# Bismarrck/tensoralloy

Hardware: AMD Instinct MI355X
Metric: atom-steps/sec (energy+forces), 4000-atom Ni rcut=6.5 A (higher is better)
Workload: dtype f64

## Files before the change

### tensoralloy_amd/csrc/ta_api.hip

```cpp
#include <hip/hip_runtime.h>

#include <algorithm>
#include <chrono>
#include <climits>
#include <cmath>
#include <cstdio>
#include <cstdlib>
#include <cstring>
#include <stdexcept>
#include <string>
#include <vector>

#include "ta_device.h"
#include "ta_internal.h"
#include "ta_md.h"
#include "ta_neb.h"
#include "ta_relax.h"

namespace ta {
size_t mlp_scratch_doubles(const MlpDev &mlp);
void launch_mlp_impl(const MlpDev &mlp, int activation, int ndim, const int32_t *atoms, int n_atoms,
                     const DeviceBatch &b, const Options &opt, double *scratch, hipStream_t s,
                     MlpLaunchInfo *info = nullptr);
size_t mlp_all_scratch_doubles(const MlpDev *mlps_host, int nel, const int32_t *elem_start);
size_t td_scratch_doubles(const MlpDev *nets, int nel, int K, const int32_t *elem_start, bool da_global);
void launch_td_all(const MlpDev *nets_dev, const MlpDev *nets_host, int nel, int K, int act_h, int act,
                   int sommerfeld, int ndim, const DeviceBatch &b, bool da_global, const double *T, double *u_atom,
                   double *s_atom, double *scratch, hipStream_t s, MlpLaunchInfo *info = nullptr);
void launch_mlp_all(const MlpDev *mlps_dev, const MlpDev *mlps_host, int nel, int activation, int ndim,
                    const DeviceBatch &b, const Options &opt, double *scratch, hipStream_t s,
                    MlpLaunchInfo *info = nullptr);
int mlp_param_count(const MlpDev &mlp);
size_t mlp_grad_scratch_doubles(const MlpDev &mlp, int n_atoms);
size_t mlp_grad_partial_doubles(const MlpDev &mlp, int n_atoms);
void launch_mlp_grad(const MlpDev &mlp, int activation, int ndim, const int32_t *atoms, int n_atoms,
                     const DeviceBatch &b, const double *frame_coeff, double *scratch, double *partial,
                     double *grad, hipStream_t s);
size_t mlp_grad2_scratch_doubles(const MlpDev &mlp, int n_atoms);
void launch_mlp_grad2(const MlpDev &mlp, int activation, int ndim, const int32_t *atoms, int n_atoms,
                      const DeviceBatch &b, const double *dG, const double *frame_coeff, double *scratch,
                      double *partial, double *grad, hipStream_t s, double *kappa_out = nullptr);
int td_param_count(const MlpDev *nets, int nel);
void td_grad2_sizes(const MlpDev *nets, int nel, int K, const int32_t *elem_start, size_t *scratch,
                    size_t *partial);
void launch_td_grad2(const MlpDev *nets_dev, const MlpDev *nets_host, int nel, int K, int act_h, int act,
                     int sommerfeld, int ndim, const DeviceBatch &b, const double *T, const double *dG,
                     const double *coeff, double *scratch, double *partial, double *grad, hipStream_t s);
void launch_pair_vec(const DeviceBatch &b, double *Dv, hipStream_t s);
void launch_backward_hvp(const SFParams &sf, const AngChunk &ch, int nb, int ng, int nz, bool first, bool angular,
                         const DeviceBatch &b, const double *Dv, const double *Dd, const double *wdot, double *gv,
                         double *gd, hipStream_t s);
void launch_hvp_gather(const DeviceBatch &b, const double *Dv, const double *Dd, const double *gv, const double *gd,
                       double *fdot, double *wdot_at, hipStream_t s);
void launch_pair_tangent(const DeviceBatch &b, const double *dR, const double *dh, double *dD, hipStream_t s);
void launch_descriptor_jvp(const DeviceBatch &b, int ndim, const double *J, const double *dD, double *dG,
                           hipStream_t s);
void launch_one_hot(double *dEdG, int64_t n_atoms, int ndim, int c, hipStream_t s);
struct GrapModel;
bool grap_hvp_supported(const GrapModel *);
void launch_grap_hvp(GrapModel *, const DeviceBatch &b, double eps, const double *Dv, const double *Dd,
                     const double *wdot, double *gv, double *gd, hipStream_t s);
GrapModel *grap_create(const ta_model_desc *m, std::string &err);
int grap_ndim(const GrapModel *g);
bool grap_uses_filter_net(const GrapModel *g);
void grap_destroy(GrapModel *);
void grap_ensure(GrapModel *, const DeviceBatch &b);
void launch_grap_forward(GrapModel *, const DeviceBatch &b, double eps, hipStream_t s);
void launch_grap_backward(GrapModel *, const DeviceBatch &b, hipStream_t s);
int64_t grap_filter_param_count(const GrapModel *g);
void grap_update_filter_weights(GrapModel *g, const double *flat, int64_t n, hipStream_t s);
int grap_filter_table_knots(const GrapModel *g);
void grap_set_filter_tables(GrapModel *g, bool on, int n_knots, hipStream_t s);
int grap_filter_table_target(const GrapModel *g, bool on, int n_knots);
void grap_mark_trained(GrapModel *g);
void grap_suspend_filter_tables(GrapModel *g, bool suspend);
std::string grap_filter_train_refusal(const GrapModel *g);
size_t grap_filter_grad_doubles(const GrapModel *g, const DeviceBatch &b);
void launch_grap_filter_tangent(GrapModel *g, const DeviceBatch &b, double eps, const double *Dv, const double *Dd,
                                double *Gdot, hipStream_t s);
void grap_filter_gradient(GrapModel *g, const DeviceBatch &b, double eps, const double *Dv, const double *Dd,
                          const double *kappa, double *scratch, double *grad, hipStream_t s);
struct EamModel;
EamModel *eam_create(const ta_model_desc *m, const Options &opt, std::string &err);
void eam_destroy(EamModel *);
void eam_ensure(EamModel *, const DeviceBatch &b);
void eam_tabulate(EamModel *m, int n_r, const double *r, int n_rho, const double *rho, double *rho_of_r,
                  double *phi_of_r, double *embed_of_rho, double *u_of_r, double *w_of_r,
                  hipStream_t s);
void eam_compute(EamModel *, const DeviceBatch &b, uint32_t want, hipStream_t s,
                 hipEvent_t *ev );
void eam_set_list_cutoff(EamModel *, double rc );
bool eam_is_plain(const EamModel *);
void eam_set_nn_tables(EamModel *, bool on);
bool eam_hvp_supported(const EamModel *);
size_t eam_hvp_extra_doubles(const EamModel *, const DeviceBatch &b, int n_dir);
void eam_hvp(EamModel *, const DeviceBatch &b, int n_dir, bool unit, int first, const double *dR, const double *dh,
             double *dFdot, double *fdot, double *wdot, double *extra, hipStream_t s);
bool eam_nn_tables_on(const EamModel *);
void eam_mark_trained(EamModel *);
int64_t eam_param_count(const EamModel *);
void eam_update_weights(EamModel *, const double *flat, int64_t n);
int64_t eam_constant_count(const EamModel *);
void eam_get_constants(const EamModel *, double *flat);
void eam_update_constants(EamModel *, const double *flat, int64_t n);
void eam_constant_gradient(EamModel *, const DeviceBatch &b, const double *frame_coeff, const double *dR,
                           const double *dh, double *grad, hipStream_t s);
void eam_energy_gradient(EamModel *, const DeviceBatch &b, const double *frame_coeff, double *grad,
                         hipStream_t s);
bool eam_loss_gradient_supported(const EamModel *);
void eam_loss_gradient(EamModel *, const DeviceBatch &b, const double *frame_coeff, const double *dR,
                       const double *dh, double *grad, hipStream_t s);
}

namespace {

thread_local std::string g_create_error;

struct HipError : std::runtime_error {
  using std::runtime_error::runtime_error;
};

#define HIP_CHECK(expr)                                                                      \
  do {                                                                                       \
    hipError_t _e = (expr);                                                                  \
    if (_e != hipSuccess)                                                                    \
      throw HipError(std::string(#expr) + ": " + hipGetErrorString(_e) + " (" __FILE__ ":" + \
                     std::to_string(__LINE__) + ")");                                        \
  } while (0)

template <typename T>
struct DevBuf {
  T *ptr = nullptr;
  size_t cap = 0;
  void ensure(size_t n) {
    if (n <= cap) return;
    size_t want = n + n / 8 + 64;
    T *fresh = nullptr;
    hipError_t e = hipMalloc((void **)&fresh, want * sizeof(T));
    if (e != hipSuccess && ptr) {
      (void)hipGetLastError();
      HIP_CHECK(hipFree(ptr));
      ptr = nullptr;
      cap = 0;
      e = hipMalloc((void **)&fresh, want * sizeof(T));
    }
    if (e != hipSuccess) {
      (void)hipGetLastError();
      throw HipError(std::string("hipMalloc of ") + std::to_string(want * sizeof(T)) + " bytes: " +
                     hipGetErrorString(e));
    }
    if (ptr) HIP_CHECK(hipFree(ptr));
    ptr = fresh;
    cap = want;
  }
  void release() {
    if (ptr) (void)hipFree(ptr);
    ptr = nullptr;
    cap = 0;
  }
};

__global__ __launch_bounds__(256) void staged_copy_kernel(double *__restrict__ dst,
                                                          const double *__restrict__ src, size_t n) {
  for (size_t k = (size_t)blockIdx.x * 256 + threadIdx.x; k < n; k += (size_t)gridDim.x * 256) dst[k] = src[k];
}
constexpr size_t kStagedCopyMaxBytes = 4u << 20;

void staged_copy(double *dst, const double *src, size_t n, bool to_host, const ta::Options &opt, hipStream_t s) {
  if (n == 0) return;
  if (n * sizeof(double) > kStagedCopyMaxBytes || opt.staged_copy_dma) {
    HIP_CHECK(hipMemcpyAsync(dst, src, n * sizeof(double), to_host ? hipMemcpyDeviceToHost : hipMemcpyHostToDevice, s));
    return;
  }
  const unsigned blocks = (unsigned)std::min<size_t>((n + 255) / 256, 256);
  hipLaunchKernelGGL(staged_copy_kernel, dim3(blocks), dim3(256), 0, s, dst, src, n);
  HIP_CHECK(hipGetLastError());
}

void wait_stream(hipStream_t s, const ta::Options &opt) {
  if (!opt.sync_blocking) {
    const auto t0 = std::chrono::steady_clock::now();
    for (;;) {
      const hipError_t e = hipStreamQuery(s);
      if (e == hipSuccess) return;
      if (e != hipErrorNotReady) {
        (void)hipGetLastError();
        break;
      }
      if (std::chrono::steady_clock::now() - t0 > std::chrono::microseconds(400)) break;
    }
  }
  HIP_CHECK(hipStreamSynchronize(s));
}

struct PinnedBuf {
  char *ptr = nullptr;
  size_t cap = 0;
  void ensure(size_t n) {
    if (n <= cap) return;
    if (ptr) HIP_CHECK(hipHostFree(ptr));
    ptr = nullptr;
    cap = 0;
    size_t want = n + n / 8 + 256;
    HIP_CHECK(hipHostMalloc((void **)&ptr, want, hipHostMallocDefault));
    cap = want;
  }
  void release() {
    if (ptr) (void)hipHostFree(ptr);
    ptr = nullptr;
    cap = 0;
  }
};

struct ChunkPlan {
  ta::AngChunk ch;
  int nb, ng, nz;
};

}

struct ta_context {
  ta::Options opt;
  int device = 0;
  hipStream_t stream = nullptr;
  hipStream_t own_stream = nullptr;
  int kind = 0;
  int n_elements = 0;
  int activation = 0;
  double rmax = 0.0;
  ta::SFParams sf;
  std::vector<ChunkPlan> chunks;
  std::vector<ChunkPlan> chunks_v2;
  bool use_v2 = false;
  ta::MlpDev *mlp_dev = nullptr;
  ta::MlpDev mlp[ta::kMaxElements];
  bool td = false, td_sommerfeld = false;
  int td_act = 0, td_K = 0;
  ta::MlpDev td_nets[3 * ta::kMaxElements];
  ta::MlpDev *td_dev = nullptr;
  std::vector<void *> model_allocs;
  ta::EamModel *eam = nullptr;
  ta::GrapModel *grap = nullptr;

  ta::HostPairs hp;
  ta::DeviceBatch db;
  bool have_batch = false;
  uint32_t last_want = 0;

  PinnedBuf stage_in, stage_out;
  DevBuf<char> inbuf;
  DevBuf<double> results;
  size_t o_blk = 0;
  int res_n_blk = 0;
  DevBuf<double> rec, part4, G, dEdG, g, wat, bpart, fown, benergy, mlp_scratch;
  DevBuf<double> td_T, td_u, td_s;
  DevBuf<unsigned long long> masks;
  DevBuf<uint32_t> job_word;
  DevBuf<int32_t> job_count;
  DevBuf<uint32_t> job_word_own;
  DevBuf<int32_t> job_count_own;
  bool triangles = true;
  bool tri_cells_ok = false;
  bool tri_cells_wide_ok = false;
  int last_bwd_variant = 0;
  ta::MlpLaunchInfo last_mlp_launch;
  DevBuf<int32_t> pair_start, seg_start, pair_i, pair_j, pair_shift, pair_rev;
  ta::NlGrid *d_grids = nullptr;
  DevBuf<int32_t> nl_wrap, nl_binid, nl_bin_count, nl_bin_start, nl_bin_cursor, nl_bin_atoms, nl_counts;
  DevBuf<unsigned long long> nl_stats, nl_zero;
  unsigned long long *nl_stats_ptr = nullptr;
  bool nl_sorted = false;
  bool nl_rev_done = false;
  bool nl_zero_clean = false;
  int64_t nl_zero_atoms = -1;
  int nl_zero_bins = -1;
  DevBuf<double> hvp_buf;
#ifdef TA_PHASE_STAMPS
  DevBuf<unsigned long long> stamp_buf;
#endif
  DevBuf<ta::NlRec> nl_recs;
  bool pairs_on_device = false;
  bool descriptors_valid = false;
  DevBuf<double> train_scratch, train_partial, train_grad, train_coeff;
  DevBuf<double> jvp_J, tan_dD, tan_dG, tan_dir;
  DevBuf<double> filt_scratch;
  bool jvp_valid = false;

  double skin = 0.0;
  double r_list = 0.0;
  std::vector<int32_t> keep_species;
  std::vector<int32_t> keep_natoms, keep_pbc;
  std::vector<double> ref_pos, ref_cells;
  size_t o_pos = 0, o_cells = 0, o_species = 0;
  DevBuf<int32_t> ex_pair_i, ex_pair_j, ex_pair_shift, ex_pair_rev, ex_pair_start, ex_pair_stop, ex_seg_start, ex_counts,
      ex_map, ex_blk, ex_slot_q;
  bool filtered = false;
  bool upload_pending = false;
  bool mirror_next = false;
  uint32_t mirror_want = 0;
  int64_t n_list_builds = 0, n_list_reuses = 0;

  bool md_valid = false;
  DevBuf<double> md_mass, md_vel, md_ref, md_epot, md_ke;
  DevBuf<int32_t> md_blk_start;
  DevBuf<unsigned> md_status;
  PinnedBuf md_status_host;
  std::vector<int32_t> md_blk_start_host;
  int md_chunk = 0, md_n_blk = 0;
  int64_t md_ref_builds = -1;
  double md_kT0 = 0.0, md_tau = 0.0;
  double md_lv_kT0 = 0.0, md_friction = 0.0;
  uint64_t md_seed = 0;
  int64_t md_step = 0;
  DevBuf<double> md_noise;
  bool md_baro_on = false;
  bool md_baro_running = false;
  ta_md_barostat_params md_baro_p = {0.0, 0.0, 0.0, {1, 1, 1}, 1};
  DevBuf<double> md_baro_scale, md_baro_rec;
  std::vector<double> md_baro_ones;
  bool md_rec_valid = false;
  std::vector<double> md_rec_volume, md_rec_press;

  bool relax_valid = false;
  ta_fire_params relax_p = {0.1, 1.0, 0.2, 1.1, 0.5, 0.1, 0.99, 5};
  DevBuf<double> relax_vel, relax_part;
  DevBuf<uint8_t> relax_fixed;
  DevBuf<ta::RelaxFrameState> relax_state;
  DevBuf<int> relax_count;
  std::vector<ta::RelaxFrameState> relax_state_host;
  bool relax_cell_on = false;
  bool cell_running = false;
  ta_relax_cell_params relax_cell_p = {0.0, 0.0, {1, 1, 1, 1, 1, 1}, 0, 0};
  DevBuf<double> relax_cell_h0, relax_cell_cf, relax_cell_G, relax_cell_vel, relax_cell_fmax2, md_ref_cells;
  std::vector<double> relax_cell_G_host, relax_cell_vel_host;
  bool relax_band_on = false;
  bool relax_band_ran = false;
  ta_band_params relax_band_p = {0.1, 0, 0};
  std::vector<uint8_t> relax_fixed_host;
  DevBuf<double> band_force, band_tau, band_part;
  DevBuf<uint8_t> band_fixed;
  DevBuf<ta::RelaxFrameState> band_state;
  DevBuf<int32_t> band_layout;
  ta::RelaxFrameState band_state_host = {};
  std::vector<double> band_energy_host;

  hipEvent_t ev[2 * TA_N_KERNEL_SLOTS + 2] = {nullptr};
  std::string err;
};

namespace {

int fail(ta_context *h, int code, const std::string &msg) {
  if (h)
    h->err = msg;
  else
    g_create_error = msg;
  return code;
}

std::string td_inference_only(const char *fn) {
  return std::string(fn) + ": not available for finite-temperature (temperature-dependent) models "
         "(no analytic Hessian-vector products)";
}

std::string fs_inference_only(const char *fn) {
  return std::string(fn) + ": not available for eam/fs models (inference only: no weight, constant or loss "
         "gradients and no analytic Hessian-vector products; differences of the forces give the latter)";
}

template <typename T>
T *upload(ta_context *h, const std::vector<T> &v) {
  T *d = nullptr;
  size_t n = v.size() ? v.size() : 1;
  HIP_CHECK(hipMalloc((void **)&d, n * sizeof(T)));
  h->model_allocs.push_back(d);
  if (!v.empty()) HIP_CHECK(hipMemcpy(d, v.data(), v.size() * sizeof(T), hipMemcpyHostToDevice));
  return d;
}

int round_up(int x, int m) { return (x + m - 1) / m * m; }

void hd_series(int cutoff, double beta, ta::AngChunk &ch) {
  ch.n_hd = 0;
  for (double &c : ch.hd) c = 0.0;
  if (cutoff != TA_CUTOFF_COSINE || !(beta >= 0.0)) return;
  constexpr int NT = 64;
  const long double pi2 = 9.869604401089358618834490999876151135L;
  long double fc[NT], ex[NT], prod[NT];
  long double t = 1.0L;
  for (int k = 0; k < NT; ++k) {
    fc[k] = 0.5L * t + (k == 0 ? 0.5L : 0.0L);
    t *= -pi2 / (long double)((2 * k + 1) * (2 * k + 2));
  }
  t = 1.0L;
  for (int k = 0; k < NT; ++k) {
    ex[k] = t;
    t *= -(long double)beta / (long double)(k + 1);
  }
  for (int k = 0; k < NT; ++k) {
    long double acc = 0.0L;
    for (int j = 0; j <= k; ++j) acc += fc[j] * ex[k - j];
    prod[k] = acc;
  }
  constexpr int N0 = 40;
  static long double tstar[N0][N0];
  static bool have_t = false;
  if (!have_t) {
    for (auto &row : tstar)
      for (auto &c : row) c = 0.0L;
    tstar[0][0] = 1.0L;
    tstar[1][0] = -1.0L;
    tstar[1][1] = 2.0L;
    for (int n = 1; n + 1 < N0; ++n)
      for (int k = 0; k <= n + 1; ++k)
        tstar[n + 1][k] = (k > 0 ? 4.0L * tstar[n][k - 1] : 0.0L) - 2.0L * tstar[n][k] - tstar[n - 1][k];
    have_t = true;
  }
  long double tail0 = 0.0L, dtail0 = 0.0L;
  for (int k = N0; k < NT; ++k) {
    tail0 += fabsl(prod[k]);
    dtail0 += (long double)k * fabsl(prod[k]);
  }
  for (int n : {12, 16, 24}) {
    long double a[N0];
    for (int k = 0; k < N0; ++k) a[k] = prod[k];
    long double err = tail0, derr = dtail0;
    for (int d = N0 - 1; d >= n; --d) {
      const long double q = a[d] / tstar[d][d];
      for (int k = 0; k <= d; ++k) a[k] -= q * tstar[d][k];
      err += fabsl(q);
      derr += 2.0L * (long double)d * (long double)d * fabsl(q);
    }
    if (err < 1e-17L && derr < 1e-15L) {
      ch.n_hd = n;
      for (int k = 0; k < n; ++k) ch.hd[k] = (double)a[k];
      return;
    }
  }
}

void build_mlp(ta_context *h, const ta_model_desc *m, int ndim);

void build_sf_model(ta_context *h, const ta_model_desc *m) {
  using namespace ta;
  SFParams &sf = h->sf;
  std::memset(&sf, 0, sizeof(sf));
  const int nel = m->n_elements;
  if (m->n_eta < 1 || m->n_omega < 1 || !m->eta || !m->omega)
    throw std::invalid_argument("eta / omega must be non-empty");
  if (m->n_eta * m->n_omega > kMaxRadial)
    throw std::domain_error("more than 64 radial (eta x omega) combinations");
  if (!(m->rcut > 0.0)) throw std::invalid_argument("rcut must be positive");
  sf.rcut = m->rcut;
  sf.acut = m->angular ? m->acut : m->rcut;
  if (m->angular && !(m->acut > 0.0)) throw std::invalid_argument("acut must be positive");
  sf.inv_rc2 = 1.0 / (sf.rcut * sf.rcut);
  sf.inv_ac2 = 1.0 / (sf.acut * sf.acut);
  sf.two_inv_ac2 = 2.0 * sf.inv_ac2;
  sf.eps = m->eps > 0.0 ? m->eps : 1e-14;
  sf.n_elements = nel;
  sf.n_rad = m->n_eta * m->n_omega;
  sf.angular = m->angular ? 1 : 0;
  sf.cutoff = m->cutoff_function;
  if (sf.cutoff != TA_CUTOFF_COSINE && sf.cutoff != TA_CUTOFF_POLYNOMIAL)
    throw std::invalid_argument("unknown cutoff function");
  for (int e = 0; e < m->n_eta; ++e)
    for (int o = 0; o < m->n_omega; ++o) {
      sf.eta[e * m->n_omega + o] = m->eta[e];
      sf.omega[e * m->n_omega + o] = m->omega[o];
    }
  for (int c = 1; c < sf.n_rad; ++c) {
    if ((c & 3) == 0 || sf.omega[c] != sf.omega[c - 1] || !(sf.eta[c - 1] > 0.0)) continue;
    const double k = sf.eta[c] / sf.eta[c - 1];
    if (k >= 2.0 && k <= 16.0 && k == std::nearbyint(k) && k * sf.eta[c - 1] == sf.eta[c] &&
        !h->opt.no_eta_chain)
      sf.eta_pow[c] = (signed char)k;
  }
  sf.n_radial_dim = nel * sf.n_rad;
  sf.n_ang = 0;
  sf.n_beta = 0;
  if (m->angular) {
    if (m->n_beta < 1 || m->n_gamma < 1 || m->n_zeta < 1 || !m->beta || !m->gamma || !m->zeta)
      throw std::invalid_argument("beta / gamma / zeta must be non-empty for an angular model");
    if (m->n_beta > kMaxBetaSlots)
      throw std::domain_error("more than 3 beta values are not supported by the pair record");
    sf.n_beta = m->n_beta;
    for (int k = 0; k < m->n_beta; ++k) sf.beta[k] = m->beta[k];
    sf.n_ang = m->n_beta * m->n_gamma * m->n_zeta;
    for (int pass = 0; pass < 2; ++pass)
    for (int b0 = 0; b0 < m->n_beta; b0 += (pass == 0 ? 2 : 1))
      for (int g0 = 0; g0 < m->n_gamma; g0 += 2)
        for (int z0 = 0; z0 < m->n_zeta; z0 += 2) {
          ChunkPlan cp;
          std::memset(&cp, 0, sizeof(cp));
          cp.nb = std::min(pass == 0 ? 2 : 1, m->n_beta - b0);
          cp.ng = std::min(2, m->n_gamma - g0);
          cp.nz = std::min(2, m->n_zeta - z0);
          for (int ib = 0; ib < cp.nb; ++ib) {
            cp.ch.beta[ib] = m->beta[b0 + ib];
            cp.ch.hslot[ib] = b0 + ib;
          }
          cp.ch.safe_pow = m->safe_pow ? 1 : 0;
          for (int ig = 0; ig < cp.ng; ++ig) cp.ch.gamma[ig] = m->gamma[g0 + ig];
          for (int iz = 0; iz < cp.nz; ++iz) {
            const double z = m->zeta[z0 + iz];
            cp.ch.zeta[iz] = z;
            cp.ch.kz[iz] = std::pow(2.0, 1.0 - z);
            const double zr = std::nearbyint(z);
            cp.ch.zeta_int[iz] = (zr == z && z >= 1.0 && z <= 1024.0) ? (int)zr : -1;
          }
          for (int ib = 0; ib < cp.nb; ++ib)
            for (int ig = 0; ig < cp.ng; ++ig)
              for (int iz = 0; iz < cp.nz; ++iz)
                cp.ch.chan[(ib * cp.ng + ig) * cp.nz + iz] =
                    ((b0 + ib) * m->n_gamma + (g0 + ig)) * m->n_zeta + (z0 + iz);
          if (pass == 1) hd_series(sf.cutoff, cp.ch.beta[0], cp.ch);
          (pass == 0 ? h->chunks : h->chunks_v2).push_back(cp);
        }
  }
  const int n_aterms = m->angular ? nel * (nel + 1) / 2 : 0;
  (void)0;
  sf.ndim = sf.n_radial_dim + n_aterms * sf.n_ang;
  h->rmax = std::max(sf.rcut, sf.acut);
  build_mlp(h, m, sf.ndim);
}

void build_net(ta_context *h, ta::MlpDev &md, int L, const int32_t *sizes, const double *&wsrc, int resnet) {
  using namespace ta;
  if (L < 1 || L > kMaxLayers) throw std::domain_error("MLP depth out of range (1..8 layers)");
  md.n_layers = L;
  md.max_np = md.max_kp = 0;
  for (int l = 0; l < L; ++l) {
    MlpLayerDev &ly = md.layer[l];
    ly.k = sizes[l];
    ly.n = sizes[l + 1];
    if (ly.k < 1 || ly.n < 1 || ly.k > 512 || ly.n > 512)
      throw std::domain_error("MLP layer width out of range (1..512)");
    ly.kp = round_up(ly.k, 16);
    ly.np = round_up(ly.n, 16);
    ly.act = (l < L - 1) ? 1 : 0;
    ly.res = (resnet && l > 0 && l < L - 1 && ly.k == ly.n) ? 1 : 0;
    std::vector<double> w((size_t)ly.kp * ly.np, 0.0), wt((size_t)ly.np * ly.kp, 0.0), bb(ly.np, 0.0);
    for (int k = 0; k < ly.k; ++k)
      for (int n = 0; n < ly.n; ++n) {
        const double v = wsrc[(size_t)k * ly.n + n];
        w[(size_t)k * ly.np + n] = v;
        wt[(size_t)n * ly.kp + k] = v;
      }
    wsrc += (size_t)ly.k * ly.n;
    for (int n = 0; n < ly.n; ++n) bb[n] = wsrc[n];
    wsrc += ly.n;
    ly.w = upload(h, w);
    ly.wt = upload(h, wt);
    ly.b = upload(h, bb);
    md.max_np = std::max(md.max_np, ly.np);
    md.max_kp = std::max(md.max_kp, ly.kp);
  }
}

void build_mlp(ta_context *h, const ta_model_desc *m, int ndim) {
  using namespace ta;
  const int nel = m->n_elements;
  if (!m->n_layers || !m->layer_sizes || !m->weights)
    throw std::invalid_argument("MLP description missing");
  h->activation = m->activation;
  if (m->activation < 0 || m->activation > TA_ACT_ELU)
    throw std::invalid_argument("unknown activation");
  const int td = m->finite_temperature;
  const int32_t *sizes = m->layer_sizes;
  const double *wsrc = m->weights;
  if (td) {
    if ((td & ~(TA_TD_ON | TA_TD_SOMMERFELD | (0xff << TA_TD_ACT_SHIFT))) || !(td & TA_TD_ON))
      throw std::invalid_argument("unknown finite_temperature bits");
    h->td = true;
    h->td_sommerfeld = (td & TA_TD_SOMMERFELD) != 0;
    h->td_act = (td >> TA_TD_ACT_SHIFT) & 0xff;
    if (h->td_act > TA_ACT_ELU) throw std::invalid_argument("unknown activation of the H nets");
    h->td_K = 0;
    for (int q = 0; q < 3; ++q)
      for (int el = 0; el < nel; ++el) {
        MlpDev &md = h->td_nets[q * nel + el];
        const int L = m->n_layers[q * nel + el];
        if (L < 1 || L > kMaxLayers) throw std::domain_error("MLP depth out of range (1..8 layers)");
        if (q == 0) {
          if (sizes[0] != ndim) throw std::invalid_argument("H input size does not match the descriptor length");
          if (el == 0) h->td_K = sizes[L];
          if (sizes[L] != h->td_K) throw std::invalid_argument("H output width differs between elements");
        } else {
          if (sizes[0] != h->td_K + 1) throw std::invalid_argument("U / S input size must be the H width + 1");
          if (sizes[L] != 1) throw std::invalid_argument("U / S output size must be 1");
        }
        build_net(h, md, L, sizes, wsrc, m->use_resnet_dt);
        if (q == 0 && m->minmax_scale) {
          if (!m->xlo || !m->xhi) throw std::invalid_argument("minmax_scale set but xlo/xhi missing");
          std::vector<double> lo(m->xlo + (size_t)el * ndim, m->xlo + (size_t)(el + 1) * ndim);
          std::vector<double> hi(m->xhi + (size_t)el * ndim, m->xhi + (size_t)(el + 1) * ndim);
          md.xlo = upload(h, lo);
          md.xhi = upload(h, hi);
// ... 204 lines not shown
            h->db.frame_of_atom, h->d_grids, w, h->pair_i.ptr, h->pair_j.ptr, h->pair_shift.ptr,
            h->pair_rev.ptr, h->stream);
  }
  HIP_CHECK(hipGetLastError());
}

#ifdef TA_PHASE_STAMPS
static void dump_stamps(ta_context *h) {
  const std::string &path = h->opt.phase_stamps_out;
  if (path.empty() || !h->db.stamps || h->db.n_blk <= 0) return;
  const size_t n = (size_t)2 * h->db.n_blk * 8;
  std::vector<unsigned long long> v(n);
  (void)hipStreamSynchronize(h->stream);
  (void)hipMemcpy(v.data(), h->db.stamps, n * sizeof(unsigned long long), hipMemcpyDeviceToHost);
  FILE *fp = std::fopen(path.c_str(), "w");
  if (!fp) return;
  for (int k = 0; k < 2; ++k)
    for (int b = 0; b < h->db.n_blk; ++b) {
      std::fprintf(fp, "%d %d", k, b);
      for (int q = 0; q < 8; ++q) std::fprintf(fp, " %llu", v[((size_t)k * h->db.n_blk + b) * 8 + q]);
      std::fprintf(fp, "\n");
    }
  std::fclose(fp);
}
#endif

void launch_head(ta_context *h, const ta::DeviceBatch &db, hipStream_t s) {
  if (h->td)
    ta::launch_td_all(h->td_dev, h->td_nets, h->n_elements, h->td_K, h->td_act, h->activation,
                      h->td_sommerfeld ? 1 : 0, h->sf.ndim, db, h->opt.mlp_da_global, h->td_T.ptr, h->td_u.ptr, h->td_s.ptr,
                      h->mlp_scratch.ptr, s, &h->last_mlp_launch);
  else
    ta::launch_mlp_all(h->mlp_dev, h->mlp, h->n_elements, h->activation, h->sf.ndim, db, h->opt, h->mlp_scratch.ptr,
                       s, &h->last_mlp_launch);
}

void compute_impl(ta_context *h, uint32_t want, bool timed, double *slot_ms) {
  using namespace ta;
#ifdef TA_PHASE_STAMPS
  if (h->db.n_blk > 0) {
    h->stamp_buf.ensure((size_t)2 * h->db.n_blk * 8 + 8);
    h->db.stamps = h->stamp_buf.ptr;
    (void)hipMemsetAsync(h->db.stamps, 0, (size_t)2 * h->db.n_blk * 8 * sizeof(unsigned long long), h->stream);
  }
#endif
  h->db.rec4 = nullptr;
  h->db.own_sums = 0;
  const DeviceBatch &db = h->db;
  hipStream_t s = h->stream;
  const bool need_forces = (want & (TA_WANT_FORCES | TA_WANT_VIRIAL)) != 0;
  auto begin = [&](int slot) {
    if (timed) HIP_CHECK(hipEventRecord(h->ev[2 * slot], s));
  };
  auto end = [&](int slot) {
    if (timed) HIP_CHECK(hipEventRecord(h->ev[2 * slot + 1], s));
  };
  bool used[TA_N_KERNEL_SLOTS] = {false};

  const bool has_mlp = h->kind == TA_MODEL_SF_MLP || h->kind == TA_MODEL_GRAP_MLP;
  if ((want & TA_WANT_REUSE_DESCRIPTORS) && has_mlp && h->descriptors_valid && !need_forces) {
    begin(TA_K_MLP);
    launch_head(h, db, s);
    end(TA_K_MLP);
    used[TA_K_MLP] = true;
  } else if (h->kind == TA_MODEL_SF_MLP) {
    h->db.rec4 = (h->sf.angular && h->use_v2 && !h->opt.full_records) ? h->db.rec : nullptr;
    if (!h->use_v2) {
      begin(TA_K_PAIR_GEOMETRY);
      launch_pair_geometry(h->sf, db, s);
      end(TA_K_PAIR_GEOMETRY);
      used[TA_K_PAIR_GEOMETRY] = true;
    }
    h->sf.ang_scale = h->use_v2 ? 1.0 : 0.5;
    const bool tri_cells = (h->relax_cell_on || h->md_baro_on) ? h->tri_cells_wide_ok : h->tri_cells_ok;
    const bool tri = h->use_v2 && h->triangles && tri_cells && h->n_elements == 1 && need_forces;
    h->db.job_word_own = (tri && h->db.job_count) ? h->job_word_own.ptr : nullptr;
    h->db.job_count_own = (tri && h->db.job_count) ? h->job_count_own.ptr : nullptr;
    h->last_bwd_variant = 0;
    const bool reduce_in_forward = h->sf.angular && h->use_v2;
    if (h->sf.angular) {
      begin(TA_K_G4_FORWARD);
      if (h->use_v2) {
        bool geometry = true;
        size_t left = h->chunks_v2.size();
        for (const ChunkPlan &cp : h->chunks_v2) {
          --left;
          launch_g4_forward_v2(h->sf, cp.ch, cp.ng, cp.nz, geometry, left == 0, db, h->opt, s);
          geometry = false;
        }
      } else
        for (const ChunkPlan &cp : h->chunks) launch_g4_forward(h->sf, cp.ch, cp.nb, cp.ng, cp.nz, db, s);
      end(TA_K_G4_FORWARD);
      used[TA_K_G4_FORWARD] = true;
    }
    if (!reduce_in_forward) {
      begin(TA_K_DESCRIPTOR_REDUCE);
      launch_descriptor_reduce(h->sf, db, s);
      end(TA_K_DESCRIPTOR_REDUCE);
      used[TA_K_DESCRIPTOR_REDUCE] = true;
    }
    begin(TA_K_MLP);
    launch_head(h, db, s);
    end(TA_K_MLP);
    used[TA_K_MLP] = true;
    if (need_forces) {
      begin(TA_K_BACKWARD);
      if (h->sf.angular) {
        bool first = true;
        if (h->use_v2)
          for (const ChunkPlan &cp : h->chunks_v2) {
            h->last_bwd_variant |= launch_backward_v2(h->sf, cp.ch, cp.ng, cp.nz, first, tri, db, h->opt, s);
            first = false;
          }
        else
          for (const ChunkPlan &cp : h->chunks) {
            launch_backward(h->sf, cp.ch, cp.nb, cp.ng, cp.nz, first, false, db, s);
            first = false;
          }
      } else {
        AngChunk dummy;
        std::memset(&dummy, 0, sizeof(dummy));
        launch_backward(h->sf, dummy, 1, 1, 1, true, true, db, s);
      }
      end(TA_K_BACKWARD);
      used[TA_K_BACKWARD] = true;
      begin(TA_K_FORCE_GATHER);
      launch_force_gather(h->sf, db, h->opt.gather_w, s);
      end(TA_K_FORCE_GATHER);
      used[TA_K_FORCE_GATHER] = true;
    }
  } else if (h->kind == TA_MODEL_GRAP_MLP) {
    const bool net_exact = ta::grap_uses_filter_net(h->grap) && !ta::grap_filter_table_knots(h->grap);
    h->db.rec4 = (!net_exact && !h->opt.full_records) ? h->db.rec : nullptr;
    begin(TA_K_GRAP);
    launch_grap_forward(h->grap, db, h->sf.eps, s);
    end(TA_K_GRAP);
    used[TA_K_GRAP] = true;
    begin(TA_K_MLP);
    launch_head(h, db, s);
    end(TA_K_MLP);
    used[TA_K_MLP] = true;
    if (need_forces) {
      begin(TA_K_BACKWARD);
      h->db.own_sums = h->opt.no_own_sums ? 0 : 1;
      launch_grap_backward(h->grap, db, s);
      end(TA_K_BACKWARD);
      used[TA_K_BACKWARD] = true;
      begin(TA_K_FORCE_GATHER);
      launch_force_gather(h->sf, db, h->opt.gather_w, s);
      end(TA_K_FORCE_GATHER);
      used[TA_K_FORCE_GATHER] = true;
    }
  } else {
    h->db.rec4 = h->opt.full_records ? nullptr : h->db.rec;
    begin(TA_K_EAM);
    eam_compute(h->eam, db, want, s, nullptr);
    end(TA_K_EAM);
    used[TA_K_EAM] = true;
  }
  begin(TA_K_FRAME_REDUCE);
  {
    double *mirror = nullptr;
    int64_t n_tail = 0;
    h->mirror_want = 0;
    if (h->mirror_next && !timed) {
      const size_t N = (size_t)db.n_atoms, F = (size_t)db.n_frames;
      h->stage_out.ensure((10 * F + 4 * N + 2) * sizeof(double));
      mirror = reinterpret_cast<double *>(h->stage_out.ptr);
      n_tail = (int64_t)(need_forces ? 4 * N : N);
      h->mirror_want = want | TA_WANT_ENERGY | TA_WANT_ATOMIC;
    }
    launch_frame_reduce(db, need_forces, mirror, n_tail, s);
  }
  end(TA_K_FRAME_REDUCE);
  used[TA_K_FRAME_REDUCE] = true;
  HIP_CHECK(hipGetLastError());
  h->last_want = want;
  h->descriptors_valid = true;

  if (timed) {
    HIP_CHECK(hipStreamSynchronize(s));
    for (int k = 0; k < TA_N_KERNEL_SLOTS; ++k) {
      if (!used[k]) continue;
      float ms = 0.f;
      HIP_CHECK(hipEventElapsedTime(&ms, h->ev[2 * k], h->ev[2 * k + 1]));
      slot_ms[k] += ms;
    }
  }
}

template <typename F>
int guarded(ta_context *h, F &&fn) {
  try {
    if (h) HIP_CHECK(hipSetDevice(h->device));
    fn();
    return TA_OK;
  } catch (const HipError &e) {
    return fail(h, TA_ERR_HIP, e.what());
  } catch (const std::domain_error &e) {
    return fail(h, TA_ERR_UNSUPPORTED, e.what());
  } catch (const std::invalid_argument &e) {
    return fail(h, TA_ERR_INVALID, e.what());
  } catch (const std::bad_alloc &) {
    return fail(h, TA_ERR_NOMEM, "host allocation failed");
  } catch (const std::exception &e) {
    return fail(h, TA_ERR_INVALID, e.what());
  }
}

}

extern "C" {

int ta_abi_version(void) { return TA_ABI_VERSION; }
int ta_model_desc_size(void) { return (int)sizeof(ta_model_desc); }

int ta_device_count(void) {
  int n = 0;
  if (hipGetDeviceCount(&n) != hipSuccess) return 0;
  return n;
}

const char *ta_last_error(ta_handle h) { return h ? h->err.c_str() : g_create_error.c_str(); }

int ta_create(const ta_model_desc *model, int device, ta_handle *out) {
  if (!model || !out) return fail(nullptr, TA_ERR_INVALID, "null argument");
  *out = nullptr;
  int ndev = 0;
  if (hipGetDeviceCount(&ndev) != hipSuccess || ndev <= 0)
    return fail(nullptr, TA_ERR_HIP, "no HIP device available: this library has no CPU fallback");
  if (device < 0 || device >= ndev) return fail(nullptr, TA_ERR_INVALID, "device index out of range");
  if (model->n_elements < 1 || model->n_elements > ta::kMaxElements)
    return fail(nullptr, TA_ERR_UNSUPPORTED, "n_elements must be in 1..8");
  ta_context *h = new ta_context();
  h->opt = ta::options_from_env();
  h->device = device;
  h->kind = model->kind;
  h->n_elements = model->n_elements;
  int rc = guarded(h, [&]() {
    hipDeviceProp_t prop;
    HIP_CHECK(hipGetDeviceProperties(&prop, device));
    if (std::strncmp(prop.gcnArchName, "gfx950", 6) != 0)
      throw HipError(std::string("device is ") + prop.gcnArchName +
                     ", this library is built for gfx950 only");
    HIP_CHECK(hipStreamCreateWithFlags(&h->own_stream, hipStreamNonBlocking));
    h->stream = h->own_stream;
    for (auto &e : h->ev) HIP_CHECK(hipEventCreate(&e));
    if (model->kind == TA_MODEL_SF_MLP) {
      build_sf_model(h, model);
    } else if (model->kind == TA_MODEL_GRAP_MLP) {
      if (model->cutoff_function != TA_CUTOFF_COSINE && model->cutoff_function != TA_CUTOFF_POLYNOMIAL)
        throw std::invalid_argument("unknown cutoff function");
      std::string err;
      h->grap = ta::grap_create(model, err);
      if (!h->grap) throw std::invalid_argument(err);
      h->rmax = model->rcut;
      std::memset(&h->sf, 0, sizeof(h->sf));
      h->sf.n_elements = model->n_elements;
      h->sf.eps = model->eps > 0.0 ? model->eps : 1e-14;
      h->sf.ndim = ta::grap_ndim(h->grap);
      build_mlp(h, model, h->sf.ndim);
    } else if (model->kind == TA_MODEL_EAM_ALLOY || model->kind == TA_MODEL_EAM_ADP || model->kind == TA_MODEL_EAM_FS) {
      std::string err;
      h->eam = ta::eam_create(model, h->opt, err);
      if (!h->eam) throw std::invalid_argument(err);
      h->rmax = model->rcut;
      std::memset(&h->sf, 0, sizeof(h->sf));
      h->sf.n_elements = model->n_elements;
      h->sf.eps = model->eps > 0.0 ? model->eps : 1e-14;
    } else {
      throw std::invalid_argument("unknown model kind");
    }
  });
  if (rc != TA_OK) {
    g_create_error = h->err;
    ta_destroy(h);
    return rc;
  }
  *out = h;
  return TA_OK;
}

int ta_destroy(ta_handle h) {
  if (!h) return TA_OK;
  (void)hipSetDevice(h->device);
#ifdef TA_PHASE_STAMPS
  dump_stamps(h);
#endif
  if (h->stream) (void)hipStreamSynchronize(h->stream);
  for (void *p : h->model_allocs) (void)hipFree(p);
  if (h->eam) ta::eam_destroy(h->eam);
  if (h->grap) ta::grap_destroy(h->grap);
  h->stage_in.release(); h->stage_out.release(); h->inbuf.release(); h->results.release();
  h->rec.release(); h->part4.release(); h->G.release();
  h->dEdG.release(); h->g.release(); h->wat.release(); h->bpart.release(); h->fown.release();
  h->benergy.release(); h->mlp_scratch.release();
  h->train_scratch.release(); h->train_partial.release(); h->train_grad.release(); h->train_coeff.release();
  h->jvp_J.release(); h->tan_dD.release(); h->tan_dG.release(); h->tan_dir.release();
  h->pair_start.release(); h->seg_start.release(); h->pair_i.release(); h->pair_j.release();
  h->pair_shift.release(); h->pair_rev.release();
  for (auto *b : {&h->ex_pair_i, &h->ex_pair_j, &h->ex_pair_shift, &h->ex_pair_rev, &h->ex_pair_start, &h->ex_pair_stop,
                  &h->ex_seg_start, &h->ex_counts, &h->ex_map, &h->ex_blk, &h->ex_slot_q})
    b->release();
  h->masks.release(); h->job_word.release(); h->job_count.release();
  h->job_word_own.release(); h->job_count_own.release();
  for (auto *b : {&h->nl_wrap, &h->nl_binid, &h->nl_bin_count, &h->nl_bin_start, &h->nl_bin_cursor,
                  &h->nl_bin_atoms, &h->nl_counts})
    b->release();
  h->nl_stats.release();
  h->nl_zero.release();
  h->hvp_buf.release();
  h->filt_scratch.release();
  h->nl_recs.release();
  for (auto *b : {&h->md_mass, &h->md_vel, &h->md_ref, &h->md_epot, &h->md_ke, &h->md_noise}) b->release();
  h->md_blk_start.release();
  h->md_status.release();
  h->md_status_host.release();
  h->relax_vel.release();
  h->relax_part.release();
  h->relax_fixed.release();
  h->relax_state.release();
  h->relax_count.release();
  for (auto *b : {&h->band_force, &h->band_tau, &h->band_part}) b->release();
  h->band_fixed.release();
  h->band_state.release();
  h->band_layout.release();
  for (auto *b : {&h->relax_cell_h0, &h->relax_cell_cf, &h->relax_cell_G, &h->relax_cell_vel, &h->relax_cell_fmax2,
                  &h->md_ref_cells})
    b->release();
  for (auto &e : h->ev)
    if (e) (void)hipEventDestroy(e);
  if (h->own_stream) (void)hipStreamDestroy(h->own_stream);
  delete h;
  return TA_OK;
}

}

namespace {
void ensure_job_lists(ta_context *h, size_t n_blk) {
  if (h->opt.no_jobs || !h->use_v2 || n_blk == 0) {
    h->db.job_count = nullptr;
    return;
  }
  const int stride = ta::v2_job_stride(h->db.cap);
  h->job_word.ensure(n_blk * (size_t)stride + 8);
  h->job_count.ensure(n_blk + 8);
  if (h->n_elements == 1) {
    h->job_word_own.ensure(n_blk * (size_t)stride + 8);
    h->job_count_own.ensure(n_blk + 8);
  }
  h->db.job_word = h->job_word.ptr;
  h->db.job_count = h->job_count.ptr;
  h->db.job_stride = stride;
}

bool filter_applies(const ta_context *h) {
  if (!(h->skin > 0.0) || h->hp.n_atoms == 0 || h->opt.no_list_filter) return false;
  if (h->kind == TA_MODEL_SF_MLP) return h->use_v2;
  if (h->kind == TA_MODEL_EAM_ALLOY || h->kind == TA_MODEL_EAM_FS) return ta::eam_is_plain(h->eam);
  return false;
}

void apply_filter(ta_context *h) {
  using namespace ta;
  const size_t N = (size_t)h->hp.n_atoms, P = (size_t)h->hp.n_pairs;
  const int nel = h->n_elements;
  h->ex_pair_i.ensure(P + 1);
  h->ex_pair_j.ensure(P + 1);
  h->ex_pair_shift.ensure(3 * P + 3);
  h->ex_pair_rev.ensure(P + 1);
  h->ex_pair_start.ensure(N + 1);
  h->ex_pair_stop.ensure(N + 1);
  h->ex_seg_start.ensure(N * (nel + 1) + 1);
  h->ex_map.ensure(P + 1);
  const int n_run_slots = nl_filter_blocks((int)N);
  h->ex_blk.ensure((size_t)n_run_slots + 4);
  const bool blocks = h->kind == TA_MODEL_SF_MLP;
  const bool indirect = blocks && !h->opt.filter_rev_kernel;
  if (indirect) h->ex_slot_q.ensure(P + 1);
  nl_filter((int)N, (int64_t)P, nel, h->rmax, h->db.pos, h->db.cells, h->db.frame_of_atom,
            h->pair_start.ptr, h->seg_start.ptr, h->pair_j.ptr, h->pair_shift.ptr, h->pair_rev.ptr, h->ex_map.ptr,
            h->ex_seg_start.ptr, h->ex_pair_start.ptr, h->ex_pair_stop.ptr, h->ex_pair_i.ptr, h->ex_pair_j.ptr,
            h->ex_pair_shift.ptr, h->ex_pair_rev.ptr, indirect ? h->ex_slot_q.ptr : nullptr, h->db.cap,
            blocks ? h->ex_blk.ptr : nullptr, h->stream);
  h->db.slot_q = indirect ? h->ex_slot_q.ptr : nullptr;
  h->db.rev_super = indirect ? h->pair_rev.ptr : nullptr;
  h->db.rev_map = indirect ? h->ex_map.ptr : nullptr;
  HIP_CHECK(hipGetLastError());
  h->db.pair_start = h->ex_pair_start.ptr;
  h->db.pair_stop = h->ex_pair_stop.ptr;
  h->db.seg_start = h->ex_seg_start.ptr;
  h->db.pair_i = h->ex_pair_i.ptr;
  h->db.pair_j = h->ex_pair_j.ptr;
  h->db.pair_shift = h->ex_pair_shift.ptr;
  h->db.pair_rev = h->ex_pair_rev.ptr;
  if (blocks) {
    h->db.blk_center = h->ex_blk.ptr;
    h->db.n_blk = n_run_slots;
    h->db.blk_groups = n_run_slots / 16;
    h->db.n_blk_dev = nullptr;
    ensure_job_lists(h, (size_t)n_run_slots);
  }
  h->filtered = true;
}

bool cells_admit_triangles(double rmax, int32_t n_frames, const ta_frame *frames) {
  for (int f = 0; f < n_frames; ++f) {
    const double *c = frames[f].cell;
    const double vol = std::fabs(c[0] * (c[4] * c[8] - c[5] * c[7]) - c[1] * (c[3] * c[8] - c[5] * c[6]) +
                                 c[2] * (c[3] * c[7] - c[4] * c[6]));
    for (int k = 0; k < 3; ++k) {
      if (!frames[f].pbc[k]) continue;
      const double *u = c + 3 * ((k + 1) % 3), *v = c + 3 * ((k + 2) % 3);
      const double nx = u[1] * v[2] - u[2] * v[1], ny = u[2] * v[0] - u[0] * v[2], nz = u[0] * v[1] - u[1] * v[0];
      const double area = std::sqrt(nx * nx + ny * ny + nz * nz);
      if (!(vol > rmax * area)) return false;
    }
  }
  return true;
}

void set_frames_impl(ta_context *h, int32_t n_frames, const ta_frame *frames, ta_batch_info *info) {
  for (int f = 0; f < n_frames; ++f) {
    const ta_frame &fr = frames[f];
    if (fr.n_atoms < 0 || (fr.n_atoms > 0 && (!fr.species || !fr.positions)) || !fr.cell || !fr.pbc)
      throw std::invalid_argument("frame " + std::to_string(f) + ": null array");
  }
  const auto t_begin = std::chrono::steady_clock::now();
  if (h->upload_pending) {
    HIP_CHECK(hipStreamSynchronize(h->stream));
    h->upload_pending = false;
  }
  h->have_batch = false;
  h->descriptors_valid = false;
  h->jvp_valid = false;
  h->mirror_want = 0;
  h->filtered = false;
  h->db.slot_q = h->db.rev_super = h->db.rev_map = nullptr;
  h->db.pair_stop = nullptr;
  h->db.blk_groups = 0;
  h->db.n_blk_dev = nullptr;
  h->r_list = h->rmax + h->skin;
  h->tri_cells_ok = cells_admit_triangles(h->rmax, n_frames, frames);
  h->tri_cells_wide_ok = cells_admit_triangles(h->r_list, n_frames, frames);
  size_t N = 0;
  for (int f = 0; f < n_frames; ++f) N += (size_t)frames[f].n_atoms;
  if (N >= (1u << 30)) throw std::runtime_error("batch too large for 32-bit atom indices");
  const size_t F = (size_t)n_frames;
  const int nel = h->n_elements;
  auto align16 = [](size_t x) { return (x + 15) & ~(size_t)15; };
  const size_t o_pos = 0;
  const size_t o_cells = align16(o_pos + 3 * N * sizeof(double));
  const size_t o_grids = align16(o_cells + 9 * F * sizeof(double));
  const size_t o_species = align16(o_grids + F * sizeof(ta::NlGrid));
  const size_t o_foa = align16(o_species + N * sizeof(int32_t));
  const size_t o_astart = align16(o_foa + N * sizeof(int32_t));
  const size_t o_elem = align16(o_astart + (F + 1) * sizeof(int32_t));
  const size_t o_blk = align16(o_elem + N * sizeof(int32_t));
  const size_t total = align16(o_blk + (N + 2) * sizeof(int32_t));
  h->stage_in.ensure(total);
  h->inbuf.ensure(total);
  char *hb = h->stage_in.ptr;
  double *pos = reinterpret_cast<double *>(hb + o_pos);
  double *cells = reinterpret_cast<double *>(hb + o_cells);
  ta::NlGrid *grids = reinterpret_cast<ta::NlGrid *>(hb + o_grids);
  int32_t *species = reinterpret_cast<int32_t *>(hb + o_species);
  int32_t *foa = reinterpret_cast<int32_t *>(hb + o_foa);
  int32_t *astart = reinterpret_cast<int32_t *>(hb + o_astart);
  int32_t *elem_atoms = reinterpret_cast<int32_t *>(hb + o_elem);
  size_t a = 0;
  astart[0] = 0;
  for (int f = 0; f < n_frames; ++f) {
    const ta_frame &fr = frames[f];
    const size_t n = (size_t)fr.n_atoms;
    if (n) {
      std::memcpy(&pos[3 * a], fr.positions, 3 * n * sizeof(double));
      std::memcpy(&species[a], fr.species, n * sizeof(int32_t));
    }
    std::memcpy(&cells[9 * (size_t)f], fr.cell, 9 * sizeof(double));
    for (size_t i = a; i < a + n; ++i) {
      foa[i] = f;
      if (species[i] < 0 || species[i] >= nel)
        throw std::runtime_error("frame " + std::to_string(f) + ": species index out of range");
      if (!std::isfinite(pos[3 * i]) || !std::isfinite(pos[3 * i + 1]) || !std::isfinite(pos[3 * i + 2]))
        throw std::runtime_error("frame " + std::to_string(f) + ": non-finite position");
    }
    a += n;
    astart[f + 1] = (int32_t)a;
  }
  {
    std::vector<int32_t> count(nel + 1, 0);
    for (size_t i = 0; i < N; ++i) count[species[i] + 1]++;
    for (int e = 0; e < nel; ++e) count[e + 1] += count[e];
    for (int e = 0; e <= nel; ++e) h->db.elem_start[e] = count[e];
    std::vector<int32_t> fill(count.begin(), count.end() - 1);
    for (size_t i = 0; i < N; ++i) elem_atoms[fill[species[i]]++] = (int32_t)i;
  }
  const auto t_nl = std::chrono::steady_clock::now();
  int n_bins = 0;
  bool device_nl = N > 0 && !h->opt.host_nl;
  for (int f = 0; f < n_frames && device_nl; ++f) {
    device_nl = ta::nl_make_grid(frames[f], h->r_list, n_bins, grids[f]);
    if (device_nl) n_bins += ta::nl_bins(grids[f]);
    if (n_bins > (1 << 24)) device_nl = false;
  }
  if (!device_nl) std::memset(static_cast<void *>(grids), 0, F * sizeof(ta::NlGrid));
  if (o_blk)
    staged_copy(reinterpret_cast<double *>(h->inbuf.ptr), reinterpret_cast<const double *>(hb), o_blk / sizeof(double),
                false, h->opt, h->stream);
  char *db_ = h->inbuf.ptr;
  h->db.n_frames = n_frames;
  h->db.pos = reinterpret_cast<double *>(db_ + o_pos);
  h->db.cells = reinterpret_cast<double *>(db_ + o_cells);
  h->d_grids = reinterpret_cast<ta::NlGrid *>(db_ + o_grids);
  h->db.species = reinterpret_cast<int32_t *>(db_ + o_species);
  h->db.frame_of_atom = reinterpret_cast<int32_t *>(db_ + o_foa);
  h->db.atom_start = reinterpret_cast<int32_t *>(db_ + o_astart);
  h->db.elem_atoms = reinterpret_cast<int32_t *>(db_ + o_elem);
  h->db.blk_center = reinterpret_cast<int32_t *>(db_ + o_blk);
  if (device_nl) {
    h->hp.atom_start.assign(astart, astart + F + 1);
    h->hp.frame_of_atom.assign(foa, foa + N);
    build_pairs_on_device(h, N, n_bins);
  } else {
    h->pairs_on_device = false;
    ta::build_pairs(n_frames, frames, nel, h->r_list, h->hp);
  }
  double nl_ms = std::chrono::duration<double, std::milli>(std::chrono::steady_clock::now() - t_nl).count();
  upload_batch(h);
  const auto t_fill = std::chrono::steady_clock::now();
  const bool list_done = h->pairs_on_device && h->nl_sorted && h->nl_rev_done;
  if (h->pairs_on_device && !list_done) {
    fill_pairs_on_device(h);
    staged_copy(reinterpret_cast<double *>(h->stage_out.ptr), reinterpret_cast<const double *>(h->nl_stats_ptr),
                8, true, h->opt, h->stream);
  }
  bool shapes_ok = h->n_elements <= 3;
  if (h->n_elements == 4 || h->n_elements == 5) {
    shapes_ok = !h->chunks_v2.empty();
    for (const ChunkPlan &cp : h->chunks_v2) shapes_ok = shapes_ok && cp.ng == 2 && cp.nz == 2;
  }
  h->use_v2 = h->kind == TA_MODEL_SF_MLP && h->sf.angular && shapes_ok &&
              h->hp.nnl_max <= ta::kCapMax && !h->opt.force_v1;
  const int cap = std::max(ta::kCapMin, (h->hp.nnl_max + 63) / 64 * 64);
  h->db.cap = cap;
  {
    int32_t *blk = reinterpret_cast<int32_t *>(hb + o_blk);
    int nb = 0;
    if (h->use_v2 && N) {
      blk[nb++] = 0;
      int32_t load = 0, ncent = 0;
      for (size_t i = 0; i < N; ++i) {
        const int32_t cnt = h->hp.pair_start[i + 1] - h->hp.pair_start[i];
        if (load + cnt > cap || ncent >= ta::kMaxCentersPerBlock) {
          blk[nb++] = (int32_t)i;
          load = 0;
          ncent = 0;
        }
        load += cnt;
        ++ncent;
      }
      blk[nb++] = (int32_t)N;
    }
    h->db.n_blk = nb ? nb - 1 : 0;
    h->res_n_blk = h->db.n_blk;
    h->o_blk = o_blk;
    ensure_job_lists(h, (size_t)h->db.n_blk);
    if (nb) {
      if (list_done)
        staged_copy(reinterpret_cast<double *>(db_ + o_blk), reinterpret_cast<const double *>(blk), ((size_t)nb + 1) / 2,
                    false, h->opt, h->stream);
      else
        HIP_CHECK(hipMemcpyAsync(db_ + o_blk, blk, (size_t)nb * sizeof(int32_t), hipMemcpyHostToDevice, h->stream));
    }
  }
  if (h->kind == TA_MODEL_SF_MLP) {
    if (!h->use_v2 && ta::g4_lds_bytes(h->hp.nnl_max) > 160 * 1024 && h->sf.angular)
      throw std::domain_error("more than 1150 neighbours per atom exceed the LDS staging buffer");
    size_t need = ta::mlp_all_scratch_doubles(h->mlp, h->n_elements, h->db.elem_start);
    h->mlp_scratch.ensure(need);
  } else if (h->kind == TA_MODEL_GRAP_MLP) {
    h->mlp_scratch.ensure(ta::mlp_all_scratch_doubles(h->mlp, h->n_elements, h->db.elem_start));
    ta::grap_ensure(h->grap, h->db);
  } else {
    ta::eam_ensure(h->eam, h->db);
  }
  if (h->td) {
    const size_t N = (size_t)h->db.n_atoms;
    h->mlp_scratch.ensure(ta::td_scratch_doubles(h->td_nets, h->n_elements, h->td_K, h->db.elem_start, h->opt.mlp_da_global));
    h->td_u.ensure(N + 1);
    h->td_s.ensure(N + 1);
    h->td_T.ensure((size_t)h->db.n_frames + 1);
  }
  h->o_pos = o_pos;
  h->o_cells = o_cells;
  h->o_species = o_species;
  h->ref_pos.assign(pos, pos + 3 * N);
  h->ref_cells.assign(cells, cells + 9 * F);
  h->keep_species.assign(species, species + N);
  h->keep_natoms.resize(F);
  h->keep_pbc.resize(3 * F);
  for (size_t f = 0; f < F; ++f) {
    h->keep_natoms[f] = frames[f].n_atoms;
    for (int a3 = 0; a3 < 3; ++a3) h->keep_pbc[3 * f + a3] = frames[f].pbc[a3] ? 1 : 0;
  }
  if (list_done) {
    h->upload_pending = true;
  } else {
    wait_stream(h->stream, h->opt);
    h->upload_pending = false;
  }
  if (h->pairs_on_device && !list_done) {
    nl_ms += std::chrono::duration<double, std::milli>(std::chrono::steady_clock::now() - t_fill).count();
    if (reinterpret_cast<const int32_t *>(h->stage_out.ptr)[6] != 0)
      throw std::runtime_error("neighbour list is not symmetric (reverse pair missing)");
  }
  if (filter_applies(h)) apply_filter(h);
  if (h->eam) ta::eam_set_list_cutoff(h->eam, (h->skin > 0.0 && !h->filtered) ? h->rmax : 0.0);
  ++h->n_list_builds;
  h->have_batch = true;
  if (info) {
    info->n_frames = n_frames;
    info->n_atoms = h->hp.n_atoms;
    info->n_pairs = h->hp.n_pairs;
    info->n_triples = h->hp.n_triples;
    info->nnl_max = h->hp.nnl_max;
    info->descriptor_dim = (h->kind == TA_MODEL_SF_MLP || h->kind == TA_MODEL_GRAP_MLP) ? h->sf.ndim : 0;
    info->nl_on_device = h->pairs_on_device ? 1 : 0;
    info->reserved_ = 0;
    info->nl_ms = nl_ms;
    info->set_frames_ms =
        std::chrono::duration<double, std::milli>(std::chrono::steady_clock::now() - t_begin).count();
  }
}
void rebuild_list(ta_context *h, const double *positions, const double *cells) {
  const size_t F = h->keep_natoms.size();
  std::vector<ta_frame> frames(F);
  const std::vector<int32_t> species(h->keep_species), pbc(h->keep_pbc), natoms(h->keep_natoms);
  const std::vector<double> old_cells(h->ref_cells);
  size_t a = 0;
  for (size_t f = 0; f < F; ++f) {
    frames[f].n_atoms = natoms[f];
    frames[f].species = species.data() + a;
    frames[f].positions = positions + 3 * a;
    frames[f].cell = (cells ? cells : old_cells.data()) + 9 * f;
    frames[f].pbc = pbc.data() + 3 * f;
    a += (size_t)natoms[f];
  }
  set_frames_impl(h, (int32_t)F, frames.data(), nullptr);
}
}

extern "C" {

int ta_set_frames(ta_handle h, int32_t n_frames, const ta_frame *frames, ta_batch_info *info) {
  if (!h) return TA_ERR_INVALID;
  if (n_frames < 0 || (n_frames > 0 && !frames)) return fail(h, TA_ERR_INVALID, "bad frames argument");
  h->md_valid = false;
  h->relax_valid = false;
  h->relax_cell_on = false;
  h->relax_band_on = h->relax_band_ran = false;
  return guarded(h, [&]() {
    set_frames_impl(h, n_frames, frames, info);
    if (h->td)
      HIP_CHECK(hipMemsetAsync(h->td_T.ptr, 0, (size_t)n_frames * sizeof(double), h->stream));
  });
}

int ta_set_electron_temperatures(ta_handle h, int32_t n_frames, const double *T) {
  if (!h) return TA_ERR_INVALID;
  if (!h->td) return fail(h, TA_ERR_INVALID, "ta_set_electron_temperatures: not a temperature-dependent model");
  if (!h->have_batch && h->keep_natoms.empty()) return fail(h, TA_ERR_INVALID, "no resident batch");
  if (n_frames != (int32_t)h->keep_natoms.size() || (n_frames > 0 && !T))
    return fail(h, TA_ERR_INVALID, "ta_set_electron_temperatures: one temperature per frame of the batch");
  for (int32_t f = 0; f < n_frames; ++f)
    if (!std::isfinite(T[f])) return fail(h, TA_ERR_INVALID, "electron temperatures must be finite");
  return guarded(h, [&]() {
    HIP_CHECK(hipStreamSynchronize(h->stream));
    if (n_frames > 0) {
      HIP_CHECK(hipMemcpyAsync(h->td_T.ptr, T, (size_t)n_frames * sizeof(double), hipMemcpyHostToDevice, h->stream));
      HIP_CHECK(hipStreamSynchronize(h->stream));
    }
  });
}

int ta_get_td_results(ta_handle h, double *energy, double *eentropy, double *energy_atomic, double *eentropy_atomic) {
  if (!h) return TA_ERR_INVALID;
  if (!h->td) return fail(h, TA_ERR_INVALID, "ta_get_td_results: not a temperature-dependent model");
  if (!h->have_batch) return fail(h, TA_ERR_INVALID, "no resident batch");
  return guarded(h, [&]() {
    const size_t N = (size_t)h->db.n_atoms, F = h->keep_natoms.size();
    std::vector<double> u(N), s(N);
    HIP_CHECK(hipStreamSynchronize(h->stream));
    if (N) {
      HIP_CHECK(hipMemcpy(u.data(), h->td_u.ptr, N * sizeof(double), hipMemcpyDeviceToHost));
      HIP_CHECK(hipMemcpy(s.data(), h->td_s.ptr, N * sizeof(double), hipMemcpyDeviceToHost));
    }
    if (energy_atomic && N) std::memcpy(energy_atomic, u.data(), N * sizeof(double));
    if (eentropy_atomic && N) std::memcpy(eentropy_atomic, s.data(), N * sizeof(double));
    size_t a = 0;
    for (size_t f = 0; f < F; ++f) {
      double su = 0.0, ss = 0.0;
      for (int32_t k = 0; k < h->keep_natoms[f]; ++k, ++a) {
        su += u[a];
        ss += s[a];
      }
      if (energy) energy[f] = su;
      if (eentropy) eentropy[f] = ss;
    }
  });
}

int ta_set_skin(ta_handle h, double skin) {
  if (!h) return TA_ERR_INVALID;
  if (!(skin >= 0.0) || !std::isfinite(skin)) return fail(h, TA_ERR_INVALID, "skin must be a finite length >= 0");
  if (skin != h->skin) {
    h->skin = skin;
    h->have_batch = false;
    h->descriptors_valid = false;
  }
  return TA_OK;
}

int ta_update_positions(ta_handle h, const double *positions, const double *cells, int32_t *rebuilt) {
  if (!h || !positions) return fail(h, TA_ERR_INVALID, "null argument");
  if (h->ref_pos.empty() && h->keep_natoms.empty())
    return fail(h, TA_ERR_INVALID, "ta_update_positions called before ta_set_frames");
  return guarded(h, [&]() {
    const size_t N = h->keep_species.size(), F = h->keep_natoms.size();
    bool keep = h->have_batch && h->skin > 0.0;
    if (keep && cells) keep = std::memcmp(cells, h->ref_cells.data(), 9 * F * sizeof(double)) == 0;
    if (keep) {
      if (h->upload_pending) {
        HIP_CHECK(hipStreamSynchronize(h->stream));
        h->upload_pending = false;
      }
      double *stage = reinterpret_cast<double *>(h->stage_in.ptr + h->o_pos);
      std::memcpy(stage, positions, 3 * N * sizeof(double));
      staged_copy(h->db.pos, stage, 3 * N, false, h->opt, h->stream);
      h->upload_pending = true;
      if (h->filtered) apply_filter(h);
      h->descriptors_valid = false;
      h->jvp_valid = false;
      const double lim2 = 0.25 * h->skin * h->skin;
      const double *ref = h->ref_pos.data();
      for (size_t i = 0; i < N; ++i) {
        const double dx = positions[3 * i] - ref[3 * i], dy = positions[3 * i + 1] - ref[3 * i + 1],
                     dz = positions[3 * i + 2] - ref[3 * i + 2];
        const double d2 = dx * dx + dy * dy + dz * dz;
        if (!(d2 <= lim2)) {
          keep = false;
          break;
        }
      }
    }
    if (rebuilt) *rebuilt = keep ? 0 : 1;
    if (keep) {
      ++h->n_list_reuses;
      return;
    }
    rebuild_list(h, positions, cells);
    if (cells && h->relax_cell_on && h->relax_valid && F) {
      HIP_CHECK(hipMemcpy(h->relax_cell_h0.ptr, h->ref_cells.data(), 9 * F * sizeof(double), hipMemcpyHostToDevice));
      h->relax_cell_G_host.assign(9 * F, 0.0);
      for (size_t f = 0; f < F; ++f) h->relax_cell_G_host[9 * f] = h->relax_cell_G_host[9 * f + 4] = h->relax_cell_G_host[9 * f + 8] = 1.0;
      h->relax_cell_vel_host.assign(9 * F, 0.0);
    }
  });
}

int ta_list_stats(ta_handle h, int64_t *n_builds, int64_t *n_reuses) {
  if (!h) return TA_ERR_INVALID;
  if (n_builds) *n_builds = h->n_list_builds;
  if (n_reuses) *n_reuses = h->n_list_reuses;
  return TA_OK;
}

int ta_list_sizes(ta_handle h, int64_t *n_pairs, int64_t *n_triples, int32_t *nnl_max) {
  if (!h) return TA_ERR_INVALID;
  if (!h->have_batch) return fail(h, TA_ERR_INVALID, "no resident batch");
  if (n_pairs) *n_pairs = h->hp.n_pairs;
  if (n_triples) *n_triples = h->hp.n_triples;
  if (nnl_max) *nnl_max = h->hp.nnl_max;
  return TA_OK;
}

int ta_compute(ta_handle h, uint32_t want) {
  if (!h) return TA_ERR_INVALID;
  if (!h->have_batch) return fail(h, TA_ERR_INVALID, "ta_compute called before ta_set_frames");
  return guarded(h, [&]() { compute_impl(h, want, false, nullptr); });
}

int ta_synchronize(ta_handle h) {
  if (!h) return TA_ERR_INVALID;
  return guarded(h, [&]() { HIP_CHECK(hipStreamSynchronize(h->stream)); });
}

namespace {
const double *results_to_stage(ta_context *h, bool energy, bool forces, bool virial, bool atomic, double *descriptors) {
  const size_t N = (size_t)h->db.n_atoms, F = (size_t)h->db.n_frames;
  hipStream_t s = h->stream;
  const bool have_forces = (h->last_want & (TA_WANT_FORCES | TA_WANT_VIRIAL)) != 0;
  if ((forces || virial) && !have_forces)
    throw std::invalid_argument("forces / virial requested but the last ta_compute did not produce them");
  if (descriptors && h->kind != TA_MODEL_SF_MLP && h->kind != TA_MODEL_GRAP_MLP)
    throw std::invalid_argument("descriptors are only defined for symmetry-function and GRAP models");
  size_t lo = (size_t)-1, hi = 0;
  auto need = [&](bool on, size_t off, size_t n) {
    if (!on || n == 0) return;
    lo = std::min(lo, off);
    hi = std::max(hi, off + n);
  };
  need(energy, 0, F);
  need(virial, F, 9 * F);
  need(atomic, 10 * F, N);
  need(forces, 10 * F + N, 3 * N);
  const double *stage = nullptr;
  const bool fv = (h->mirror_want & (TA_WANT_FORCES | TA_WANT_VIRIAL)) != 0;
  if (hi > lo && h->mirror_want && (!(forces || virial) || fv)) {
    stage = reinterpret_cast<const double *>(h->stage_out.ptr);
  } else if (hi > lo) {
    h->mirror_want = 0;
    h->stage_out.ensure((hi - lo) * sizeof(double));
    stage = reinterpret_cast<const double *>(h->stage_out.ptr) - lo;
    staged_copy(reinterpret_cast<double *>(h->stage_out.ptr), h->results.ptr + lo, hi - lo, true, h->opt, s);
  }
  if (descriptors && N)
    HIP_CHECK(hipMemcpyAsync(descriptors, h->db.G, N * h->sf.ndim * sizeof(double), hipMemcpyDeviceToHost, s));
  wait_stream(s, h->opt);
  h->upload_pending = false;
  return stage;
}
}

int ta_get_results(ta_handle h, double *energy, double *forces, double *virial, double *atomic,
                   double *descriptors) {
  if (!h) return TA_ERR_INVALID;
  if (!h->have_batch) return fail(h, TA_ERR_INVALID, "no resident batch");
  return guarded(h, [&]() {
    const size_t N = (size_t)h->db.n_atoms, F = (size_t)h->db.n_frames;
    const double *stage = results_to_stage(h, energy != nullptr, forces != nullptr, virial != nullptr,
                                           atomic != nullptr, descriptors);
    if (energy && F) std::memcpy(energy, stage, F * sizeof(double));
    if (virial && F) std::memcpy(virial, stage + F, 9 * F * sizeof(double));
    if (atomic && N) std::memcpy(atomic, stage + 10 * F, N * sizeof(double));
    if (forces && N) std::memcpy(forces, stage + 10 * F + N, 3 * N * sizeof(double));
  });
}

int ta_view_results(ta_handle h, uint32_t want, const double **energy, const double **forces,
                    const double **virial, const double **atomic) {
  if (!h) return TA_ERR_INVALID;
  if (!h->have_batch) return fail(h, TA_ERR_INVALID, "no resident batch");
  return guarded(h, [&]() {
    const size_t N = (size_t)h->db.n_atoms, F = (size_t)h->db.n_frames;
    const bool fv = (want & (TA_WANT_FORCES | TA_WANT_VIRIAL)) != 0;
    const double *stage = results_to_stage(h, energy != nullptr, forces && fv, virial && fv,
                                           atomic && (want & TA_WANT_ATOMIC), nullptr);
    if (energy) *energy = (stage && F) ? stage : nullptr;
    if (virial) *virial = (stage && fv && F) ? stage + F : nullptr;
    if (atomic) *atomic = (stage && (want & TA_WANT_ATOMIC) && N) ? stage + 10 * F : nullptr;
    if (forces) *forces = (stage && fv && N) ? stage + 10 * F + N : nullptr;
  });
}

int ta_step(ta_handle h, const double *positions, const double *cells, uint32_t want, double *energy,
            double *forces, double *virial, double *atomic, int32_t *rebuilt) {
  int rc = ta_update_positions(h, positions, cells, rebuilt);
  if (rc != TA_OK) return rc;
  h->mirror_next = true;
  rc = ta_compute(h, want);
  h->mirror_next = false;
  if (rc != TA_OK) return rc;
  return ta_get_results(h, energy, forces, virial, atomic, nullptr);
}

// ... 1986 lines not shown
```

### tensoralloy_amd/csrc/ta_device.h

```cpp
#pragma once
#include <hip/hip_runtime.h>

#include <cstdint>

#include "ta_options.h"
#include "tensoralloy_amd.h"

namespace ta {

constexpr int kMaxRadial = 64;
constexpr int kMaxElements = 8;
constexpr int kMaxBetaSlots = 3;
constexpr int kRecDoubles = 8;
constexpr int kMaxLayers = 8;
constexpr int kCapMin = 192;
constexpr int kCapMax = 1024;
constexpr int kMaxCentersPerBlock = 16;
constexpr int kMaxHd = 24;

struct SFParams {
  double rcut, acut;
  double inv_rc2, inv_ac2;
  double two_inv_ac2;
  double eps;
  double ang_scale;
  int n_elements;
  int n_rad;
  int n_ang;
  int n_radial_dim;
  int ndim;
  int angular;
  int cutoff;
  int n_beta;
  double eta[kMaxRadial], omega[kMaxRadial];
  double beta[kMaxBetaSlots];
  signed char eta_pow[kMaxRadial];
};

struct AngChunk {
  double beta[2];
  int hslot[2];
  double gamma[2];
  double zeta[2];
  double kz[2];
  int zeta_int[2];
  int chan[8];
  int safe_pow;
  int n_hd;
  double hd[kMaxHd];
};

struct DeviceBatch {
  int64_t n_atoms = 0, n_pairs = 0;
  int n_frames = 0, nnl_max = 0;
  double *pos = nullptr;
  double *cells = nullptr;
  int32_t *species = nullptr;
  int32_t *frame_of_atom = nullptr;
  int32_t *atom_start = nullptr;
  int32_t *pair_start = nullptr;
  int32_t *pair_stop = nullptr;
  int32_t *seg_start = nullptr;
  int32_t *pair_i = nullptr, *pair_j = nullptr, *pair_shift = nullptr, *pair_rev = nullptr;
  const int32_t *slot_q = nullptr, *rev_super = nullptr, *rev_map = nullptr;
  int32_t *blk_center = nullptr;
  int n_blk = 0;
  int blk_groups = 0;
  const int32_t *n_blk_dev = nullptr;
  int cap = kCapMin;
  int32_t *elem_atoms = nullptr;
  int32_t elem_start[kMaxElements + 1] = {0};

  double *rec = nullptr;
  double *rec4 = nullptr;
  double *part4 = nullptr;
  unsigned long long *masks = nullptr;
  uint32_t *job_word = nullptr;
  int32_t *job_count = nullptr;
  int job_stride = 0;
  uint32_t *job_word_own = nullptr;
  int32_t *job_count_own = nullptr;
  double *G = nullptr;
  double *dEdG = nullptr;
  double *eatom = nullptr;
  double *g = nullptr;
  double *forces = nullptr;
  double *wat = nullptr;
  double *fown = nullptr;
  int own_sums = 0;
#ifdef TA_PHASE_STAMPS
  unsigned long long *stamps = nullptr;
#endif
  double *bpart = nullptr;
  double *energy = nullptr;
  double *virial = nullptr;
  double *batch_energy = nullptr;
};

__host__ __device__ inline int triangle_owner_rank(uint32_t index_sum) {
#ifdef __HIP_DEVICE_COMPILE__
  const uint32_t h = __umul24(index_sum, 0x9E3779u);
#else
  const uint32_t h = index_sum * 0x9E3779u;
#endif
  return (int)(((h & 0xFFFFFFu) * 3u) >> 24);
}
__host__ __device__ inline bool owns_triangle(int32_t i, int32_t j, int32_t k) {
  return triangle_owner_rank((uint32_t)i + (uint32_t)j + (uint32_t)k) == (j < i ? 1 : 0) + (k < i ? 1 : 0);
}

#ifdef __HIPCC__
__device__ __forceinline__ int pair_stop_of(const DeviceBatch &b, int64_t i) {
  return b.pair_stop ? b.pair_stop[i] : b.pair_start[i + 1];
}
#endif

#ifdef __HIPCC__
__device__ __forceinline__ int pair_rev_of(const DeviceBatch &b, int q) {
  return b.slot_q ? b.rev_map[b.rev_super[b.slot_q[q]]] : b.pair_rev[q];
}
__device__ __forceinline__ const double2 *pair_geom(const DeviceBatch &b, size_t q) {
  return reinterpret_cast<const double2 *>(b.rec4 ? b.rec4 + 4 * q : b.rec + kRecDoubles * q);
}
#endif

struct MlpLayerDev {
  int k, n;
  int kp, np;
  double *w;
  double *wt;
  double *b;
  int act;
  int res;
};
struct MlpDev {
  int n_layers = 0;
  MlpLayerDev layer[kMaxLayers];
  double *xlo = nullptr, *xhi = nullptr;
  int max_np = 0, max_kp = 0;
};

struct MlpLaunchInfo {
  int family = 0;
  int threads = 0;
  int lh = 0;
  int nt = 0;
  int grid_x = 0, grid_y = 0;
  long long lds_bytes = 0;
  int da = 0;
};

void launch_pair_geometry(const SFParams &sf, const DeviceBatch &b, hipStream_t s);
void launch_g4_forward(const SFParams &sf, const AngChunk &ch, int nb, int ng, int nz,
                       const DeviceBatch &b, hipStream_t s);
void launch_descriptor_reduce(const SFParams &sf, const DeviceBatch &b, hipStream_t s);
void launch_mlp(const SFParams &sf, const MlpDev &mlp, int activation, int element,
                const DeviceBatch &b, hipStream_t s);
void launch_backward(const SFParams &sf, const AngChunk &ch, int nb, int ng, int nz,
                     bool first, bool radial_only, const DeviceBatch &b, hipStream_t s);
void launch_force_gather(const SFParams &sf, const DeviceBatch &b, int gather_w, hipStream_t s);
void launch_frame_reduce(const DeviceBatch &b, bool want_virial, double *mirror, int64_t n_tail, hipStream_t s);

size_t g4_lds_bytes(int nnl_max);

size_t v2_lds_bytes(bool backward, int cap, int n_local = 0, int nspec = 0, bool triangles = false);
int v2_job_stride(int cap);
void launch_g4_forward_v2(const SFParams &sf, const AngChunk &ch, int ng, int nz, bool geometry,
                          bool reduce, const DeviceBatch &b, const Options &opt, hipStream_t s);
int launch_backward_v2(const SFParams &sf, const AngChunk &ch, int ng, int nz, bool first, bool triangles,
                       const DeviceBatch &b, const Options &opt, hipStream_t s);

struct NlGrid {
  double h[9];
  double hinv[9];
  double lo[3];
  double inv_w[3];
  int32_t nb[3];
  int32_t pbc[3];
  int32_t bin_offset;
  int32_t pad_;
  int32_t m[3];
  int32_t ortho;
  double bw[3];
};
struct NlRec {
  double x, y, z;
  int32_t wx, wy, wz;
  int32_t j;
  int32_t sp;
  int32_t pad_;
};
struct NlWork {
  int32_t *wrap;
  int32_t *binid;
  int32_t *bin_count;
  int32_t *bin_start;
  int32_t *bin_cursor;
  int32_t *bin_atoms;
  NlRec *recs;
  int32_t *counts;
  int32_t *seg_start;
  unsigned long long *stats;
};
bool nl_make_grid(const ta_frame &fr, double rmax, int bin_offset, NlGrid &g);
int nl_bins(const NlGrid &g);
void nl_count(int n_atoms, int n_bins, int nel, double rmax, const double *pos, const int32_t *species,
              const int32_t *frame_of_atom, const NlGrid *grids, NlWork &w, int32_t *pair_start,
              hipStream_t s);
size_t nl_build_zero_words(int n_atoms, int n_bins);
void nl_build(int n_atoms, int n_bins, int nel, double rmax, const double *pos, const int32_t *species,
              const int32_t *frame_of_atom, const NlGrid *grids, NlWork &w, unsigned long long *zero,
              bool zero_is_clean, long long capacity, int32_t *pair_start, int32_t *host_pair_start,
              int32_t *pair_i, int32_t *pair_j, int32_t *pair_shift, int32_t *pair_rev, long long rev_cover,
              hipStream_t s);
void nl_reverse_sorted(int64_t n_pairs, int nel, const int32_t *species, const int32_t *seg_start,
                       const int32_t *pair_i, const int32_t *pair_j, const int32_t *pair_shift,
                       int32_t *pair_rev, unsigned long long *stats, hipStream_t s);
int nl_filter_blocks(int n_atoms);
void nl_filter(int n_atoms, int64_t n_super, int nel, double rmax, const double *pos, const double *cells,
               const int32_t *frame_of_atom, const int32_t *start_super, const int32_t *seg_super,
               const int32_t *pj_super, const int32_t *ps_super, const int32_t *rev_super, int32_t *map,
               int32_t *seg_exact, int32_t *pair_start, int32_t *pair_stop, int32_t *pi_out, int32_t *pj_out,
               int32_t *ps_out, int32_t *rev_out, int32_t *slot_q, int cap, int32_t *blk_center, hipStream_t s);
void nl_fill(int n_atoms, int64_t n_pairs, int nel, double rmax, const double *pos,
             const int32_t *species, const int32_t *frame_of_atom, const NlGrid *grids, NlWork &w,
             int32_t *pair_i, int32_t *pair_j, int32_t *pair_shift, int32_t *pair_rev, hipStream_t s);

}
```

### tensoralloy_amd/csrc/ta_kernels_v2.hip

```cpp
#include <hip/hip_runtime.h>

#include <cstdio>
#include <cstdlib>
#include <stdexcept>
#include <type_traits>

#include "ta_device.h"
#include "ta_math.h"
#include "ta_reduce.h"

namespace ta {
namespace {

constexpr int kBlock = 256;
constexpr int kNF = 8;
constexpr int kNFf = 7;
constexpr int kSegW = 6;
constexpr int kOwnCtl = 60 + 2 * kMaxCentersPerBlock * kSegW;
constexpr int kJobCtlBytes = (kOwnCtl + 40) * 4;
__host__ __device__ inline int v2_pcols(int cap, int nspec) {
  return nspec >= 1 ? cap / 4 + kMaxCentersPerBlock * nspec : cap;
}
constexpr int kRingPad = 64;
constexpr int kRTab = 8;

#ifdef TA_LDS_PROBE
__device__ __forceinline__ bool kProbe(int flags, int bit) { return (flags >> bit) & 1; }
#else
__device__ __forceinline__ constexpr bool kProbe(int, int) { return false; }
#endif

#ifdef TA_PHASE_STAMPS
#define TA_STAMP(b, kernel, k)                                                                          \
  do {                                                                                                  \
    if ((b).stamps && threadIdx.x == 0)                                                                 \
      (b).stamps[((size_t)(kernel) * gridDim.x + blockIdx.x) * 8 + (k)] = __builtin_amdgcn_s_memrealtime(); \
  } while (0)
#else
#define TA_STAMP(b, kernel, k) do {} while (0)
#endif

__device__ __forceinline__ int angular_term2(int s1, int s2, int nel) {
  int a = s1 < s2 ? s1 : s2, b = s1 < s2 ? s2 : s1;
  return a * nel - (a * (a - 1)) / 2 + (b - a);
}
__device__ __forceinline__ int radial_term2(int center, int other) {
  return other == center ? 0 : (other < center ? other + 1 : other);
}

struct Fields {
  double2 *zr, *xy, *ih, *gs;
  double *sp1;
  float *xf, *yf, *zf;
};

__device__ __forceinline__ Fields carve(double *lds, int cap, bool forward = false) {
  Fields f;
  f.zr = reinterpret_cast<double2 *>(lds);
  f.xy = f.zr + cap;
  f.ih = f.xy + cap;
  f.gs = forward ? nullptr : f.ih + cap;
  f.sp1 = forward ? reinterpret_cast<double *>(f.ih + cap) : nullptr;
  f.xf = forward ? reinterpret_cast<float *>(f.sp1 + cap) : nullptr;
  f.yf = forward ? f.xf + (2 * cap + kRingPad) : nullptr;
  f.zf = forward ? f.yf + (2 * cap + kRingPad) : nullptr;
  return f;
}

template <int HD>
__device__ __forceinline__ void hd_eval(const SFParams &sf, const AngChunk &ch, double beta,
                                        double u, double &h, double &dh) {
  if constexpr (HD > 0) {
    double p = ch.hd[HD - 1], d = 0.0;
#pragma unroll
    for (int k = HD - 2; k >= 0; --k) {
      d = fma(d, u, p);
      p = fma(p, u, ch.hd[k]);
    }
    h = p;
    dh = d;
  } else {
    double fd, dfd;
    cutoff_u(sf.cutoff, u, fd, dfd);
    const double ed = ta_exp(-beta * u);
    h = ed * fd;
    dh = ed * (dfd - beta * fd);
  }
}
template <int HD>
__device__ __forceinline__ double hd_value(const SFParams &sf, const AngChunk &ch, double beta,
                                           double u) {
  if constexpr (HD > 0) {
    double p = ch.hd[HD - 1];
#pragma unroll
    for (int k = HD - 2; k >= 0; --k) p = fma(p, u, ch.hd[k]);
    return p;
  } else {
    return ta_exp(-beta * u) * cutoff_u_value(sf.cutoff, u);
  }
}

template <int HD>
__device__ __forceinline__ void stage(const SFParams &sf, const AngChunk &ch, double beta, const DeviceBatch &b,
                                      const Fields &f, int s0, int M, int geom = 0, bool forward = false,
                                      int *jidx = nullptr) {
  for (int item = threadIdx.x; item < M; item += blockDim.x) {
    double2 v0, v1, v2;
    if (geom) {
      const int64_t p = (int64_t)s0 + item;
      const int i = b.pair_i[p], j = b.pair_j[p];
      const double *h = b.cells + 9 * (size_t)b.frame_of_atom[i];
      const double sx = (double)b.pair_shift[3 * p], sy = (double)b.pair_shift[3 * p + 1],
                   sz = (double)b.pair_shift[3 * p + 2];
      const double *ri = b.pos + 3 * (size_t)i, *rj = b.pos + 3 * (size_t)j;
      const double dx = (rj[0] - ri[0]) + (sx * h[0] + sy * h[3] + sz * h[6]);
      const double dy = (rj[1] - ri[1]) + (sx * h[1] + sy * h[4] + sz * h[7]);
      const double dz = (rj[2] - ri[2]) + (sx * h[2] + sy * h[5] + sz * h[8]);
      const double r2 = dx * dx + dy * dy + dz * dz + sf.eps;
      v0 = make_double2(dx, dy);
      v1 = make_double2(dz, r2);
      v2 = make_double2(1.0 / sqrt(r2), 0.0);
      if (b.rec4) {
        double2 *dst = reinterpret_cast<double2 *>(b.rec4 + 4 * (size_t)p);
        dst[0] = v0;
        dst[1] = v1;
      } else {
        double2 *dst = reinterpret_cast<double2 *>(b.rec + kRecDoubles * (size_t)p);
        dst[0] = v0;
        dst[1] = v1;
        dst[2] = v2;
        dst[3] = make_double2(0.0, 0.0);
      }
    } else if (b.rec4) {
      const double2 *src = reinterpret_cast<const double2 *>(b.rec4 + 4 * (size_t)(s0 + item));
      v0 = src[0];
      v1 = src[1];
      v2 = make_double2(1.0 / sqrt(v1.y), 0.0);
    } else {
      const double2 *src = reinterpret_cast<const double2 *>(b.rec + kRecDoubles * (size_t)(s0 + item));
      v0 = src[0];
      v1 = src[1];
      v2 = src[2];
    }
    f.xy[item] = v0;
    f.zr[item] = v1;
    if (forward) {
      const int ci = b.pair_i[s0 + item];
      const int cbase = b.pair_start[ci] - s0, cn = pair_stop_of(b, ci) - b.pair_start[ci];
      const int k0 = 2 * cbase + (item - cbase);
      f.xf[k0] = f.xf[k0 + cn] = (float)v0.x;
      f.yf[k0] = f.yf[k0 + cn] = (float)v0.y;
      f.zf[k0] = f.zf[k0 + cn] = (float)v1.x;
    }
    const double u = v1.y * sf.inv_ac2;
    double H = 0.0, L = 0.0;
    if (u < 1.0) {
      if (forward) {
        H = hd_value<HD>(sf, ch, beta, u);
      } else {
        double dH;
        hd_eval<HD>(sf, ch, beta, u, H, dH);
        L = (H != 0.0) ? sf.two_inv_ac2 * dH / H : 0.0;
      }
    }
    f.ih[item] = make_double2(v2.x, H);
    if (jidx) jidx[item] = b.pair_j[s0 + item];
    else if (forward) f.sp1[item] = (double)b.species[b.pair_j[s0 + item]];
    else f.gs[item] = make_double2(L, (double)b.species[b.pair_j[s0 + item]]);
  }
  __syncthreads();
}

__device__ __forceinline__ unsigned long long partner_mask(const SFParams &sf, const Fields &f,
                                                           int base, int n, int a, int sc, int smax) {
  const int ring = 2 * base + a;
  const float ax = f.xf[ring], ay = f.yf[ring], az = f.zf[ring];
  const float lim = (float)(sf.acut * sf.acut) * 1.0001f;
  unsigned long long mask = 0ull;
  const int count = smax - sc + 1;
  typedef float f32x2 __attribute__((ext_vector_type(2)));
  const f32x2 ax2 = {ax, ax}, ay2 = {ay, ay}, az2 = {az, az};
  for (int g = 0; g < 4 && 16 * g < count; ++g) {
    const float *px = f.xf + ring + sc + 16 * g, *py = f.yf + ring + sc + 16 * g,
                *pz = f.zf + ring + sc + 16 * g;
    unsigned m = 0u;
#pragma unroll
    for (int k = 14; k >= 0; k -= 2) {
      const f32x2 vx = {px[k], px[k + 1]}, vy = {py[k], py[k + 1]}, vz = {pz[k], pz[k + 1]};
      const f32x2 ex = vx - ax2, ey = vy - ay2, ez = vz - az2;
      const f32x2 d2 = __builtin_elementwise_fma(ex, ex, __builtin_elementwise_fma(ey, ey, ez * ez));
      const float dhi = d2.y, dlo = d2.x;
      asm("v_cmp_lt_f32 vcc, %1, %2\n\tv_addc_co_u32 %0, vcc, %0, %0, vcc" : "+v"(m) : "v"(dhi), "v"(lim) : "vcc");
      asm("v_cmp_lt_f32 vcc, %1, %2\n\tv_addc_co_u32 %0, vcc, %0, %0, vcc" : "+v"(m) : "v"(dlo), "v"(lim) : "vcc");
    }
    mask |= (unsigned long long)m << (16 * g);
  }
  if (count < 64) mask &= (1ull << count) - 1ull;
  const int half = n >> 1;
  if (!(n & 1) && a >= half && half >= sc && half < sc + 64) mask &= ~(1ull << (half - sc));
  return mask;
}

__device__ __forceinline__ void deal_by_popcount(const Fields &f, int cap, int M, int &item,
                                                 unsigned long long &mask) {
  int *hist = reinterpret_cast<int *>(f.xf);
  int *start = hist + 66;
  unsigned long long *pmask = reinterpret_cast<unsigned long long *>(hist + 132);
  int *pitem = reinterpret_cast<int *>(pmask + cap);
  const int tid = threadIdx.x;
  const bool active = tid < M;
  __syncthreads();
  if (tid < 66) hist[tid] = 0;
  __syncthreads();
  const int bucket = 64 - (active ? __popcll(mask) : 0);
  int rank = 0;
  if (active) rank = atomicAdd(&hist[bucket], 1);
  __syncthreads();
  if (tid < 65) {
    int s = 0;
    for (int k = 0; k < tid; ++k) s += hist[k];
    start[tid] = s;
  }
  __syncthreads();
  if (active) {
    const int slot = start[bucket] + rank;
    pitem[slot] = item;
    pmask[slot] = mask;
  }
  __syncthreads();
  if (active) {
    item = pitem[tid];
    mask = pmask[tid];
  }
}

struct JobLists {
  uint32_t *word;
  int *hist, *start;
};

__device__ __forceinline__ JobLists job_lists(const Fields &f) {
  JobLists j;
  j.word = reinterpret_cast<uint32_t *>(f.xf);
  return j;
}
__device__ __forceinline__ int job_item(uint32_t w) { return (int)(w & 255u); }
__device__ __forceinline__ int job_centre(uint32_t w) { return (int)((w >> 10) & 15u); }
static_assert(kMaxCentersPerBlock <= 16, "four bits of a job word name the centre");

__host__ __device__ inline size_t v2_counter_offset(int cap) {
  const size_t end = (size_t)cap * kNFf * sizeof(double) + 3 * (size_t)(2 * cap + kRingPad) * sizeof(float);
  return (end + 15) & ~(size_t)15;
}
__host__ __device__ inline int v2_max_jobs(int cap) { return 4 * cap; }

__device__ __forceinline__ int make_jobs(JobLists &j, bool active, int item, int centre, unsigned long long m0) {
  const int tid = threadIdx.x;
  int cnt[4] = {0, 0, 0, 0}, rank[4] = {0, 0, 0, 0};
  if (active) {
#pragma unroll
    for (int w = 0; w < 4; ++w) {
      const int c = __popc((unsigned)((m0 >> (16 * w)) & 0xffffull));
      cnt[w] = c;
      if (c) rank[w] = atomicAdd(&j.hist[16 - c], 1);
    }
  }
  __syncthreads();
  if (tid < 64) {
    const int v = tid < 16 ? j.hist[tid] : 0;
    int incl = v;
#pragma unroll
    for (int off = 1; off < 16; off <<= 1) {
      const int u = __shfl_up(incl, off);
      if (tid >= off) incl += u;
    }
    if (tid < 16) j.start[tid] = incl - v;
    if (tid == 15) j.start[16] = incl;
  }
  __syncthreads();
  if (active) {
#pragma unroll
    for (int w = 0; w < 4; ++w)
      if (cnt[w]) {
        const int slot = j.start[16 - cnt[w]] + rank[w];
        j.word[slot] = (uint32_t)item | ((uint32_t)w << 8) | ((uint32_t)centre << 10) |
                       ((uint32_t)((m0 >> (16 * w)) & 0xffffull) << 16);
      }
  }
  const int n = j.start[16];
  __syncthreads();
  return n;
}

__device__ __forceinline__ int job_slot(int r, int tid, int T) { return r * T + ((r & 1) ? T - 1 - tid : tid); }

__device__ __forceinline__ void make_owned_jobs(int *hist, int *start, const uint32_t word[4], const unsigned own[4],
                                                uint32_t *out, int32_t *count) {
  const int tid = threadIdx.x;
  int cnt[4], rank[4] = {0, 0, 0, 0};
#pragma unroll
  for (int r = 0; r < 4; ++r) {
    cnt[r] = __popc(own[r]);
    if (cnt[r]) rank[r] = atomicAdd(&hist[16 - cnt[r]], 1);
  }
  __syncthreads();
  if (tid < 64) {
    const int v = tid < 16 ? hist[tid] : 0;
    int incl = v;
#pragma unroll
    for (int off = 1; off < 16; off <<= 1) {
      const int u = __shfl_up(incl, off);
      if (tid >= off) incl += u;
    }
    if (tid < 16) start[tid] = incl - v;
    if (tid == 15) *count = incl;
  }
  __syncthreads();
#pragma unroll
  for (int r = 0; r < 4; ++r)
    if (cnt[r]) out[start[16 - cnt[r]] + rank[r]] = (word[r] & 0xffffu) | (own[r] << 16);
}

template <int NG, int NZ>
__device__ __forceinline__ void defz_coeffs(const AngChunk &ch, const double *wsrc, double pc[5]) {
  double p0 = 0.0, p1 = 0.0, p2 = 0.0, p3 = 0.0, p4 = 0.0;
#pragma unroll
  for (int ig = 0; ig < NG; ++ig) {
    const double g1 = ch.gamma[ig], g2 = g1 * g1;
    const double w1 = wsrc[ch.chan[ig * NZ]] * ch.kz[0], w4 = wsrc[ch.chan[ig * NZ + 1]] * ch.kz[1];
    p0 += w1 + w4;
    p1 += g1 * (w1 + 4.0 * w4);
    p2 += 6.0 * g2 * w4;
    p3 += 4.0 * g2 * g1 * w4;
    p4 += g2 * g2 * w4;
  }
  pc[0] = p0;
  pc[1] = 0.5 * p1;
  pc[2] = 0.25 * p2;
  pc[3] = 0.125 * p3;
  pc[4] = 0.0625 * p4;
}

__device__ __forceinline__ double rsqrt_f64(double x) {
  double y = __builtin_amdgcn_rsq(x);
  const double hx = 0.5 * x;
  y = fma(y, fma(-hx * y, y, 0.5), y);
  y = fma(y, fma(-hx * y, y, 0.5), y);
  return y;
}

__device__ __forceinline__ void reduce_radial_from_lds(const SFParams &sf, const DeviceBatch &b,
                                                       const Fields &f, int c0, int c1, int s0) {
  const int nel = sf.n_elements;
  const int w = threadIdx.x >> 6, l = threadIdx.x & 63, nwaves = blockDim.x >> 6;
  bool no_shift = true;
  for (int c = 0; c < sf.n_rad; ++c) no_shift = no_shift && sf.omega[c] == 0.0;
  for (int64_t i = c0 + w; i < c1; i += nwaves) {
    const int sA = b.species[i];
    const int32_t *seg = b.seg_start + (size_t)i * (nel + 1);
    double *Gi = b.G + (size_t)i * sf.ndim;
    for (int sb = 0; sb < nel; ++sb) {
      const int tr = radial_term2(sA, sb);
      const int q0 = seg[sb] - s0, q1 = seg[sb + 1] - s0;
      for (int cc = 0; cc < sf.n_rad; cc += 4) {
        double acc[4] = {0.0, 0.0, 0.0, 0.0};
        for (int q = q0 + l; q < q1; q += 64) {
          const double r2 = f.zr[q].y;
          const double u = r2 * sf.inv_rc2;
          const double fc = (u < 1.0) ? cutoff_u_value(sf.cutoff, u) : 0.0;
          if (no_shift) {
#pragma unroll
            for (int k = 0; k < 4; ++k) {
              const int c = (cc + k < sf.n_rad) ? cc + k : cc;
              acc[k] += ta_exp(-sf.eta[c] * u) * fc;
            }
          } else {
            const double r = sqrt(r2);
#pragma unroll
            for (int k = 0; k < 4; ++k) {
              const int c = (cc + k < sf.n_rad) ? cc + k : cc;
              const double dr = r - sf.omega[c];
              acc[k] += ta_exp(-sf.eta[c] * dr * dr * sf.inv_rc2) * fc;
            }
          }
        }
#pragma unroll
        for (int k = 0; k < 4; ++k) {
          const double v = wave_sum(acc[k]);
          if (l == 0 && cc + k < sf.n_rad) Gi[tr * sf.n_rad + cc + k] = v;
        }
      }
    }
  }
}

template <int NSPEC, int NG, int NZ>
__device__ __forceinline__ void reduce_angular_from_lds(const SFParams &sf, const AngChunk &ch,
                                                        const DeviceBatch &b, const double *red, int cap,
                                                        int c0, int c1, int s0, int sp_lo, int sp_hi) {
  const int nel = sf.n_elements;
  const int w = threadIdx.x >> 6, l = threadIdx.x & 63, nwaves = blockDim.x >> 6;
  for (int64_t i = c0 + w; i < c1; i += nwaves) {
    const int32_t *seg = b.seg_start + (size_t)i * (nel + 1);
    double *Gi = b.G + (size_t)i * sf.ndim + sf.n_radial_dim;
    for (int sp = sp_lo; sp < sp_hi; ++sp)
      for (int sg = 0; sg < NSPEC; ++sg) {
        const int t = angular_term2(sg, sp, nel);
        const int q0 = seg[sg] - s0, q1 = seg[sg + 1] - s0;
#pragma unroll
        for (int gz = 0; gz < NG * NZ; ++gz) {
          double v = 0.0;
          const double *col = red + (size_t)((sp - sp_lo) * NG * NZ + gz) * cap;
          for (int q = q0 + l; q < q1; q += 64) v += col[q];
          v = wave_sum(v) * sf.ang_scale;
          if (l == 0) {
            double *dst = Gi + t * sf.n_ang + ch.chan[gz];
            *dst = (sg >= sp) ? v : *dst + v;
          }
        }
      }
  }
}

template <int NSPEC, int NG, int NZ>
__device__ __forceinline__ void assemble_flat(const SFParams &sf, const AngChunk &ch, const DeviceBatch &b,
                                              const Fields &f, const double *P, const int *sslot, int c0, int c1,
                                              int s0, int item, bool active, bool skip_radial, int cap) {
  constexpr int kGZ = NG * NZ;
  constexpr int kTerms = NSPEC * (NSPEC + 1) / 2;
  double *R = reinterpret_cast<double *>(f.xy);
  const int row = threadIdx.x >> 4, l = threadIdx.x & 15, nrows = blockDim.x >> 4;
  const int ncent = c1 - c0;
  bool no_shift = true;
  for (int c = 0; c < sf.n_rad; ++c) no_shift = no_shift && sf.omega[c] == 0.0;
  const double r2 = active ? f.zr[item].y : 0.0;
  const int n_rad = skip_radial ? 0 : sf.n_rad;
  for (int cc = 0; cc == 0 || cc < n_rad; cc += 4) {
    if (cc) __syncthreads();
    if (active && cc < n_rad) {
      const double u = r2 * sf.inv_rc2;
      const double fc = (u < 1.0) ? cutoff_u_value(sf.cutoff, u) : 0.0;
      const double r = no_shift ? 0.0 : sqrt(r2);
      double ev[4];
#pragma unroll
      for (int k = 0; k < 4; ++k) {
        const int c = (cc + k < n_rad) ? cc + k : cc;
        const int pw = (cc + k < n_rad && k > 0) ? sf.eta_pow[c] : 0;
        if (pw > 0) {
          ev[k] = pow_int_m1(ev[k > 0 ? k - 1 : 0], pw) * ev[k > 0 ? k - 1 : 0];
        } else {
          double arg = sf.eta[c] * u;
          if (!no_shift) {
            const double dr = r - sf.omega[c];
            arg = sf.eta[c] * dr * dr * sf.inv_rc2;
          }
          ev[k] = ta_exp(-arg);
        }
        R[k * cap + item] = ev[k] * fc;
      }
    }
    __syncthreads();
    const int nrad_here = cc < n_rad ? (n_rad - cc < 4 ? n_rad - cc : 4) : 0;
    const int n_radial_tasks = NSPEC * nrad_here;
    const int per_centre = n_radial_tasks + (cc == 0 ? kTerms * kGZ : 0);
    for (int t = row; t < ncent * per_centre; t += nrows) {
      const int ci = t / per_centre, k = t - ci * per_centre;
      const int64_t i = c0 + ci;
      const int32_t *seg = b.seg_start + (size_t)i * (NSPEC + 1);
      double *Gi = b.G + (size_t)i * sf.ndim;
      double v = 0.0;
      if (k < n_radial_tasks) {
        const int sb = NSPEC == 1 ? 0 : k / nrad_here, kk = k - sb * nrad_here;
        const double *col = R + (size_t)kk * cap;
        for (int q = seg[sb] - s0 + l; q < seg[sb + 1] - s0; q += 16) v += col[q];
        v = row16_sum(v);
        if (l == 0) Gi[radial_term2(b.species[i], sb) * sf.n_rad + cc + kk] = v;
      } else {
        const int k2 = k - n_radial_tasks;
        const int term = k2 / kGZ, gz = k2 - term * kGZ;
        int sa = 0, sb = 0;
        for (int rem = term, len = NSPEC; rem >= len; rem -= len, --len) ++sa;
        sb = term - (sa * NSPEC - (sa * (sa - 1)) / 2) + sa;
        const int *ss = sslot + ci * kSegW;
        const double *colA = P + (size_t)(sa * kGZ + gz) * v2_pcols(cap, NSPEC);
        for (int q = ss[sb] + l; q < ss[sb + 1]; q += 16) v += colA[q];
        if (sa != sb) {
          const double *colB = P + (size_t)(sb * kGZ + gz) * v2_pcols(cap, NSPEC);
          for (int q = ss[sa] + l; q < ss[sa + 1]; q += 16) v += colB[q];
        }
        v = row16_sum(v);
        if (l == 0) Gi[sf.n_radial_dim + term * sf.n_ang + ch.chan[gz]] = v * sf.ang_scale;
      }
    }
  }
}

__device__ __forceinline__ void stagger(int flags) {
  const int n = (flags >> 8) & 0xff;
  if (n && ((blockIdx.x >> ((flags >> 16) & 31)) & 1))
    for (int k = 0; k < n; ++k) __builtin_amdgcn_s_sleep(127);
}

template <int NSPEC, int NG, int NZ, int HD, bool DEFZ, int CAP, int WPE = (DEFZ && NSPEC <= 2 ? 5 : 0)>
__global__ __launch_bounds__(kBlock)
    __attribute__((amdgpu_waves_per_eu(WPE > 0 ? WPE : 1, 8))) void g4_forward_v2_kernel(SFParams sf, AngChunk ch,
                                                               DeviceBatch b, int flags) {
  static_assert(!DEFZ || NZ == 2, "DEFZ needs the two-zeta grid");
  const int kCap = CAP > 0 ? CAP : b.cap;
  const int geom = flags & 1;
  if (b.n_blk_dev && (int)blockIdx.x >= *b.n_blk_dev) return;
  stagger(flags);
  extern __shared__ double lds[];
  const Fields f = carve(lds, kCap, true);
  const int slot = b.blk_groups > 0 ? 16 * ((int)blockIdx.x % b.blk_groups) + (int)blockIdx.x / b.blk_groups
                                    : (int)blockIdx.x;
  const int c0 = b.blk_center[slot], c1 = b.blk_center[slot + 1];
  if (c0 >= c1) return;
  const int s0 = b.pair_start[c0];
  const int M = pair_stop_of(b, c1 - 1) - s0;
  const double beta = ch.beta[0];
  if (b.job_count) {
    char *raw = reinterpret_cast<char *>(lds);
    int *cnt = reinterpret_cast<int *>(raw + v2_counter_offset(kCap));
    if (threadIdx.x < 40) cnt[threadIdx.x] = 0;
    else if (threadIdx.x < 40 + 17 && (int)threadIdx.x - 40 <= c1 - c0)
      cnt[threadIdx.x] = ((int)threadIdx.x - 40 < c1 - c0 ? b.pair_start[c0 + threadIdx.x - 40] : s0 + M) - s0;
    else if (threadIdx.x >= 64 && (int)threadIdx.x - 64 < (c1 - c0) * (NSPEC + 1)) {
      const int k = ((int)threadIdx.x - 64) / (NSPEC + 1), sg = ((int)threadIdx.x - 64) % (NSPEC + 1);
      cnt[60 + k * kSegW + sg] = b.seg_start[(size_t)(c0 + k) * (NSPEC + 1) + sg] - s0;
    }
    if (NSPEC == 1 && b.job_word_own && threadIdx.x < 20) cnt[kOwnCtl + threadIdx.x] = 0;
    double *P0 = reinterpret_cast<double *>(raw + v2_counter_offset(kCap) + kJobCtlBytes);
    for (int k = threadIdx.x; k < NSPEC * NG * NZ * v2_pcols(kCap, NSPEC); k += blockDim.x) P0[k] = 0.0;
  }
  int *jidx = (NSPEC == 1 && b.job_word_own && b.job_count) ? reinterpret_cast<int *>(f.sp1) : nullptr;
  TA_STAMP(b, 0, 0);
  stage<HD>(sf, ch, beta, b, f, s0, M, geom, true, jidx);
  TA_STAMP(b, 0, 1);
  if (b.job_count && threadIdx.x == 0) {
    int *ctl = reinterpret_cast<int *>(reinterpret_cast<char *>(lds) + v2_counter_offset(kCap));
    const int *segl = ctl + 60;
    int *sslot = ctl + 60 + kMaxCentersPerBlock * kSegW;
    int acc = 0;
    for (int k = 0; k < c1 - c0; ++k)
      for (int sg = 0; sg <= NSPEC; ++sg) {
        sslot[k * kSegW + sg] = acc;
        if (sg < NSPEC) acc += (segl[k * kSegW + sg + 1] - segl[k * kSegW + sg] + 3) >> 2;
      }
  }

  auto run_item = [&](int item, bool have_mask, unsigned long long mask0, double *out, double *pacc, auto is_job) {
    constexpr bool kJob = decltype(is_job)::value;
    const int64_t p = (int64_t)s0 + item;
    int base, n;
    int pslot = item;
    unsigned own = 0u;
    int kbit = 0;
    uint32_t sij = 0u;
    int ic = 0, rij = 0;
    if constexpr (kJob) {
      const int *cstart = reinterpret_cast<const int *>(reinterpret_cast<const char *>(lds) + v2_counter_offset(kCap)) + 40;
      const int ci = job_centre((uint32_t)mask0);
      if (NSPEC == 1 && jidx) {
        ic = c0 + ci;
        const int j = jidx[item];
        sij = (uint32_t)ic + (uint32_t)j;
        rij = j < ic ? 1 : 0;
      }
      base = cstart[ci];
      n = cstart[ci + 1] - base;
      {
        const int *segl = cstart + 20, *sslot = segl + kMaxCentersPerBlock * kSegW;
        const int sg = NSPEC == 1 ? 0 : (int)f.sp1[item];
        pslot = sslot[ci * kSegW + sg] + ((item - segl[ci * kSegW + sg]) >> 2);
      }
    } else {
      const int i = b.pair_i[p];
      base = b.pair_start[i] - s0;
      n = pair_stop_of(b, i) - b.pair_start[i];
    }
    const int a = item - base;
    const double2 axy = f.xy[item], azr = f.zr[item], aih = f.ih[item];
    const double ax = axy.x, ay = axy.y, az = azr.x;
    const double ra2 = azr.y, inv_ra = aih.x, Ha = aih.y;

    double acc[NSPEC][NG][NZ];
#pragma unroll
    for (int sp = 0; sp < NSPEC; ++sp)
#pragma unroll
      for (int ig = 0; ig < NG; ++ig)
#pragma unroll
        for (int iz = 0; iz < NZ; ++iz) acc[sp][ig][iz] = 0.0;
    double mom[NSPEC][5];
#pragma unroll
    for (int sp = 0; sp < NSPEC; ++sp)
#pragma unroll
      for (int k = 0; k < 5; ++k) mom[sp][k] = 0.0;

    auto triple = [&](int bl) {
        bl = (int)min((unsigned)bl, (unsigned)bl - (unsigned)n);
        const int q = kProbe(flags, 30) ? (int)threadIdx.x : base + bl;
        const double2 bxy = f.xy[q], bzr = f.zr[q];
        const double ex = bxy.x - ax, ey = bxy.y - ay, ez = bzr.x - az;
        const double d2 = fma(ex, ex, fma(ey, ey, fma(ez, ez, sf.eps)));
        const double u = kProbe(flags, 30) ? 0.5 : d2 * sf.inv_ac2;
        if (!(u < 1.0)) return;
        if constexpr (kJob && NSPEC == 1) {
          if (jidx) {
            const int kk = jidx[q];
            own |= (triangle_owner_rank(sij + (uint32_t)kk) == rij + (kk < ic ? 1 : 0) ? 1u : 0u) << kbit;
          }
        }
        const double2 bih = f.ih[kProbe(flags, 29) ? (int)threadIdx.x : q];
        const double cth = (ra2 + bzr.y - d2) * 0.5 * inv_ra * bih.x;
        const double common = Ha * bih.y * hd_value<HD>(sf, ch, beta, u);
        const int sb = NSPEC == 1 ? 0 : (int)f.sp1[q];
        if constexpr (DEFZ) {
          const double c2 = cth * cth;
          const double t1 = common * cth, t2 = common * c2, t3 = t1 * c2, t4 = t2 * c2;
#pragma unroll
          for (int sp = 0; sp < NSPEC; ++sp) {
            const bool on = NSPEC == 1 || sb == sp;
            mom[sp][0] += on ? common : 0.0;
            mom[sp][1] += on ? t1 : 0.0;
            mom[sp][2] += on ? t2 : 0.0;
            mom[sp][3] += on ? t3 : 0.0;
            mom[sp][4] += on ? t4 : 0.0;
          }
        } else {
#pragma unroll
          for (int ig = 0; ig < NG; ++ig) {
            const double basev = fma(ch.gamma[ig], cth, 1.0);
#pragma unroll
            for (int iz = 0; iz < NZ; ++iz) {
              double pw;
              if (ch.zeta_int[iz] > 0)
                pw = pow_int_m1(basev, ch.zeta_int[iz]) * basev;
              else
                pw = safe_pow_value(ch.safe_pow, basev, ch.zeta[iz]);
              const double v = pw * common;
#pragma unroll
              for (int sp = 0; sp < NSPEC; ++sp)
                acc[sp][ig][iz] += (NSPEC == 1 || sb == sp) ? v : 0.0;
            }
          }
        }
    };
    if constexpr (kJob) {
      const uint32_t jw = (uint32_t)mask0;
      unsigned m = (flags & (1 << 24)) ? 0u : jw >> 16;
      const int k0 = a + 1 + 16 * (int)((jw >> 8) & 3u);
      while (m) {
        const int k = __ffs((int)m) - 1;
        m &= m - 1;
        kbit = k;
        triple(k0 + k);
      }
    } else {
    const int smax = (Ha != 0.0) ? n / 2 : 0;
    for (int sc = 1; sc <= smax; sc += 64) {
      unsigned long long mask;
      if (have_mask) {
        mask = (flags & (1 << 24)) ? 0ull : mask0;
      } else {
        mask = partner_mask(sf, f, base, n, a, sc, smax);
        if (b.masks) b.masks[(size_t)(sc >> 6) * b.n_pairs + p] = mask;
      }
      while (mask) {
        const int k = __ffsll((long long)mask) - 1;
        mask &= mask - 1;
        triple(a + sc + k);
      }
    }
    }
    if constexpr (DEFZ) {
#pragma unroll
      for (int sp = 0; sp < NSPEC; ++sp)
#pragma unroll
        for (int ig = 0; ig < NG; ++ig) {
          const double g1 = ch.gamma[ig], g2 = g1 * g1;
          acc[sp][ig][0] = fma(g1, mom[sp][1], mom[sp][0]);
          acc[sp][ig][1] = fma(g2 * g2, mom[sp][4], fma(4.0 * g2 * g1, mom[sp][3],
                               fma(6.0 * g2, mom[sp][2], fma(4.0 * g1, mom[sp][1], mom[sp][0]))));
        }
    }
#pragma unroll
    for (int sp = 0; sp < NSPEC; ++sp)
#pragma unroll
      for (int ig = 0; ig < NG; ++ig)
#pragma unroll
        for (int iz = 0; iz < NZ; ++iz) {
          const int c = ch.chan[ig * NZ + iz];
          const double v = acc[sp][ig][iz] * ch.kz[iz];
          if (pacc) {
            if (v != 0.0) atomicAdd(&pacc[(size_t)((sp * NG + ig) * NZ + iz) * v2_pcols(kCap, NSPEC) + pslot], v);
          } else if (out)
            out[(sp * NG + ig) * NZ + iz] = v;
          else
            b.part4[(size_t)(sp * sf.n_ang + c) * b.n_pairs + p] = v;
        }
    return own;
  };

  int item = threadIdx.x;
  const bool active = item < M;
  int n_own = 0;
  if (active) {
    const int i = b.pair_i[s0 + item];
    n_own = pair_stop_of(b, i) - b.pair_start[i];
  }
  const bool one_pass = M <= (int)blockDim.x && !__syncthreads_or(active && (n_own >> 1) > 64);
  if (one_pass) {
    unsigned long long mask = 0ull;
    if (active) {
      const int64_t p = (int64_t)s0 + item;
      const int i = b.pair_i[p];
      const int base = b.pair_start[i] - s0;
      const int smax = (f.ih[item].y != 0.0) ? n_own / 2 : 0;
      if (smax > 0 && !(flags & (1 << 25))) mask = partner_mask(sf, f, base, n_own, item - base, 1, smax);
      if (b.masks && !b.job_count) b.masks[p] = mask;
    }
    TA_STAMP(b, 0, 2);
    if (b.job_count) {
      char *raw = reinterpret_cast<char *>(lds);
      JobLists jl = job_lists(f);
      jl.hist = reinterpret_cast<int *>(raw + v2_counter_offset(kCap));
      jl.start = jl.hist + 20;
      double *P = reinterpret_cast<double *>(raw + v2_counter_offset(kCap) + kJobCtlBytes);
      const int n_jobs = make_jobs(jl, active, item, active ? b.pair_i[s0 + item] - c0 : 0, mask);
      TA_STAMP(b, 0, 3);
      const size_t jbase = (size_t)blockIdx.x * b.job_stride;
      if (threadIdx.x == 0) b.job_count[blockIdx.x] = n_jobs;
      for (int slot = threadIdx.x; slot < n_jobs; slot += blockDim.x) b.job_word[jbase + slot] = jl.word[slot];
      TA_STAMP(b, 0, 4);
      uint32_t swept[4] = {0u, 0u, 0u, 0u};
      unsigned owned[4] = {0u, 0u, 0u, 0u};
      if (!(flags & (1 << 27)))
        for (int r = 0; r * (int)blockDim.x < n_jobs; ++r) {
          const int slot = job_slot(r, threadIdx.x, blockDim.x);
          if (slot < n_jobs) {
            const uint32_t jw = jl.word[slot];
            const unsigned o = run_item(job_item(jw), true, jw, nullptr, P, std::true_type{});
            if (r < 4) {
              swept[r] = jw;
              owned[r] = o;
            }
          }
        }
      if (jidx)
        make_owned_jobs(jl.hist + kOwnCtl, jl.hist + kOwnCtl + 20, swept, owned, b.job_word_own + jbase,
                        b.job_count_own + blockIdx.x);
      __syncthreads();
      TA_STAMP(b, 0, 5);
      if (flags & 4) {
        assemble_flat<NSPEC, NG, NZ>(sf, ch, b, f, P, jl.hist + 60 + kMaxCentersPerBlock * kSegW, c0, c1, s0, item, active,
                                     (flags & (1 << 26)) != 0, kCap);
        TA_STAMP(b, 0, 6);
        return;
      }
      if (active) {
        const int64_t p = (int64_t)s0 + threadIdx.x;
        const int ci = b.pair_i[p] - c0, sg = NSPEC == 1 ? 0 : (int)f.sp1[threadIdx.x];
        const int *segl = jl.hist + 60, *sslot = segl + kMaxCentersPerBlock * kSegW;
        const int rel = (int)threadIdx.x - segl[ci * kSegW + sg];
        const int pidx = sslot[ci * kSegW + sg] + (rel >> 2);
        const bool holds = (rel & 3) == 0;
#pragma unroll
        for (int sp = 0; sp < NSPEC; ++sp)
#pragma unroll
          for (int gz = 0; gz < NG * NZ; ++gz)
            b.part4[(size_t)(sp * sf.n_ang + ch.chan[gz]) * b.n_pairs + p] =
                holds ? P[(size_t)(sp * NG * NZ + gz) * v2_pcols(kCap, NSPEC) + pidx] : 0.0;
      }
    } else {
    deal_by_popcount(f, kCap, M, item, mask);
    constexpr int kLocal = NSPEC * NG * NZ;
    constexpr int kGZ = NG * NZ;
    constexpr int kSpPerPass = 8 / kGZ;
    if (flags & 4) {
      double mine[kLocal];
#pragma unroll
      for (int k = 0; k < kLocal; ++k) mine[k] = 0.0;
      if (active) run_item(item, true, mask, mine, nullptr, std::false_type{});
      __syncthreads();
      double *red = reinterpret_cast<double *>(f.xy);
#pragma unroll
      for (int sp_lo = 0; sp_lo < NSPEC; sp_lo += kSpPerPass) {
        const int sp_hi = sp_lo + kSpPerPass < NSPEC ? sp_lo + kSpPerPass : NSPEC;
        if (active) {
#pragma unroll
          for (int k = 0; k < kSpPerPass * kGZ; ++k)
            if (sp_lo * kGZ + k < kLocal) red[(size_t)k * kCap + item] = mine[sp_lo * kGZ + k];
        }
        __syncthreads();
        if (sp_lo == 0) reduce_radial_from_lds(sf, b, f, c0, c1, s0);
        reduce_angular_from_lds<NSPEC, NG, NZ>(sf, ch, b, red, kCap, c0, c1, s0, sp_lo, sp_hi);
        __syncthreads();
      }
      return;
    }
    if (active) run_item(item, true, mask, nullptr, nullptr, std::false_type{});
    }
  } else {
    if (b.job_count && threadIdx.x == 0) b.job_count[blockIdx.x] = -1;
    if (jidx && threadIdx.x == 0) b.job_count_own[blockIdx.x] = -1;
    for (int it = threadIdx.x; it < M; it += blockDim.x) run_item(it, false, 0ull, nullptr, nullptr, std::false_type{});
  }

  if (flags & 2) {
    __syncthreads();
    const int ncent = c1 - c0;
    const int nwaves = blockDim.x >> 6;
    if (ncent <= nwaves) {
      const int w = threadIdx.x >> 6, l = threadIdx.x & 63;
      const bool act = w < ncent;
      const int64_t i = c0 + (act ? w : 0);
      atom_descriptors<64>(sf, b, i, l, act, [&](int c, double v) { b.G[(size_t)i * sf.ndim + c] = v; });
    } else {
      const int row = threadIdx.x >> 4, l = threadIdx.x & 15, nrows = blockDim.x >> 4;
      for (int k0 = 0; k0 < ncent; k0 += nrows) {
        const bool act = k0 + row < ncent;
        const int64_t i = c0 + (act ? k0 + row : 0);
        atom_descriptors<16>(sf, b, i, l, act, [&](int c, double v) { b.G[(size_t)i * sf.ndim + c] = v; });
      }
    }
  }
}

template <int NSPEC, int NG, int NZ, int HD, bool DEFZ, int CAP, int WPE = (DEFZ ? (NSPEC <= 2 ? 5 : 4) : 0),
          bool TRI = false>
__global__ __launch_bounds__(kBlock)
    __attribute__((amdgpu_waves_per_eu(WPE > 0 ? WPE : 1, 8))) void backward_v2_kernel(SFParams sf, AngChunk ch,
                                                             DeviceBatch b, int flags) {
  static_assert(!DEFZ || NZ == 2, "DEFZ needs the two-zeta grid");
  static_assert(!TRI || (NSPEC == 1 && DEFZ && HD > 0), "the triangle build is one-element, default grid, Hd series");
  const int first = flags & 1;
  if (b.n_blk_dev && (int)blockIdx.x >= *b.n_blk_dev) return;
  stagger(flags);
  extern __shared__ double lds[];
  const int kCap = CAP > 0 ? CAP : b.cap;
  const Fields f = carve(lds, kCap);
  double *gacc = lds + kNF * kCap + kCap / 8;
  const int slot = b.blk_groups > 0 ? 16 * ((int)blockIdx.x % b.blk_groups) + (int)blockIdx.x / b.blk_groups
                                    : (int)blockIdx.x;
  const int c0 = b.blk_center[slot], c1 = b.blk_center[slot + 1];
  if (c0 >= c1) return;
  const int s0 = b.pair_start[c0];
  const int M = pair_stop_of(b, c1 - 1) - s0;
  const double beta = ch.beta[0];
  for (int k = threadIdx.x; k < 3 * kCap; k += blockDim.x) gacc[k] = 0.0;
  int *cstart = reinterpret_cast<int *>(gacc) - 20;
  if ((int)threadIdx.x <= c1 - c0 && threadIdx.x < 17)
    cstart[threadIdx.x] = ((int)threadIdx.x < c1 - c0 ? b.pair_start[c0 + threadIdx.x] : s0 + M) - s0;
  double *pctab = gacc + 3 * kCap;
  if constexpr (DEFZ && NSPEC == 1) {
    const int k = (int)blockDim.x - 1 - (int)threadIdx.x;
    if (k < c1 - c0) {
      const double *wsrc = b.dEdG + (size_t)(c0 + k) * sf.ndim + sf.n_radial_dim;
      double p0 = 0.0, p1 = 0.0, p2 = 0.0, p3 = 0.0, p4 = 0.0;
#pragma unroll
      for (int ig = 0; ig < NG; ++ig) {
        const double g1 = ch.gamma[ig], g2 = g1 * g1;
        const double w1 = wsrc[ch.chan[ig * NZ]] * ch.kz[0], w4 = wsrc[ch.chan[ig * NZ + 1]] * ch.kz[1];
        p0 += w1 + w4;
        p1 += g1 * (w1 + 4.0 * w4);
        p2 += 6.0 * g2 * w4;
        p3 += 4.0 * g2 * g1 * w4;
        p4 += g2 * g2 * w4;
      }
      pctab[5 * k] = p0;
      pctab[5 * k + 1] = 0.5 * p1;
      pctab[5 * k + 2] = 0.25 * p2;
      pctab[5 * k + 3] = 0.125 * p3;
      pctab[5 * k + 4] = 0.0625 * p4;
    }
  }
  double *rtab = pctab + 5 * kMaxCentersPerBlock;
  const bool use_rtab = first && NSPEC * sf.n_rad <= kRTab;
  if (use_rtab) {
    const int per = NSPEC * sf.n_rad;
    const int t = (int)blockDim.x - 1 - (int)threadIdx.x - kMaxCentersPerBlock;
    if (t >= 0 && t < (c1 - c0) * per) {
      const int ci = t / per, rem = t - ci * per;
      const int sb = rem / sf.n_rad, c = rem - sb * sf.n_rad;
      const int64_t i = c0 + ci;
      rtab[ci * kRTab + rem] = b.dEdG[(size_t)i * sf.ndim + radial_term2(b.species[i], sb) * sf.n_rad + c];
    }
  }
  double2 *pn01 = reinterpret_cast<double2 *>(rtab + kMaxCentersPerBlock * kRTab), *pn23 = pn01 + kCap;
  double *pn4 = reinterpret_cast<double *>(pn23 + kCap);
  if constexpr (TRI) {
    for (int item = threadIdx.x; item < M; item += blockDim.x) {
      double pc[5];
      defz_coeffs<NG, NZ>(ch, b.dEdG + (size_t)b.pair_j[s0 + item] * sf.ndim + sf.n_radial_dim, pc);
      pn01[item] = make_double2(pc[0], pc[1]);
      pn23[item] = make_double2(pc[2], pc[3]);
      pn4[item] = pc[4];
    }
  }
  TA_STAMP(b, 1, 0);
  stage<HD>(sf, ch, beta, b, f, s0, M);
  TA_STAMP(b, 1, 1);
  const int nel = sf.n_elements;

  auto run_tri = [&](int item, bool have_mask, unsigned long long mask0, auto is_job) {
    constexpr bool kJob = decltype(is_job)::value;
    const int64_t p = (int64_t)s0 + item;
    int i, base, n;
    if constexpr (kJob) {
      const int ci = job_centre((uint32_t)mask0);
      i = c0 + ci;
      base = cstart[ci];
      n = cstart[ci + 1] - base;
    } else {
      i = b.pair_i[p];
      base = b.pair_start[i] - s0;
      n = pair_stop_of(b, i) - b.pair_start[i];
    }
    const int a = item - base;
    const double2 axy = f.xy[item], azr = f.zr[item], aih = f.ih[item], ags = f.gs[item];
    const double ax = axy.x, ay = axy.y, az = azr.x;
    const double A = azr.y, inv_ra = aih.x, Ha = aih.y, La = ags.x;
    const double inv_A = inv_ra * inv_ra;
    double pi_[5], pj_[5];
#pragma unroll
    for (int k = 0; k < 5; ++k) pi_[k] = pctab[5 * (i - c0) + k];
    {
      const double2 p01 = pn01[item], p23 = pn23[item];
      pj_[0] = p01.x;
      pj_[1] = p01.y;
      pj_[2] = p23.x;
      pj_[3] = p23.y;
      pj_[4] = pn4[item];
    }
    const int ja = kJob ? 0 : b.pair_j[p];
    double csum = 0.0, gx = 0.0, gy = 0.0, gz = 0.0;
    auto tri = [&](int bl) {
      bl = (int)min((unsigned)bl, (unsigned)bl - (unsigned)n);
      const int q = base + bl;
      if constexpr (!kJob) {
        if (!owns_triangle(i, ja, b.pair_j[s0 + q])) return;
      }
      const double2 bxy = f.xy[q], bzr = f.zr[q];
      const double bx = bxy.x, by = bxy.y, bz = bzr.x;
      const double ex = bx - ax, ey = by - ay, ez = bz - az;
      const double D = fma(ex, ex, fma(ey, ey, fma(ez, ez, sf.eps)));
      const double u = D * sf.inv_ac2;
      if (!(u < 1.0)) return;
      const double2 bih = f.ih[q], bgs = f.gs[q], p01 = pn01[q], p23 = pn23[q];
      const double pk4 = pn4[q];
      const double B = bzr.y, inv_rb = bih.x, Hb = bih.y, Lb = bgs.x;
      double Hd, dHd;
      hd_eval<HD>(sf, ch, beta, u, Hd, dHd);
      const double inv_d = rsqrt_f64(D);
      const double inv_ab = inv_ra * inv_rb, inv_ad = inv_ra * inv_d, inv_bd = inv_rb * inv_d;
      const double wi = (A + B - D) * inv_ab, wj = (A + D - B) * inv_ad, wk = (B + D - A) * inv_bd;
      const double Si = fma(fma(fma(fma(pi_[4], wi, pi_[3]), wi, pi_[2]), wi, pi_[1]), wi, pi_[0]);
      const double Pi = fma(fma(fma(4.0 * pi_[4], wi, 3.0 * pi_[3]), wi, 2.0 * pi_[2]), wi, pi_[1]);
      const double Sj = fma(fma(fma(fma(pj_[4], wj, pj_[3]), wj, pj_[2]), wj, pj_[1]), wj, pj_[0]);
      const double Pj = fma(fma(fma(4.0 * pj_[4], wj, 3.0 * pj_[3]), wj, 2.0 * pj_[2]), wj, pj_[1]);
      const double Sk = fma(fma(fma(fma(pk4, wk, p23.y), wk, p23.x), wk, p01.y), wk, p01.x);
      const double Pk = fma(fma(fma(4.0 * pk4, wk, 3.0 * p23.y), wk, 2.0 * p23.x), wk, p01.y);
      const double HH = Ha * Hb, T = HH * Hd;
      const double sum = Si + Sj + Sk;
      const double TS = T * sum;
      const double X = (sum * HH) * (sf.two_inv_ac2 * dHd);
      const double Yi = Pi * T, Yj = Pj * T, Yk = Pk * T;
      const double Ywi = Yi * wi, Ywj = Yj * wj, Ywk = Yk * wk;
      const double inv_D = inv_d * inv_d;
      const double ZD = (Ywj + Ywk) * inv_D;
      const double Yjd = Yj * inv_ad, Ykd = Yk * inv_bd;
      const double ca = fma(TS, La, fma(-(Ywi + Ywj), inv_A, fma(4.0, Yjd, X - ZD)));
      const double cb = fma(TS, Lb, fma(-(Ywi + Ywk), inv_rb * inv_rb, fma(4.0, Ykd, X - ZD)));
      const double Q = fma(2.0, fma(Yi, inv_ab, -(Yjd + Ykd)), ZD - X);
      csum += ca;
      gx = fma(Q, bx, gx);
      gy = fma(Q, by, gy);
      gz = fma(Q, bz, gz);
      atomicAdd(&gacc[q], fma(cb, bx, Q * ax));
      atomicAdd(&gacc[kCap + q], fma(cb, by, Q * ay));
      atomicAdd(&gacc[2 * kCap + q], fma(cb, bz, Q * az));
    };
    if constexpr (kJob) {
      const uint32_t jw = (uint32_t)mask0;
      unsigned m = (flags & (1 << 24)) ? 0u : jw >> 16;
      const int k0 = a + 1 + 16 * (int)((jw >> 8) & 3u);
      while (m) {
        const int k = __ffs((int)m) - 1;
        m &= m - 1;
        tri(k0 + k);
      }
    } else {
      const int smax = (Ha != 0.0) ? n / 2 : 0;
      for (int sc = 1; sc <= smax; sc += 64) {
        unsigned long long mask = have_mask ? mask0 : b.masks[(size_t)(sc >> 6) * b.n_pairs + p];
        if (flags & (1 << 24)) mask = 0ull;
        while (mask) {
          const int k = __ffsll((long long)mask) - 1;
          mask &= mask - 1;
          tri(a + sc + k);
        }
      }
    }
    atomicAdd(&gacc[item], fma(csum, ax, gx));
    atomicAdd(&gacc[kCap + item], fma(csum, ay, gy));
    atomicAdd(&gacc[2 * kCap + item], fma(csum, az, gz));
  };

  auto run_item = [&](int item, bool have_mask, unsigned long long mask0, auto is_job) {
    constexpr bool kJob = decltype(is_job)::value;
    const int64_t p = (int64_t)s0 + item;
    int i, base, n;
    if constexpr (kJob) {
      const int ci = job_centre((uint32_t)mask0);
      i = c0 + ci;
      base = cstart[ci];
      n = cstart[ci + 1] - base;
    } else {
      i = b.pair_i[p];
      base = b.pair_start[i] - s0;
      n = pair_stop_of(b, i) - b.pair_start[i];
    }
    const int a = item - base;
    const double2 axy = f.xy[item], azr = f.zr[item], aih = f.ih[item], ags = f.gs[item];
    const double ax = axy.x, ay = axy.y, az = azr.x;
    const double ra2 = azr.y, inv_ra = aih.x, Ha = aih.y, La = ags.x;
    const double inv_ra2 = inv_ra * inv_ra;
    const int sa = (int)ags.y;

    constexpr bool kTable = kJob && DEFZ && NSPEC == 1;
    double w_[NSPEC][NG][NZ], wd[NSPEC][NG][NZ];
#pragma unroll
    for (int sp = 0; sp < (kTable ? 0 : NSPEC); ++sp) {
      const double *wsrc = b.dEdG + (size_t)i * sf.ndim + sf.n_radial_dim +
                           angular_term2(sa, sp, nel) * sf.n_ang;
#pragma unroll
      for (int ig = 0; ig < NG; ++ig)
#pragma unroll
        for (int iz = 0; iz < NZ; ++iz) {
          w_[sp][ig][iz] = wsrc[ch.chan[ig * NZ + iz]] * ch.kz[iz];
          wd[sp][ig][iz] = w_[sp][ig][iz] * ch.zeta[iz] * ch.gamma[ig];
        }
    }

    double pc[NSPEC][5];
    if constexpr (kTable) {
      const double *src = pctab + 5 * (i - c0);
#pragma unroll
      for (int k = 0; k < 5; ++k) pc[0][k] = src[k];
    } else if constexpr (DEFZ) {
#pragma unroll
      for (int sp = 0; sp < NSPEC; ++sp) {
#pragma unroll
        for (int k = 0; k < 5; ++k) pc[sp][k] = 0.0;
#pragma unroll
        for (int ig = 0; ig < NG; ++ig) {
          const double g1 = ch.gamma[ig], g2 = g1 * g1;
          const double w1 = w_[sp][ig][0], w4 = w_[sp][ig][1];
          pc[sp][0] += w1 + w4;
          pc[sp][1] += 0.5 * g1 * (w1 + 4.0 * w4);
          pc[sp][2] += 0.25 * 6.0 * g2 * w4;
          pc[sp][3] += 0.125 * 4.0 * g2 * g1 * w4;
          pc[sp][4] += 0.0625 * g2 * g2 * w4;
        }
      }
    }
    double csum = 0.0, gx = 0.0, gy = 0.0, gz = 0.0;
    auto triple = [&](int bl) {
        bl = (int)min((unsigned)bl, (unsigned)bl - (unsigned)n);
        const int q = kProbe(flags, 30) ? (int)threadIdx.x : base + bl;
        const double2 bxy = f.xy[q], bzr = f.zr[q];
        const double bx = bxy.x, by = bxy.y, bz = bzr.x;
        const double ex = bx - ax, ey = by - ay, ez = bz - az;
        const double d2 = fma(ex, ex, fma(ey, ey, fma(ez, ez, sf.eps)));
        const double u = kProbe(flags, 30) ? 0.5 : d2 * sf.inv_ac2;
        if (!(u < 1.0)) return;
        const int q2 = kProbe(flags, 29) ? (int)threadIdx.x : q;
        const double2 bih = f.ih[q2], bgs = f.gs[q2];
        const double inv_rb = bih.x, Hb = bih.y, Lb = bgs.x;
        const int sb = NSPEC == 1 ? 0 : (int)bgs.y;
        const double inv_ab = inv_ra * inv_rb;
        const double w = (ra2 + bzr.y - d2) * inv_ab;
        double Hd, dHd;
        hd_eval<HD>(sf, ch, beta, u, Hd, dHd);
        const double Hd2 = sf.two_inv_ac2 * dHd;
        double S0 = 0.0, Yc, Y;
        const double HH = Ha * Hb, T = HH * Hd;
        if constexpr (DEFZ) {
          double p0 = pc[0][0], p1 = pc[0][1], p2 = pc[0][2], p3 = pc[0][3], p4 = pc[0][4];
#pragma unroll
          for (int sp = 1; sp < NSPEC; ++sp) {
            p0 = (sb == sp) ? pc[sp][0] : p0;
            p1 = (sb == sp) ? pc[sp][1] : p1;
            p2 = (sb == sp) ? pc[sp][2] : p2;
            p3 = (sb == sp) ? pc[sp][3] : p3;
            p4 = (sb == sp) ? pc[sp][4] : p4;
          }
          S0 = fma(fma(fma(fma(p4, w, p3), w, p2), w, p1), w, p0);
          const double S1w = fma(fma(fma(4.0 * p4, w, 3.0 * p3), w, 2.0 * p2), w, p1);
          const double Z = S1w * T;
          Yc = Z * w;
          Y = Z + Z;
        } else {
          const double cth = 0.5 * w;
          double S1 = 0.0;
#pragma unroll
          for (int ig = 0; ig < NG; ++ig) {
            const double basev = fma(ch.gamma[ig], cth, 1.0);
#pragma unroll
            for (int iz = 0; iz < NZ; ++iz) {
              double ws = w_[0][ig][iz], wds = wd[0][ig][iz];
#pragma unroll
              for (int sp = 1; sp < NSPEC; ++sp) {
                ws = (sb == sp) ? w_[sp][ig][iz] : ws;
                wds = (sb == sp) ? wd[sp][ig][iz] : wds;
              }
              double pm1;
              if (ch.zeta_int[iz] > 0)
                pm1 = pow_int_m1(basev, ch.zeta_int[iz]);
              else
                pm1 = safe_pow_grad(ch.safe_pow, basev, ch.zeta[iz] - 1.0);
              S0 = fma(ws, pm1 * basev, S0);
              S1 = fma(wds, pm1, S1);
            }
          }
          Y = S1 * T;
          Yc = Y * cth;
        }
        const double S0T = S0 * T;
        const double X = (S0 * HH) * Hd2;
        const double ca = fma(S0T, La, fma(-Yc, inv_ra2, X));
        const double cb = fma(S0T, Lb, fma(-Yc, inv_rb * inv_rb, X));
        const double Q = fma(Y, inv_ab, -X);
        csum += ca;
        gx = fma(Q, bx, gx);
        gy = fma(Q, by, gy);
        gz = fma(Q, bz, gz);
        const int q3 = kProbe(flags, 28) ? (int)threadIdx.x : q;
        atomicAdd(&gacc[q3], fma(cb, bx, Q * ax));
        atomicAdd(&gacc[kCap + q3], fma(cb, by, Q * ay));
        atomicAdd(&gacc[2 * kCap + q3], fma(cb, bz, Q * az));
    };
    if constexpr (kJob) {
      const uint32_t jw = (uint32_t)mask0;
      unsigned m = (flags & (1 << 24)) ? 0u : jw >> 16;
      const int k0 = a + 1 + 16 * (int)((jw >> 8) & 3u);
      while (m) {
        const int k = __ffs((int)m) - 1;
        m &= m - 1;
        triple(k0 + k);
      }
    } else {
    const int smax = (Ha != 0.0) ? n / 2 : 0;
    for (int sc = 1; sc <= smax; sc += 64) {
      unsigned long long mask = have_mask ? mask0 : b.masks[(size_t)(sc >> 6) * b.n_pairs + p];
      if (flags & (1 << 24)) mask = 0ull;
      while (mask) {
        const int k = __ffsll((long long)mask) - 1;
        mask &= mask - 1;
        triple(a + sc + k);
      }
    }
    }
    atomicAdd(&gacc[item], fma(csum, ax, gx));
    atomicAdd(&gacc[kCap + item], fma(csum, ay, gy));
    atomicAdd(&gacc[2 * kCap + item], fma(csum, az, gz));
  };

  {
    int item = threadIdx.x;
    const bool active = item < M;
    int n_own = 0;
    if (active) {
      const int i = b.pair_i[s0 + item];
      n_own = pair_stop_of(b, i) - b.pair_start[i];
    }
    const bool one_pass = M <= (int)blockDim.x && !__syncthreads_or(active && (n_own >> 1) > 64);
    const int32_t *jcount = TRI ? b.job_count_own : b.job_count;
    const uint32_t *jword = TRI ? b.job_word_own : b.job_word;
    const int n_jobs = (one_pass && jcount) ? jcount[blockIdx.x] : -1;
    if (n_jobs >= 0) {
      const size_t jbase = (size_t)blockIdx.x * b.job_stride;
      uint32_t jws[4];
#pragma unroll
      for (int r = 0; r < 4; ++r) {
        const int slot = job_slot(r, threadIdx.x, blockDim.x);
        jws[r] = slot < n_jobs ? jword[jbase + slot] : 0u;
      }
      TA_STAMP(b, 1, 2);
#pragma unroll
      for (int r = 0; r < 4; ++r) {
        if (r * (int)blockDim.x >= n_jobs) break;
        const int slot = job_slot(r, threadIdx.x, blockDim.x);
        if (slot < n_jobs) {
          if constexpr (TRI) run_tri(job_item(jws[r]), true, jws[r], std::true_type{});
          else run_item(job_item(jws[r]), true, jws[r], std::true_type{});
        }
      }
      TA_STAMP(b, 1, 3);
    } else if (one_pass) {
      unsigned long long mask = 0ull;
      if (active) {
        const int64_t p = (int64_t)s0 + item;
        const int smax = (f.ih[item].y != 0.0) ? n_own / 2 : 0;
        if (smax > 0) mask = b.masks[p];
      }
      if (active) {
        if constexpr (TRI) run_tri(item, true, mask, std::false_type{});
        else run_item(item, true, mask, std::false_type{});
      }
    } else {
      for (int it = threadIdx.x; it < M; it += blockDim.x) {
        if constexpr (TRI) run_tri(it, false, 0ull, std::false_type{});
        else run_item(it, false, 0ull, std::false_type{});
      }
    }
  }
  __syncthreads();
  TA_STAMP(b, 1, 4);
  for (int item = threadIdx.x; item < M; item += blockDim.x) {
    const int64_t p = (int64_t)s0 + item;
    double gx = gacc[item], gy = gacc[kCap + item], gz = gacc[2 * kCap + item];
    if (first) {
      const double *wr;
      if (use_rtab) {
        int ci = 0;
        for (int k = 1; k < c1 - c0; ++k) ci += (item >= cstart[k]) ? 1 : 0;
        wr = rtab + ci * kRTab + (NSPEC == 1 ? 0 : (int)f.gs[item].y * sf.n_rad);
      } else {
        const int i = b.pair_i[p];
        wr = b.dEdG + (size_t)i * sf.ndim + radial_term2(b.species[i], (int)f.gs[item].y) * sf.n_rad;
      }
      const double r2 = f.zr[item].y, inv_r = f.ih[item].x;
      const double ur = r2 * sf.inv_rc2;
      double s = 0.0;
      if (ur < 1.0) {
        double fc, dfdu;
        cutoff_u(sf.cutoff, ur, fc, dfdu);
        const double r = r2 * inv_r;
        const double dfdr = dfdu * 2.0 * r * sf.inv_rc2;
        double e = 0.0;
        for (int c = 0; c < sf.n_rad; ++c) {
          const double dr = r - sf.omega[c];
          const int pw = sf.eta_pow[c];
          e = pw > 0 ? pow_int_m1(e, pw) * e : ta_exp(-sf.eta[c] * dr * dr * sf.inv_rc2);
          s = fma(wr[c], e * (dfdr - 2.0 * sf.eta[c] * dr * fc * sf.inv_rc2), s);
        }
      }
      s *= inv_r;
      gx = fma(s, f.xy[item].x, gx);
      gy = fma(s, f.xy[item].y, gy);
      gz = fma(s, f.zr[item].x, gz);
    } else {
      gx += b.g[4 * (size_t)p];
      gy += b.g[4 * (size_t)p + 1];
      gz += b.g[4 * (size_t)p + 2];
    }
    b.g[4 * (size_t)p] = gx;
    b.g[4 * (size_t)p + 1] = gy;
    b.g[4 * (size_t)p + 2] = gz;
  }
  TA_STAMP(b, 1, 5);
}

template <int NSPEC, int NG, int NZ>
void fwd_t(const SFParams &sf, const AngChunk &ch, const DeviceBatch &b, int geom, int wpe, hipStream_t s) {
  const dim3 grid((unsigned)b.n_blk), block((unsigned)(b.cap < kBlock ? b.cap : kBlock));
  const size_t lds = v2_lds_bytes(false, b.cap, b.job_count ? NSPEC * NG * NZ : 0, NSPEC);
  if constexpr (NZ == 2) {
    if (ch.n_hd == 12 && ch.zeta_int[0] == 1 && ch.zeta_int[1] == 4) {
      if (b.cap == kCapMin) {
        if constexpr (NSPEC <= 2) {
          if (wpe != 5) {
            hipLaunchKernelGGL((g4_forward_v2_kernel<NSPEC, NG, NZ, 12, true, kCapMin, 6>), grid, block, lds, s, sf, ch,
                               b, geom);
            return;
          }
        }
        hipLaunchKernelGGL((g4_forward_v2_kernel<NSPEC, NG, NZ, 12, true, kCapMin>), grid, block, lds, s, sf, ch, b, geom);
      } else
        hipLaunchKernelGGL((g4_forward_v2_kernel<NSPEC, NG, NZ, 12, true, 0>), grid, block, lds, s, sf, ch, b, geom);
      return;
    }
    if (ch.n_hd == 16 && ch.zeta_int[0] == 1 && ch.zeta_int[1] == 4) {
      hipLaunchKernelGGL((g4_forward_v2_kernel<NSPEC, NG, NZ, 16, true, 0>), grid, block, lds, s, sf, ch, b, geom);
      return;
    }
  }
  if (ch.n_hd > 0 && ch.n_hd <= 16)
    hipLaunchKernelGGL((g4_forward_v2_kernel<NSPEC, NG, NZ, 16, false, 0>), grid, block, lds, s, sf, ch, b, geom);
  else if (ch.n_hd == 24)
    hipLaunchKernelGGL((g4_forward_v2_kernel<NSPEC, NG, NZ, 24, false, 0>), grid, block, lds, s, sf, ch, b, geom);
  else
    hipLaunchKernelGGL((g4_forward_v2_kernel<NSPEC, NG, NZ, 0, false, 0>), grid, block, lds, s, sf, ch, b, geom);
}
template <int NSPEC, int NG, int NZ>
void bwd_t(const SFParams &sf, const AngChunk &ch, const DeviceBatch &b, int first, bool tri, int wpe, int &variant,
           hipStream_t s) {
  const dim3 grid((unsigned)b.n_blk), block((unsigned)(b.cap < kBlock ? b.cap : kBlock));
  const size_t lds = v2_lds_bytes(true, b.cap);
  variant = 1;
  if constexpr (NZ == 2 && NSPEC == 1) {
    if (tri && (ch.n_hd == 12 || ch.n_hd == 16) && ch.zeta_int[0] == 1 && ch.zeta_int[1] == 4) {
      const size_t lds_t = v2_lds_bytes(true, b.cap, 0, 0, true);
      variant = 2;
      if (ch.n_hd == 12 && b.cap == kCapMin && wpe == 4)
        hipLaunchKernelGGL((backward_v2_kernel<1, NG, NZ, 12, true, kCapMin, 4, true>), grid, block, lds_t, s, sf, ch,
                           b, first);
      else if (ch.n_hd == 12 && b.cap == kCapMin)
        hipLaunchKernelGGL((backward_v2_kernel<1, NG, NZ, 12, true, kCapMin, 5, true>), grid, block, lds_t, s, sf, ch,
                           b, first);
      else if (ch.n_hd == 12)
        hipLaunchKernelGGL((backward_v2_kernel<1, NG, NZ, 12, true, 0, 5, true>), grid, block, lds_t, s, sf, ch, b,
                           first);
      else
        hipLaunchKernelGGL((backward_v2_kernel<1, NG, NZ, 16, true, 0, 5, true>), grid, block, lds_t, s, sf, ch, b,
                           first);
      return;
    }
  }
  if constexpr (NZ == 2) {
    if (ch.n_hd == 12 && ch.zeta_int[0] == 1 && ch.zeta_int[1] == 4) {
      if (b.cap == kCapMin) {
        if constexpr (NSPEC == 1) {
          if (wpe == 6) {
            hipLaunchKernelGGL((backward_v2_kernel<NSPEC, NG, NZ, 12, true, kCapMin, 6>), grid, block, lds, s, sf, ch,
                               b, first);
            return;
          }
        }
        hipLaunchKernelGGL((backward_v2_kernel<NSPEC, NG, NZ, 12, true, kCapMin>), grid, block, lds, s, sf, ch, b, first);
      } else
        hipLaunchKernelGGL((backward_v2_kernel<NSPEC, NG, NZ, 12, true, 0>), grid, block, lds, s, sf, ch, b, first);
      return;
    }
    if (ch.n_hd == 16 && ch.zeta_int[0] == 1 && ch.zeta_int[1] == 4) {
      hipLaunchKernelGGL((backward_v2_kernel<NSPEC, NG, NZ, 16, true, 0>), grid, block, lds, s, sf, ch, b, first);
      return;
    }
  }
  if (ch.n_hd > 0 && ch.n_hd <= 16)
    hipLaunchKernelGGL((backward_v2_kernel<NSPEC, NG, NZ, 16, false, 0>), grid, block, lds, s, sf, ch, b, first);
  else if (ch.n_hd == 24)
    hipLaunchKernelGGL((backward_v2_kernel<NSPEC, NG, NZ, 24, false, 0>), grid, block, lds, s, sf, ch, b, first);
  else
    hipLaunchKernelGGL((backward_v2_kernel<NSPEC, NG, NZ, 0, false, 0>), grid, block, lds, s, sf, ch, b, first);
}

}

size_t v2_lds_bytes(bool backward, int cap, int n_local, int nspec, bool triangles) {
  if (!backward && n_local > 0)
    return v2_counter_offset(cap) + kJobCtlBytes + (size_t)n_local * v2_pcols(cap, nspec) * sizeof(double);
  if (backward)
    return (size_t)cap * kNF * sizeof(double) + cap + 3 * (size_t)cap * sizeof(double) +
           kMaxCentersPerBlock * (5 + kRTab) * sizeof(double) + (triangles ? 5 * (size_t)cap * sizeof(double) : 0);
  return (size_t)cap * kNF * sizeof(double) + 3 * (size_t)(2 * cap + kRingPad) * sizeof(float) + cap;
}
int v2_job_stride(int cap) { return v2_max_jobs(cap); }

#ifdef TA_V2_FEW
#define TA_DISPATCH_V2(FN, ...)                                   \
  do {                                                            \
    const int key = nspec * 100 + ng * 10 + nz;                   \
    if (key == 122) FN<1, 2, 2>(__VA_ARGS__);                     \
    else if (key == 222) FN<2, 2, 2>(__VA_ARGS__);                \
    else throw std::domain_error("TA_V2_FEW build");              \
  } while (0)
#else
#define TA_DISPATCH_V2(FN, ...)                                   \
  do {                                                            \
    const int key = nspec * 100 + ng * 10 + nz;                   \
    switch (key) {                                                \
      case 111: FN<1, 1, 1>(__VA_ARGS__); break;                  \
      case 112: FN<1, 1, 2>(__VA_ARGS__); break;                  \
      case 121: FN<1, 2, 1>(__VA_ARGS__); break;                  \
      case 122: FN<1, 2, 2>(__VA_ARGS__); break;                  \
      case 211: FN<2, 1, 1>(__VA_ARGS__); break;                  \
      case 212: FN<2, 1, 2>(__VA_ARGS__); break;                  \
      case 221: FN<2, 2, 1>(__VA_ARGS__); break;                  \
      case 222: FN<2, 2, 2>(__VA_ARGS__); break;                  \
      case 311: FN<3, 1, 1>(__VA_ARGS__); break;                  \
      case 312: FN<3, 1, 2>(__VA_ARGS__); break;                  \
      case 321: FN<3, 2, 1>(__VA_ARGS__); break;                  \
      case 322: FN<3, 2, 2>(__VA_ARGS__); break;                  \
      case 422: FN<4, 2, 2>(__VA_ARGS__); break;                  \
      case 522: FN<5, 2, 2>(__VA_ARGS__); break;                  \
      default:                                                    \
        throw std::domain_error("no second-generation angular kernel for this (species, gamma, zeta) shape"); \
    }                                                             \
  } while (0)
#endif

static int stagger_bits(const Options &opt, bool backward) {
#ifdef TA_PROBE_SWITCHES
  if (opt.debug_no_triples) return 1 << 24;
  if (opt.debug_skip >= 0) return opt.debug_skip << 24;
  return backward ? opt.stagger_bwd : opt.stagger_fwd;
#else
  (void)opt;
  (void)backward;
  return 0;
#endif
}

void launch_g4_forward_v2(const SFParams &sf, const AngChunk &ch, int ng, int nz, bool geometry,
                          bool reduce, const DeviceBatch &b, const Options &opt, hipStream_t s) {
  if (b.n_blk == 0) return;
  const int nspec = sf.n_elements;
  const int geom = (geometry ? 1 : 0) | (reduce ? 2 : 0) | ((geometry && reduce) ? 4 : 0) |
                   stagger_bits(opt, false);
  TA_DISPATCH_V2(fwd_t, sf, ch, b, geom, opt.fwd_wpe, s);
}

int launch_backward_v2(const SFParams &sf, const AngChunk &ch, int ng, int nz, bool first, bool triangles,
                       const DeviceBatch &b, const Options &opt, hipStream_t s) {
  if (b.n_blk == 0) return 0;
  const int nspec = sf.n_elements;
  const int f = (first ? 1 : 0) | stagger_bits(opt, true);
  int variant = 0;
  TA_DISPATCH_V2(bwd_t, sf, ch, b, f, triangles, opt.bwd_wpe, variant, s);
  return variant;
}

}
```

### tensoralloy_amd/csrc/ta_nlist.hip

```cpp
#include <hip/hip_runtime.h>

#include <cmath>
#include <stdexcept>
#include <vector>

#include "ta_device.h"
#include "ta_internal.h"

namespace ta {
namespace {

constexpr int kBlock = 256;

__global__ __launch_bounds__(kBlock) void bin_atoms_kernel(int n_atoms, const double *pos,
                                                           const int32_t *frame_of_atom,
                                                           const NlGrid *grids, int32_t *wrap,
                                                           int32_t *binid, int32_t *bin_count,
                                                           int32_t *slot_in_bin, unsigned long long *clear,
                                                           int n_clear) {
  const int i = blockIdx.x * kBlock + threadIdx.x;
  for (int k = i; k < n_clear; k += gridDim.x * kBlock) clear[k] = 0ull;
  if (i >= n_atoms) return;
  const NlGrid &g = grids[frame_of_atom[i]];
  const double *r = pos + 3 * (size_t)i;
// ... 298 lines not shown
    int run = incl - sum;
    for (int w = 0; w < wave; ++w) run += wtot[w];
    for (int k = lo; k < hi; ++k) {
      start[k] = run;
      run += bin_count[k];
    }
    if (t == kBlock - 1) start[n_bins] = run;
    __syncthreads();
    if (blockIdx.x == 0)
      for (int k = t; k <= n_bins; k += kBlock) bin_start[k] = start[k];
  }
  const int i = blockIdx.x * kBlock + threadIdx.x;
  if (i >= n_atoms) return;
  NlRec r;
  r.x = pos[3 * (size_t)i];
  r.y = pos[3 * (size_t)i + 1];
  r.z = pos[3 * (size_t)i + 2];
  r.wx = wrap[3 * (size_t)i];
  r.wy = wrap[3 * (size_t)i + 1];
  r.wz = wrap[3 * (size_t)i + 2];
  r.j = i;
  r.sp = species[i];
  r.pad_ = 0;
  const int first = SCAN ? start[binid[i]] : bin_start[binid[i]];
  recs[first + slot_in_bin[i]] = r;
}

__global__ __launch_bounds__(64 * kBuildGroup) void build_pairs_kernel(
    int n_atoms, int nel, double rmax, const double *pos, const int32_t *frame_of_atom, const NlGrid *grids,
    const int32_t *wrap, const int32_t *binid, const int32_t *bin_start, const NlRec *recs, int32_t *bin_count,
    int n_bins, unsigned long long *gstate, long long capacity, int32_t *seg_start, int32_t *pair_start,
    int32_t *host_pair_start, int32_t *pair_i, int32_t *pair_j, int32_t *pair_shift,
    unsigned long long *stats) {
  __shared__ unsigned long long stash[kBuildGroup][kBuildStash];
  __shared__ unsigned short rank16[kBuildGroup][kBuildStash];
  __shared__ int cnt[kBuildGroup], cstart[kBuildGroup];
  __shared__ long long s_base;
  __shared__ int s_write;
  const int w = threadIdx.x >> 6, lane = threadIdx.x & 63;
  const int i = __builtin_amdgcn_readfirstlane(blockIdx.x * kBuildGroup + w);
  const bool act = i < n_atoms;
  for (int k = blockIdx.x * 64 * kBuildGroup + threadIdx.x; k <= n_bins; k += gridDim.x * 64 * kBuildGroup)
    bin_count[k] = 0;
  unsigned long long *mine = stash[w];
  int n = 0;
  bool bad = false;
  if (act) {
    const NlGrid &g = grids[__builtin_amdgcn_readfirstlane(frame_of_atom[i])];
    const int local = binid[i] - g.bin_offset;
    const int bz = local % g.nb[2], by = (local / g.nb[2]) % g.nb[1], bx = local / (g.nb[2] * g.nb[1]);
    const double rix = pos[3 * (size_t)i], riy = pos[3 * (size_t)i + 1], riz = pos[3 * (size_t)i + 2];
    const int wix = wrap[3 * (size_t)i], wiy = wrap[3 * (size_t)i + 1], wiz = wrap[3 * (size_t)i + 2];
    const double rmax2 = rmax * rmax;
    const int e0 = 2 * g.m[0] + 1, e1 = 2 * g.m[1] + 1, e2 = 2 * g.m[2] + 1;
    const int n_combo = e0 * e1 * e2;
    constexpr int kSelf = 0x888;
    const int own[3] = {bx, by, bz};
    double inbin[3];
#pragma unroll
    for (int a = 0; a < 3; ++a) {
      double fa = rix * g.hinv[0 * 3 + a] + riy * g.hinv[1 * 3 + a] + riz * g.hinv[2 * 3 + a];
      if (g.pbc[a]) fa -= floor(fa);
      const double t = (fa - g.lo[a]) * g.inv_w[a] - own[a];
      inbin[a] = t < 0.0 ? 0.0 : (t > 1.0 ? 1.0 : t);
    }
    for (int c0 = 0; c0 < n_combo; c0 += 27) {
      int lo = 0, len = 0, code = kSelf;
      if (lane < 27 && c0 + lane < n_combo) {
        const int id = c0 + lane;
        const int d[3] = {id / (e1 * e2) - g.m[0], (id / e2) % e1 - g.m[1], id % e2 - g.m[2]};
        int c[3] = {bx + d[0], by + d[1], bz + d[2]};
        int sh[3] = {0, 0, 0};
        bool ok = true;
        {
          double far2 = 0.0, far1 = 0.0;
#pragma unroll
          for (int a = 0; a < 3; ++a) {
            const double gap = d[a] == 0 ? 0.0 : ((d[a] < 0 ? -d[a] - 1 + inbin[a] : d[a] - inbin[a]) * g.bw[a]);
            far2 = fma(gap, gap, far2);
            far1 = gap > far1 ? gap : far1;
          }
          const double lim = rmax * (1.0 + 1e-9);
          if (g.ortho ? far2 > lim * lim : far1 > lim) ok = false;
        }
#pragma unroll
        for (int a = 0; a < 3; ++a) {
          if (c[a] < 0 || c[a] >= g.nb[a]) {
            if (!g.pbc[a]) ok = false;
            sh[a] = c[a] >= 0 ? c[a] / g.nb[a] : -((-c[a] + g.nb[a] - 1) / g.nb[a]);
            c[a] -= sh[a] * g.nb[a];
          }
        }
        if (ok) {
          const int bin = g.bin_offset + (c[0] * g.nb[1] + c[1]) * g.nb[2] + c[2];
          lo = bin_start[bin];
          len = bin_start[bin + 1] - lo;
          code = (sh[0] + 8) | ((sh[1] + 8) << 4) | ((sh[2] + 8) << 8);
        }
      }
      int incl = len;
#pragma unroll
      for (int off = 1; off < 32; off <<= 1) {
        const int v = __shfl_up(incl, off);
        if (lane >= off) incl += v;
      }
      const int excl = incl - len;
      const int total = __builtin_amdgcn_readlane(incl, 26);
      const int delta = lo - excl;
      for (int base = 0; base < total; base += 64) {
        const int f = base + lane;
        int k = 0;
#pragma unroll
        for (int q = 1; q < 27; ++q) k += f >= __builtin_amdgcn_readlane(excl, q);
        const int dl = __shfl(delta, k);
        const int cd = __shfl(code, k);
        bool valid = false;
        unsigned long long key = 0;
        if (f < total) {
          const NlRec r = recs[dl + f];
          const int Sx = (cd & 15) - 8 - r.wx + wix, Sy = ((cd >> 4) & 15) - 8 - r.wy + wiy,
                    Sz = ((cd >> 8) & 15) - 8 - r.wz + wiz;
          const double Dx = r.x - rix + (Sx * g.h[0] + Sy * g.h[3] + Sz * g.h[6]);
          const double Dy = r.y - riy + (Sx * g.h[1] + Sy * g.h[4] + Sz * g.h[7]);
          const double Dz = r.z - riz + (Sx * g.h[2] + Sy * g.h[5] + Sz * g.h[8]);
          const double r2 = Dx * Dx + Dy * Dy + Dz * Dz;
          valid = r2 < rmax2 * (1.0 - 1e-14) || (r2 <= rmax2 * (1.0 + 1e-14) && sqrt(r2) < rmax);
          valid = valid && !(r.j == i && cd == kSelf);
          if (valid) {
            if (abs(Sx) >= kShiftBias || abs(Sy) >= kShiftBias || abs(Sz) >= kShiftBias) bad = true;
            key = nl_key(r.sp, r.j, Sx, Sy, Sz);
          }
        }
        const unsigned long long m = __ballot(valid);
        const int at = n + __popcll(m & ((1ull << lane) - 1ull));
        if (valid && at < kBuildStash) mine[at] = key;
        n += __popcll(m);
      }
    }
    if (n > kBuildStash) bad = true;
    bad = __any(bad);
  }
  const int nn = bad ? 0 : n;
  if (lane == 0) cnt[w] = nn;
  __syncthreads();

  if (w == 0) {
    const int c = lane < kBuildGroup ? cnt[lane] : 0;
    int incl = c;
#pragma unroll
    for (int off = 1; off < kBuildGroup; off <<= 1) {
      const int v = __shfl_up(incl, off);
      if (lane >= off) incl += v;
    }
    if (lane < kBuildGroup) cstart[lane] = incl - c;
    {
      unsigned long long tri = (unsigned long long)c * (unsigned long long)(c > 0 ? c - 1 : 0) / 2ull;
      int mx = c;
#pragma unroll
      for (int off = 1; off < kBuildGroup; off <<= 1) {
        tri += __shfl_xor(tri, off);
        mx = max(mx, __shfl_xor(mx, off));
      }
      if (lane == 0) {
        if (tri) atomicAdd(stats, tri);
        if (mx) atomicMax(reinterpret_cast<int32_t *>(stats) + 2, mx);
      }
    }
    const unsigned long long total = (unsigned long long)__builtin_amdgcn_readlane(incl, kBuildGroup - 1);
    const int gi = blockIdx.x;
    if (lane == 0)
      __hip_atomic_store(&gstate[gi], (gi == 0 ? kStatePrefix : kStateSum) | total, __ATOMIC_RELAXED,
                         __HIP_MEMORY_SCOPE_AGENT);
    unsigned long long before = 0;
    bool gave_up = false;
    int spins = 0;
    for (int hi = gi - 1; hi >= 0;) {
      const int k = hi - lane;
      const unsigned long long v =
          k >= 0 ? __hip_atomic_load(&gstate[k], __ATOMIC_RELAXED, __HIP_MEMORY_SCOPE_AGENT) : kStatePrefix;
      const unsigned fl = (unsigned)(v >> 62);
      const unsigned long long m_prefix = __ballot(fl == 2), m_empty = __ballot(fl == 0);
      const int first = m_prefix ? __builtin_ctzll(m_prefix) : 63;
      const unsigned long long need = first >= 63 ? ~0ull : ((2ull << first) - 1ull);
      if (m_empty & need) {
        if (++spins > kSpinLimit) {
          gave_up = true;
          break;
        }
        __builtin_amdgcn_s_sleep(4);
        continue;
      }
      unsigned long long part = lane <= first ? (v & kStateMask) : 0ull;
#pragma unroll
      for (int off = 32; off; off >>= 1) part += __shfl_xor(part, off);
      before += part;
      if (m_prefix) break;
      hi -= 64;
    }
    if (lane == 0) {
      if (gi > 0)
        __hip_atomic_store(&gstate[gi], kStatePrefix | ((before + total) & kStateMask), __ATOMIC_RELAXED,
                           __HIP_MEMORY_SCOPE_AGENT);
      s_base = (long long)before;
      s_write = !gave_up && (long long)(before + total) <= capacity;
      if (gave_up) atomicOr(reinterpret_cast<int32_t *>(stats) + 3, 1);
      const int last = min(gi * kBuildGroup + kBuildGroup, n_atoms);
      if (last == n_atoms) {
        const unsigned long long all = before + total;
        pair_start[n_atoms] = (int32_t)all;
        if (host_pair_start) host_pair_start[n_atoms] = (int32_t)all;
        seg_start[(size_t)n_atoms * (nel + 1)] = (int32_t)all;
        stats[4] = all;
      }
    }
  }
  for (int e = lane; e < nn; e += 64) {
    const unsigned long long key = mine[e];
    int r = 0;
#pragma unroll 4
    for (int k = 0; k < nn; ++k) r += mine[k] < key;
    rank16[w][e] = (unsigned short)r;
  }
  if (act && __any(bad) && lane == 0) atomicOr(reinterpret_cast<int32_t *>(stats) + 3, 1);
  __syncthreads();
  if (!act) return;
  const long long at = s_base + cstart[w];
  int segc = 0;
  for (int e0 = 0; e0 < nn; e0 += 64) {
    const int e = e0 + lane;
    const int sp = e < nn ? (int)(mine[e] >> 61) : -1;
    for (int s = 0; s < nel; ++s) {
      const int c = __popcll(__ballot(sp == s));
      if (lane == s) segc += c;
    }
  }
  int incl = segc;
#pragma unroll
  for (int off = 1; off <= kMaxElements; off <<= 1) {
    const int v = __shfl_up(incl, off);
    if (lane >= off) incl += v;
  }
  if (lane <= nel) seg_start[(size_t)i * (nel + 1) + lane] = (int32_t)(at + incl - segc);
  if (lane == 0) {
    pair_start[i] = (int32_t)at;
    if (host_pair_start) host_pair_start[i] = (int32_t)at;
  }
  if (!s_write) return;
  for (int e = lane; e < nn; e += 64) {
    const unsigned long long key = mine[e];
    const long long slot = at + rank16[w][e];
    pair_i[slot] = i;
    pair_j[slot] = (int32_t)((key >> 30) & 0x7fffffffull);
    pair_shift[3 * slot] = (int)((key >> 20) & 1023) - kShiftBias;
    pair_shift[3 * slot + 1] = (int)((key >> 10) & 1023) - kShiftBias;
    pair_shift[3 * slot + 2] = (int)(key & 1023) - kShiftBias;
  }
}

__global__ __launch_bounds__(kBlock) void reverse_sorted_kernel(int64_t n_pairs, int nel,
                                                                const unsigned long long *n_dev, int64_t capacity,
                                                                const int32_t *species,
                                                                const int32_t *seg_start,
                                                                const int32_t *pair_i, const int32_t *pair_j,
                                                                const int32_t *pair_shift, int32_t *pair_rev,
                                                                int32_t *n_missing) {
  const int64_t p = (int64_t)blockIdx.x * kBlock + threadIdx.x;
  if (n_dev) {
    const unsigned long long n = *n_dev;
    if (n > (unsigned long long)capacity) return;
    n_pairs = (int64_t)n < n_pairs ? (int64_t)n : n_pairs;
  }
  if (p >= n_pairs) return;
  const int i = pair_i[p], j = pair_j[p];
  const int sx = pair_shift[3 * p], sy = pair_shift[3 * p + 1], sz = pair_shift[3 * p + 2];
  const int32_t *seg = seg_start + (size_t)j * (nel + 1);
  const int si = species[i];
  int lo = seg[si];
  const int end = seg[si + 1];
  int hi = end;
  while (lo < hi) {
    const int mid = (lo + hi) >> 1;
    if (pair_j[mid] < i) lo = mid + 1;
    else hi = mid;
  }
  int found = -1;
  for (int q = lo; q < end && pair_j[q] == i; ++q)
    if (pair_shift[3 * (size_t)q] == -sx && pair_shift[3 * (size_t)q + 1] == -sy &&
        pair_shift[3 * (size_t)q + 2] == -sz) {
      found = q;
      break;
    }
  pair_rev[p] = found;
  if (found < 0) atomicAdd(n_missing, 1);
}

constexpr int kFilterGroup = 16;
constexpr int kFilterMaxEl = 8;
static_assert(kFilterGroup == kMaxCentersPerBlock, "a run of the angular kernels never crosses a group");

__global__ __launch_bounds__(64 * kFilterGroup) void filter_group_kernel(
    int n_atoms, int nel, double rmax, const double *pos, const double *cells,
    const int32_t *frame_of_atom, const int32_t *start_super, const int32_t *seg_super, const int32_t *pj_super,
    const int32_t *ps_super, int32_t *seg_exact, int32_t *pair_start, int32_t *pair_stop, int32_t *pi_out,
    int32_t *pj_out, int32_t *ps_out, int32_t *map, int32_t *slot_q, int cap, int32_t *blk_center) {
  __shared__ int cnt[kFilterGroup][kFilterMaxEl + 1];
  const int w = threadIdx.x >> 6, lane = threadIdx.x & 63;
  const int i0 = blockIdx.x * kFilterGroup;
  const int i = i0 + w;
  const bool act = i < n_atoms;
  double h[9] = {0, 0, 0, 0, 0, 0, 0, 0, 0}, ri[3] = {0, 0, 0};
  const int32_t *seg = seg_super + (size_t)(act ? i : 0) * (nel + 1);
  if (act) {
    const double *hc = cells + 9 * (size_t)frame_of_atom[i];
#pragma unroll
    for (int k = 0; k < 9; ++k) h[k] = hc[k];
#pragma unroll
    for (int k = 0; k < 3; ++k) ri[k] = pos[3 * (size_t)i + k];
  }
  auto probe = [&](int q, int &j, int (&S)[3], double (&D)[3]) {
    j = pj_super[q];
#pragma unroll
    for (int c = 0; c < 3; ++c) S[c] = ps_super[3 * (size_t)q + c];
#pragma unroll
    for (int c = 0; c < 3; ++c)
      D[c] = pos[3 * (size_t)j + c] - ri[c] + (S[0] * h[c] + S[1] * h[3 + c] + S[2] * h[6 + c]);
    return sqrt(D[0] * D[0] + D[1] * D[1] + D[2] * D[2]) < rmax;
  };
  for (int s = 0; s < nel && act; ++s) {
    int running = 0;
    for (int q0 = seg[s]; q0 < seg[s + 1]; q0 += 64) {
      const int q = q0 + lane;
      bool valid = false;
      if (q < seg[s + 1]) {
        int j, S[3];
        double D[3];
        valid = probe(q, j, S, D);
      }
      running += __popcll(__ballot(valid));
    }
    if (lane == 0) cnt[w][s] = running;
  }
  if (!act && lane < nel) cnt[w][lane] = 0;
  __syncthreads();
  if (blk_center && threadIdx.x == 0) {
    int slot = i0, load = 0, nc = 0;
    const int iend = min(i0 + kFilterGroup, n_atoms);
    for (int k = 0; k < kFilterGroup && i0 + k < n_atoms; ++k) {
      int n = 0;
      for (int s = 0; s < nel; ++s) n += cnt[k][s];
      if (k == 0 || load + n > cap || nc >= kMaxCentersPerBlock) {
        blk_center[slot++] = i0 + k;
        load = 0;
        nc = 0;
      }
      load += n;
      ++nc;
    }
    for (; slot < i0 + kFilterGroup; ++slot) blk_center[slot] = iend;
    if (iend == n_atoms) blk_center[i0 + kFilterGroup] = n_atoms;
  }
  if (!act) return;
  int off = start_super[i0];
  for (int k = 0; k < w; ++k)
    for (int s = 0; s < nel; ++s) off += cnt[k][s];
  int32_t *sx = seg_exact + (size_t)i * (nel + 1);
  {
    int o = off;
    for (int s = 0; s < nel; ++s) {
      if (lane == 0) sx[s] = o;
      o += cnt[w][s];
    }
    if (lane == 0) {
      sx[nel] = o;
      pair_start[i] = off;
      pair_stop[i] = o;
    }
  }
  for (int s = 0; s < nel; ++s) {
    int running = off;
    off += cnt[w][s];
    for (int q0 = seg[s]; q0 < seg[s + 1]; q0 += 64) {
      const int q = q0 + lane;
      bool valid = false;
      int j = 0, S[3] = {0, 0, 0};
      double D[3] = {0, 0, 0};
      if (q < seg[s + 1]) valid = probe(q, j, S, D);
      const unsigned long long m = __ballot(valid);
      if (q < seg[s + 1]) {
        int slot = -1;
        if (valid) {
          slot = running + __popcll(m & ((1ull << lane) - 1ull));
          pi_out[slot] = i;
          pj_out[slot] = j;
#pragma unroll
          for (int c = 0; c < 3; ++c) ps_out[3 * (size_t)slot + c] = S[c];
          if (slot_q) slot_q[slot] = q;
        }
        map[q] = slot;
      }
      running += __popcll(m);
    }
  }
}

__global__ __launch_bounds__(kBlock) void filter_rev_kernel(int64_t n_super, const int32_t *rev_super,
                                                            const int32_t *map, int32_t *rev_out) {
  const int64_t q = (int64_t)blockIdx.x * kBlock + threadIdx.x;
  if (q >= n_super) return;
  const int slot = map[q];
  if (slot >= 0) rev_out[slot] = map[rev_super[q]];
}

inline unsigned nblk(int64_t n, int per) { return (unsigned)((n + per - 1) / per); }

}

bool nl_make_grid(const ta_frame &fr, double rmax, int bin_offset, NlGrid &g) {
  for (int k = 0; k < 9; ++k) g.h[k] = fr.cell[k];
  auto norm = [](const double *a) { return std::sqrt(a[0] * a[0] + a[1] * a[1] + a[2] * a[2]); };
  auto cross = [](const double *a, const double *b, double *c) {
    c[0] = a[1] * b[2] - a[2] * b[1];
    c[1] = a[2] * b[0] - a[0] * b[2];
    c[2] = a[0] * b[1] - a[1] * b[0];
  };
  for (int a = 0; a < 3; ++a)
    if (g.h[3 * a] == 0.0 && g.h[3 * a + 1] == 0.0 && g.h[3 * a + 2] == 0.0) return false;
  double c0[3], c1[3], c2[3];
  cross(&g.h[3], &g.h[6], c0);
  cross(&g.h[6], &g.h[0], c1);
  cross(&g.h[0], &g.h[3], c2);
  const double det = g.h[0] * c0[0] + g.h[1] * c0[1] + g.h[2] * c0[2];
  if (det == 0.0 || !std::isfinite(det)) return false;
  for (int a = 0; a < 3; ++a) {
    g.hinv[3 * a + 0] = c0[a] / det;
    g.hinv[3 * a + 1] = c1[a] / det;
    g.hinv[3 * a + 2] = c2[a] / det;
  }
  const double vol = std::fabs(det);
  const double *cr[3] = {c0, c1, c2};
  for (int a = 0; a < 3; ++a) {
    g.pbc[a] = fr.pbc[a] != 0;
    const double height = vol / norm(cr[a]);
    const double wfrac = rmax / height;
    g.m[a] = 1;
    if (g.pbc[a]) {
      const int nb = (int)std::floor(1.0 / wfrac);
      if (nb < 1) {
        const int m = (int)std::floor(rmax / height) + 1;
        if (m > 7) return false;
        g.m[a] = m;
      }
      g.nb[a] = std::max(1, std::min(nb, 64));
      g.lo[a] = 0.0;
      g.inv_w[a] = (double)g.nb[a];
    } else {
      double mn = 1e300, mx = -1e300;
      for (int i = 0; i < fr.n_atoms; ++i) {
        const double *r = &fr.positions[3 * (size_t)i];
        const double f = r[0] * g.hinv[0 * 3 + a] + r[1] * g.hinv[1 * 3 + a] + r[2] * g.hinv[2 * 3 + a];
        if (!std::isfinite(f)) return false;
        mn = std::min(mn, f);
        mx = std::max(mx, f);
      }
      if (fr.n_atoms == 0) mn = mx = 0.0;
      const double ext = mx - mn;
      int nb = (ext > 0 && wfrac > 0) ? (int)std::floor(ext / wfrac) : 1;
      nb = std::max(1, std::min(nb, 64));
      g.nb[a] = nb;
      g.lo[a] = mn;
      g.inv_w[a] = ext > 0 ? nb / ext : 0.0;
    }
  }
  for (int a = 0; a < 3; ++a) {
    const double height = vol / norm(cr[a]);
    g.bw[a] = g.inv_w[a] > 0.0 ? height / g.inv_w[a] : 0.0;
  }
  auto dot = [&](int a, int b) { return g.h[3 * a] * g.h[3 * b] + g.h[3 * a + 1] * g.h[3 * b + 1] + g.h[3 * a + 2] * g.h[3 * b + 2]; };
  g.ortho = 1;
  for (int a = 0; a < 3; ++a)
    for (int b = a + 1; b < 3; ++b)
      if (std::fabs(dot(a, b)) > 1e-12 * std::sqrt(dot(a, a) * dot(b, b))) g.ortho = 0;
  g.bin_offset = bin_offset;
  return true;
}

int nl_bins(const NlGrid &g) { return g.nb[0] * g.nb[1] * g.nb[2]; }

void nl_count(int n_atoms, int n_bins, int nel, double rmax, const double *pos, const int32_t *species,
              const int32_t *frame_of_atom, const NlGrid *grids, NlWork &w, int32_t *pair_start,
              hipStream_t s) {
  (void)hipMemsetAsync(w.bin_count, 0, (size_t)(n_bins + 1) * sizeof(int32_t), s);
  (void)hipMemsetAsync(w.bin_cursor, 0, (size_t)(n_bins + 1) * sizeof(int32_t), s);
  (void)hipMemsetAsync(w.stats, 0, 8 * sizeof(unsigned long long), s);
  if (n_atoms == 0) return;
  hipLaunchKernelGGL(bin_atoms_kernel, dim3(nblk(n_atoms, kBlock)), dim3(kBlock), 0, s, n_atoms, pos,
                     frame_of_atom, grids, w.wrap, w.binid, w.bin_count, (int32_t *)nullptr, (unsigned long long *)nullptr, 0);
  hipLaunchKernelGGL(scan_kernel, dim3(1), dim3(1024), 0, s, n_bins, w.bin_count, w.bin_start,
                     (int32_t *)nullptr);
  hipLaunchKernelGGL(fill_bins_kernel, dim3(nblk(n_atoms, kBlock)), dim3(kBlock), 0, s, n_atoms,
                     w.binid, w.bin_start, w.bin_cursor, w.bin_atoms);
  hipLaunchKernelGGL(gather_bins_kernel, dim3(nblk(n_atoms, kBlock)), dim3(kBlock), 0, s, n_atoms,
                     pos, species, w.wrap, w.binid, w.bin_start, w.bin_atoms, w.recs);
  hipLaunchKernelGGL(pairs_kernel<0>, dim3(nblk((int64_t)n_atoms * 64, kBlock)), dim3(kBlock), 0, s,
                     n_atoms, nel, rmax, pos, frame_of_atom, grids, w.wrap, w.binid, w.bin_start,
                     w.recs, w.counts, (const int32_t *)nullptr, (int32_t *)nullptr,
                     (int32_t *)nullptr, (int32_t *)nullptr);
  hipLaunchKernelGGL(scan_kernel, dim3(1), dim3(1024), 0, s, n_atoms * (nel + 1), w.counts,
                     w.seg_start, reinterpret_cast<int32_t *>(w.stats) + 4);
  hipLaunchKernelGGL(finish_starts_kernel, dim3(nblk(n_atoms + 1, kBlock)), dim3(kBlock), 0, s,
                     n_atoms, nel, w.seg_start, w.counts, pair_start, w.stats,
                     reinterpret_cast<int32_t *>(w.stats) + 2, w.stats + 4);
}

void nl_fill(int n_atoms, int64_t n_pairs, int nel, double rmax, const double *pos,
             const int32_t *species, const int32_t *frame_of_atom, const NlGrid *grids, NlWork &w,
             int32_t *pair_i, int32_t *pair_j, int32_t *pair_shift, int32_t *pair_rev,
             hipStream_t s) {
  if (n_atoms == 0) return;
  hipLaunchKernelGGL(pairs_kernel<1>, dim3(nblk((int64_t)n_atoms * 64, kBlock)), dim3(kBlock), 0, s,
                     n_atoms, nel, rmax, pos, frame_of_atom, grids, w.wrap, w.binid, w.bin_start,
                     w.recs, (int32_t *)nullptr, w.seg_start, pair_i, pair_j, pair_shift);
  if (n_pairs > 0)
    hipLaunchKernelGGL(reverse_pairs_kernel, dim3(nblk(n_pairs * 8, kBlock)), dim3(kBlock), 0, s, n_pairs,
                       nel, species, w.seg_start, pair_i, pair_j, pair_shift, pair_rev,
                       reinterpret_cast<int32_t *>(w.stats) + 6);
}

size_t nl_build_zero_words(int n_atoms, int n_bins) {
  return 8 + (size_t)nblk(n_atoms, kBuildGroup) + 1 + ((size_t)n_bins + 2 + 1) / 2;
}

void nl_build(int n_atoms, int n_bins, int nel, double rmax, const double *pos, const int32_t *species,
              const int32_t *frame_of_atom, const NlGrid *grids, NlWork &w, unsigned long long *zero,
              bool zero_is_clean, long long capacity, int32_t *pair_start, int32_t *host_pair_start,
              int32_t *pair_i, int32_t *pair_j, int32_t *pair_shift, int32_t *pair_rev, long long rev_cover,
              hipStream_t s) {
  const size_t n_groups = nblk(n_atoms, kBuildGroup);
  if (!zero_is_clean)
    (void)hipMemsetAsync(zero, 0, nl_build_zero_words(n_atoms, n_bins) * sizeof(unsigned long long), s);
  w.stats = zero;
  unsigned long long *gstate = zero + 8;
  w.bin_count = reinterpret_cast<int32_t *>(zero + 8 + n_groups + 1);
  if (n_atoms == 0) return;
  hipLaunchKernelGGL(bin_atoms_kernel, dim3(nblk(n_atoms, kBlock)), dim3(kBlock), 0, s, n_atoms, pos,
                     frame_of_atom, grids, w.wrap, w.binid, w.bin_count, w.bin_atoms, zero,
                     (int)(8 + n_groups + 1));
  if (n_bins <= kPlaceScanBins) {
    hipLaunchKernelGGL(place_recs_kernel<true>, dim3(nblk(n_atoms, kBlock)), dim3(kBlock), 0, s, n_atoms, n_bins,
                       pos, species, w.wrap, w.binid, w.bin_count, w.bin_start, w.bin_atoms, w.recs);
  } else {
    hipLaunchKernelGGL(scan_kernel, dim3(1), dim3(1024), 0, s, n_bins, w.bin_count, w.bin_start,
                       (int32_t *)nullptr);
    hipLaunchKernelGGL(place_recs_kernel<false>, dim3(nblk(n_atoms, kBlock)), dim3(kBlock), 0, s, n_atoms, n_bins,
                       pos, species, w.wrap, w.binid, w.bin_count, w.bin_start, w.bin_atoms, w.recs);
  }
  hipLaunchKernelGGL(build_pairs_kernel, dim3(n_groups), dim3(64 * kBuildGroup), 0, s, n_atoms, nel, rmax,
                     pos, frame_of_atom, grids, w.wrap, w.binid, w.bin_start, w.recs, w.bin_count, n_bins, gstate,
                     capacity, w.seg_start, pair_start, host_pair_start, pair_i, pair_j, pair_shift, zero);
  if (pair_rev && rev_cover > 0)
    hipLaunchKernelGGL(reverse_sorted_kernel, dim3(nblk(rev_cover, kBlock)), dim3(kBlock), 0, s, (int64_t)rev_cover, nel,
                       zero + 4, (int64_t)capacity, species, w.seg_start, pair_i, pair_j, pair_shift, pair_rev,
                       reinterpret_cast<int32_t *>(zero) + 6);
}

void nl_reverse_sorted(int64_t n_pairs, int nel, const int32_t *species, const int32_t *seg_start,
                       const int32_t *pair_i, const int32_t *pair_j, const int32_t *pair_shift,
                       int32_t *pair_rev, unsigned long long *stats, hipStream_t s) {
  if (n_pairs > 0)
    hipLaunchKernelGGL(reverse_sorted_kernel, dim3(nblk(n_pairs, kBlock)), dim3(kBlock), 0, s, n_pairs, nel,
                       (const unsigned long long *)nullptr, (int64_t)0, species, seg_start, pair_i, pair_j, pair_shift,
                       pair_rev,
                       reinterpret_cast<int32_t *>(stats) + 6);
}

int nl_filter_blocks(int n_atoms) { return (int)nblk(n_atoms, kFilterGroup) * kFilterGroup; }

void nl_filter(int n_atoms, int64_t n_super, int nel, double rmax, const double *pos, const double *cells,
               const int32_t *frame_of_atom, const int32_t *start_super, const int32_t *seg_super,
               const int32_t *pj_super, const int32_t *ps_super, const int32_t *rev_super, int32_t *map,
               int32_t *seg_exact, int32_t *pair_start, int32_t *pair_stop, int32_t *pi_out, int32_t *pj_out,
               int32_t *ps_out, int32_t *rev_out, int32_t *slot_q, int cap, int32_t *blk_center, hipStream_t s) {
  if (n_atoms == 0) return;
  if (nel > kFilterMaxEl) throw std::domain_error("the MD-step list filter handles at most 8 elements");
  hipLaunchKernelGGL(filter_group_kernel, dim3(nblk(n_atoms, kFilterGroup)), dim3(64 * kFilterGroup), 0, s, n_atoms,
                     nel, rmax, pos, cells, frame_of_atom, start_super, seg_super, pj_super, ps_super, seg_exact,
                     pair_start, pair_stop, pi_out, pj_out, ps_out, map, slot_q, cap, blk_center);
  if (n_super > 0 && !slot_q)
    hipLaunchKernelGGL(filter_rev_kernel, dim3(nblk(n_super, kBlock)), dim3(kBlock), 0, s, n_super, rev_super, map,
                       rev_out);
}

}
```

Baseline: 37.00 million.

## Precompute per-block 64-byte headers with centre offsets for SF-MLP kernels

Adds a 64-byte BlockHeader per run slot holding the first centre, centre count, first pair index, total pairs, 16-bit per-centre offsets and a precomputed one-pass flag. Headers are built on the host during upload and on the device in the filter kernel. The descriptor and gradient kernels load the header with wide loads into scalar registers and find each item's centre from the offsets. This replaces the per-item gathers of pair_i, pair_start and pair_stop and a block-wide reduction, and job words are prefetched before staging. The cost is extra header construction, more staged bytes, and wave-level sync in the filter kernel that must be correct.

```diff
diff --git a/tensoralloy_amd/csrc/ta_api.hip b/tensoralloy_amd/csrc/ta_api.hip
--- a/tensoralloy_amd/csrc/ta_api.hip
+++ b/tensoralloy_amd/csrc/ta_api.hip
@@ -294,6 +294,7 @@
   size_t o_pos = 0, o_cells = 0, o_species = 0;
   DevBuf<int32_t> ex_pair_i, ex_pair_j, ex_pair_shift, ex_pair_rev, ex_pair_start, ex_pair_stop, ex_seg_start, ex_counts,
       ex_map, ex_blk, ex_slot_q;
+  DevBuf<ta::BlockHeader> ex_hdr;
   bool filtered = false;
   bool upload_pending = false;
   bool mirror_next = false;
@@ -1104,6 +1105,7 @@
   for (auto *b : {&h->ex_pair_i, &h->ex_pair_j, &h->ex_pair_shift, &h->ex_pair_rev, &h->ex_pair_start, &h->ex_pair_stop,
                   &h->ex_seg_start, &h->ex_counts, &h->ex_map, &h->ex_blk, &h->ex_slot_q})
     b->release();
+  h->ex_hdr.release();
   h->masks.release(); h->job_word.release(); h->job_count.release();
   h->job_word_own.release(); h->job_count_own.release();
   for (auto *b : {&h->nl_wrap, &h->nl_binid, &h->nl_bin_count, &h->nl_bin_start, &h->nl_bin_cursor,
@@ -1178,6 +1180,7 @@
   h->ex_map.ensure(P + 1);
   const int n_run_slots = nl_filter_blocks((int)N);
   h->ex_blk.ensure((size_t)n_run_slots + 4);
+  h->ex_hdr.ensure((size_t)n_run_slots + 1);
   const bool blocks = h->kind == TA_MODEL_SF_MLP;
   const bool indirect = blocks && !h->opt.filter_rev_kernel;
   if (indirect) h->ex_slot_q.ensure(P + 1);
@@ -1185,7 +1188,7 @@
             h->pair_start.ptr, h->seg_start.ptr, h->pair_j.ptr, h->pair_shift.ptr, h->pair_rev.ptr, h->ex_map.ptr,
             h->ex_seg_start.ptr, h->ex_pair_start.ptr, h->ex_pair_stop.ptr, h->ex_pair_i.ptr, h->ex_pair_j.ptr,
             h->ex_pair_shift.ptr, h->ex_pair_rev.ptr, indirect ? h->ex_slot_q.ptr : nullptr, h->db.cap,
-            blocks ? h->ex_blk.ptr : nullptr, h->stream);
+            blocks ? h->ex_blk.ptr : nullptr, blocks ? h->ex_hdr.ptr : nullptr, h->stream);
   h->db.slot_q = indirect ? h->ex_slot_q.ptr : nullptr;
   h->db.rev_super = indirect ? h->pair_rev.ptr : nullptr;
   h->db.rev_map = indirect ? h->ex_map.ptr : nullptr;
@@ -1199,6 +1202,7 @@
   h->db.pair_rev = h->ex_pair_rev.ptr;
   if (blocks) {
     h->db.blk_center = h->ex_blk.ptr;
+    h->db.blk_hdr = h->ex_hdr.ptr;
     h->db.n_blk = n_run_slots;
     h->db.blk_groups = n_run_slots / 16;
     h->db.n_blk_dev = nullptr;
@@ -1260,7 +1264,8 @@
   const size_t o_astart = align16(o_foa + N * sizeof(int32_t));
   const size_t o_elem = align16(o_astart + (F + 1) * sizeof(int32_t));
   const size_t o_blk = align16(o_elem + N * sizeof(int32_t));
-  const size_t total = align16(o_blk + (N + 2) * sizeof(int32_t));
+  auto align64 = [](size_t x) { return (x + 63) & ~(size_t)63; };
+  const size_t total = align64(o_blk + (N + 2) * sizeof(int32_t)) + (N + 1) * sizeof(ta::BlockHeader);
   h->stage_in.ensure(total);
   h->inbuf.ensure(total);
   char *hb = h->stage_in.ptr;
@@ -1368,13 +1373,22 @@
     h->db.n_blk = nb ? nb - 1 : 0;
     h->res_n_blk = h->db.n_blk;
     h->o_blk = o_blk;
+    const size_t o_hdr = align64(o_blk + (size_t)nb * sizeof(int32_t));
+    ta::BlockHeader *hdr = reinterpret_cast<ta::BlockHeader *>(hb + o_hdr);
+    const int block = std::min(cap, 256);
+    for (int r = 0; r < h->db.n_blk; ++r) {
+      const int32_t *ps = h->hp.pair_start.data() + blk[r];
+      ta::make_block_header(hdr[r], blk[r], blk[r + 1] - blk[r], ps[0], block, [&](int k) { return ps[k + 1] - ps[k]; });
+    }
+    h->db.blk_hdr = reinterpret_cast<const ta::BlockHeader *>(db_ + o_hdr);
     ensure_job_lists(h, (size_t)h->db.n_blk);
     if (nb) {
+      const size_t bytes = o_hdr + (size_t)h->db.n_blk * sizeof(ta::BlockHeader) - o_blk;
       if (list_done)
-        staged_copy(reinterpret_cast<double *>(db_ + o_blk), reinterpret_cast<const double *>(blk), ((size_t)nb + 1) / 2,
+        staged_copy(reinterpret_cast<double *>(db_ + o_blk), reinterpret_cast<const double *>(blk), bytes / sizeof(double),
                     false, h->opt, h->stream);
       else
-        HIP_CHECK(hipMemcpyAsync(db_ + o_blk, blk, (size_t)nb * sizeof(int32_t), hipMemcpyHostToDevice, h->stream));
+        HIP_CHECK(hipMemcpyAsync(db_ + o_blk, blk, bytes, hipMemcpyHostToDevice, h->stream));
     }
   }
   if (h->kind == TA_MODEL_SF_MLP) {
diff --git a/tensoralloy_amd/csrc/ta_device.h b/tensoralloy_amd/csrc/ta_device.h
--- a/tensoralloy_amd/csrc/ta_device.h
+++ b/tensoralloy_amd/csrc/ta_device.h
@@ -50,6 +50,8 @@
   double hd[kMaxHd];
 };
 
+struct BlockHeader;
+
 struct DeviceBatch {
   int64_t n_atoms = 0, n_pairs = 0;
   int n_frames = 0, nnl_max = 0;
@@ -64,6 +66,7 @@
   int32_t *pair_i = nullptr, *pair_j = nullptr, *pair_shift = nullptr, *pair_rev = nullptr;
   const int32_t *slot_q = nullptr, *rev_super = nullptr, *rev_map = nullptr;
   int32_t *blk_center = nullptr;
+  const BlockHeader *blk_hdr = nullptr;
   int n_blk = 0;
   int blk_groups = 0;
   const int32_t *n_blk_dev = nullptr;
@@ -97,6 +100,35 @@
   double *batch_energy = nullptr;
 };
 
+struct alignas(64) BlockHeader {
+  int32_t c0;
+  int32_t info;
+  int32_t s0;
+  int32_t M;
+  uint16_t rel[24];
+};
+static_assert(sizeof(BlockHeader) == 64, "one 64-byte record per run slot");
+static_assert(kMaxCentersPerBlock + 1 <= 24 && kCapMax < (1 << 16), "16-bit entries, one per centre and the end");
+constexpr int32_t kHdrOnePass = 1 << 8;
+
+template <class CountFn>
+__host__ __device__ inline void make_block_header(BlockHeader &h, int c0, int ncent, int s0, int block, CountFn count) {
+  int m = 0;
+  bool wide = false;
+  for (int k = 0; k < 24; ++k) {
+    h.rel[k] = (uint16_t)m;
+    if (k < ncent) {
+      const int n = count(k);
+      wide = wide || (n >> 1) > 64;
+      m += n;
+    }
+  }
+  h.c0 = c0;
+  h.s0 = s0;
+  h.M = m;
+  h.info = ncent | ((ncent > 0 && m <= block && !wide) ? kHdrOnePass : 0);
+}
+
 __host__ __device__ inline int triangle_owner_rank(uint32_t index_sum) {
 #ifdef __HIP_DEVICE_COMPILE__
   const uint32_t h = __umul24(index_sum, 0x9E3779u);
@@ -221,7 +253,8 @@
                const int32_t *frame_of_atom, const int32_t *start_super, const int32_t *seg_super,
                const int32_t *pj_super, const int32_t *ps_super, const int32_t *rev_super, int32_t *map,
                int32_t *seg_exact, int32_t *pair_start, int32_t *pair_stop, int32_t *pi_out, int32_t *pj_out,
-               int32_t *ps_out, int32_t *rev_out, int32_t *slot_q, int cap, int32_t *blk_center, hipStream_t s);
+               int32_t *ps_out, int32_t *rev_out, int32_t *slot_q, int cap, int32_t *blk_center, BlockHeader *blk_hdr,
+               hipStream_t s);
 void nl_fill(int n_atoms, int64_t n_pairs, int nel, double rmax, const double *pos,
              const int32_t *species, const int32_t *frame_of_atom, const NlGrid *grids, NlWork &w,
              int32_t *pair_i, int32_t *pair_j, int32_t *pair_shift, int32_t *pair_rev, hipStream_t s);
diff --git a/tensoralloy_amd/csrc/ta_kernels_v2.hip b/tensoralloy_amd/csrc/ta_kernels_v2.hip
--- a/tensoralloy_amd/csrc/ta_kernels_v2.hip
+++ b/tensoralloy_amd/csrc/ta_kernels_v2.hip
@@ -39,6 +39,52 @@
 #else
 #define TA_STAMP(b, kernel, k) do {} while (0)
 #endif
+
+struct HeaderRegs {
+  int c0, ncent, s0, M;
+  bool one_pass;
+  uint32_t rel2[12];
+};
+__device__ __forceinline__ HeaderRegs load_header(const BlockHeader *hp, bool with_rel = true) {
+  const uint4 *src = reinterpret_cast<const uint4 *>(hp);
+  const uint4 zero = make_uint4(0u, 0u, 0u, 0u);
+  const uint4 w0 = src[0], w1 = with_rel ? src[1] : zero, w2 = with_rel ? src[2] : zero, w3 = with_rel ? src[3] : zero;
+  auto sc = [](uint32_t v) { return (uint32_t)__builtin_amdgcn_readfirstlane((int)v); };
+  HeaderRegs h;
+  h.c0 = (int)sc(w0.x);
+  const int info = (int)sc(w0.y);
+  h.ncent = info & 255;
+  h.one_pass = (info & kHdrOnePass) != 0;
+  h.s0 = (int)sc(w0.z);
+  h.M = (int)sc(w0.w);
+  h.rel2[0] = sc(w1.x); h.rel2[1] = sc(w1.y); h.rel2[2] = sc(w1.z); h.rel2[3] = sc(w1.w);
+  h.rel2[4] = sc(w2.x); h.rel2[5] = sc(w2.y); h.rel2[6] = sc(w2.z); h.rel2[7] = sc(w2.w);
+  h.rel2[8] = sc(w3.x); h.rel2[9] = sc(w3.y); h.rel2[10] = sc(w3.z); h.rel2[11] = sc(w3.w);
+  return h;
+}
+__device__ __forceinline__ int header_rel(const HeaderRegs &h, int k) {
+  return (int)((h.rel2[k >> 1] >> (16 * (k & 1))) & 0xffffu);
+}
+__device__ __forceinline__ void centre_of(const HeaderRegs &h, int item, int &ci, int &base, int &n) {
+  ci = 0;
+  base = 0;
+  int end = header_rel(h, 1);
+#pragma unroll
+  for (int k = 1; k < kMaxCentersPerBlock; ++k) {
+    const bool ge = item >= header_rel(h, k);
+    ci += ge ? 1 : 0;
+    base = ge ? header_rel(h, k) : base;
+    end = ge ? header_rel(h, k + 1) : end;
+  }
+  n = end - base;
+}
+
+__device__ __forceinline__ void centre_of_lds(const int *cstart, int ncent, int item, int &ci, int &base, int &n) {
+  ci = 0;
+  for (int k = 1; k < ncent; ++k) ci += (item >= cstart[k]) ? 1 : 0;
+  base = cstart[ci];
+  n = cstart[ci + 1] - base;
+}
 
 __device__ __forceinline__ int angular_term2(int s1, int s2, int nel) {
   int a = s1 < s2 ? s1 : s2, b = s1 < s2 ? s2 : s1;
@@ -102,13 +148,19 @@
 
 template <int HD>
 __device__ __forceinline__ void stage(const SFParams &sf, const AngChunk &ch, double beta, const DeviceBatch &b,
-                                      const Fields &f, int s0, int M, int geom = 0, bool forward = false,
-                                      int *jidx = nullptr) {
+                                      const Fields &f, const HeaderRegs &hd, bool one_el, int geom = 0,
+                                      bool forward = false, int *jidx = nullptr) {
+  const int s0 = hd.s0, M = hd.M;
   for (int item = threadIdx.x; item < M; item += blockDim.x) {
     double2 v0, v1, v2;
+    int ci = 0, cbase = 0, cn = 0;
+    if (geom || forward) centre_of(hd, item, ci, cbase, cn);
+    const bool want_j = geom || jidx || !one_el;
+    const int j = want_j ? b.pair_j[s0 + item] : 0;
+    const double spj = one_el ? 0.0 : (double)b.species[j];
     if (geom) {
       const int64_t p = (int64_t)s0 + item;
-      const int i = b.pair_i[p], j = b.pair_j[p];
+      const int i = hd.c0 + ci;
       const double *h = b.cells + 9 * (size_t)b.frame_of_atom[i];
       const double sx = (double)b.pair_shift[3 * p], sy = (double)b.pair_shift[3 * p + 1],
                    sz = (double)b.pair_shift[3 * p + 2];
@@ -145,8 +197,6 @@
     f.xy[item] = v0;
     f.zr[item] = v1;
     if (forward) {
-      const int ci = b.pair_i[s0 + item];
-      const int cbase = b.pair_start[ci] - s0, cn = pair_stop_of(b, ci) - b.pair_start[ci];
       const int k0 = 2 * cbase + (item - cbase);
       f.xf[k0] = f.xf[k0 + cn] = (float)v0.x;
       f.yf[k0] = f.yf[k0 + cn] = (float)v0.y;
@@ -164,9 +214,9 @@
       }
     }
     f.ih[item] = make_double2(v2.x, H);
-    if (jidx) jidx[item] = b.pair_j[s0 + item];
-    else if (forward) f.sp1[item] = (double)b.species[b.pair_j[s0 + item]];
-    else f.gs[item] = make_double2(L, (double)b.species[b.pair_j[s0 + item]]);
+    if (jidx) jidx[item] = j;
+    else if (forward) f.sp1[item] = spj;
+    else f.gs[item] = make_double2(L, spj);
   }
   __syncthreads();
 }
@@ -514,20 +564,22 @@
   const Fields f = carve(lds, kCap, true);
   const int slot = b.blk_groups > 0 ? 16 * ((int)blockIdx.x % b.blk_groups) + (int)blockIdx.x / b.blk_groups
                                     : (int)blockIdx.x;
-  const int c0 = b.blk_center[slot], c1 = b.blk_center[slot + 1];
-  if (c0 >= c1) return;
-  const int s0 = b.pair_start[c0];
-  const int M = pair_stop_of(b, c1 - 1) - s0;
+  const BlockHeader *hp = b.blk_hdr + slot;
+  const HeaderRegs hd = load_header(hp);
+  if (hd.ncent == 0) return;
+  const int c0 = hd.c0, c1 = hd.c0 + hd.ncent;
+  const int s0 = hd.s0, M = hd.M;
   const double beta = ch.beta[0];
+  int *const cstart_w = reinterpret_cast<int *>(reinterpret_cast<char *>(lds) + v2_counter_offset(kCap)) + 40;
+  if (threadIdx.x >= 40 && threadIdx.x < 40 + 17) cstart_w[threadIdx.x - 40] = hp->rel[threadIdx.x - 40];
   if (b.job_count) {
     char *raw = reinterpret_cast<char *>(lds);
     int *cnt = reinterpret_cast<int *>(raw + v2_counter_offset(kCap));
     if (threadIdx.x < 40) cnt[threadIdx.x] = 0;
-    else if (threadIdx.x < 40 + 17 && (int)threadIdx.x - 40 <= c1 - c0)
-      cnt[threadIdx.x] = ((int)threadIdx.x - 40 < c1 - c0 ? b.pair_start[c0 + threadIdx.x - 40] : s0 + M) - s0;
     else if (threadIdx.x >= 64 && (int)threadIdx.x - 64 < (c1 - c0) * (NSPEC + 1)) {
       const int k = ((int)threadIdx.x - 64) / (NSPEC + 1), sg = ((int)threadIdx.x - 64) % (NSPEC + 1);
-      cnt[60 + k * kSegW + sg] = b.seg_start[(size_t)(c0 + k) * (NSPEC + 1) + sg] - s0;
+      cnt[60 + k * kSegW + sg] = NSPEC == 1 ? (int)hp->rel[k + sg]
+                                            : b.seg_start[(size_t)(c0 + k) * (NSPEC + 1) + sg] - s0;
     }
     if (NSPEC == 1 && b.job_word_own && threadIdx.x < 20) cnt[kOwnCtl + threadIdx.x] = 0;
     double *P0 = reinterpret_cast<double *>(raw + v2_counter_offset(kCap) + kJobCtlBytes);
@@ -535,7 +587,7 @@
   }
   int *jidx = (NSPEC == 1 && b.job_word_own && b.job_count) ? reinterpret_cast<int *>(f.sp1) : nullptr;
   TA_STAMP(b, 0, 0);
-  stage<HD>(sf, ch, beta, b, f, s0, M, geom, true, jidx);
+  stage<HD>(sf, ch, beta, b, f, hd, NSPEC == 1, geom, true, jidx);
   TA_STAMP(b, 0, 1);
   if (b.job_count && threadIdx.x == 0) {
     int *ctl = reinterpret_cast<int *>(reinterpret_cast<char *>(lds) + v2_counter_offset(kCap));
@@ -575,9 +627,8 @@
         pslot = sslot[ci * kSegW + sg] + ((item - segl[ci * kSegW + sg]) >> 2);
       }
     } else {
-      const int i = b.pair_i[p];
-      base = b.pair_start[i] - s0;
-      n = pair_stop_of(b, i) - b.pair_start[i];
+      int ci;
+      centre_of_lds(cstart_w, c1 - c0, item, ci, base, n);
     }
     const int a = item - base;
     const double2 axy = f.xy[item], azr = f.zr[item], aih = f.ih[item];
@@ -704,18 +755,14 @@
 
   int item = threadIdx.x;
   const bool active = item < M;
-  int n_own = 0;
-  if (active) {
-    const int i = b.pair_i[s0 + item];
-    n_own = pair_stop_of(b, i) - b.pair_start[i];
-  }
-  const bool one_pass = M <= (int)blockDim.x && !__syncthreads_or(active && (n_own >> 1) > 64);
+  int ci_own = 0, base_own = 0, n_own = 0;
+  if (active) centre_of(hd, item, ci_own, base_own, n_own);
+  const bool one_pass = hd.one_pass;
   if (one_pass) {
     unsigned long long mask = 0ull;
     if (active) {
       const int64_t p = (int64_t)s0 + item;
-      const int i = b.pair_i[p];
-      const int base = b.pair_start[i] - s0;
+      const int base = base_own;
       const int smax = (f.ih[item].y != 0.0) ? n_own / 2 : 0;
       if (smax > 0 && !(flags & (1 << 25))) mask = partner_mask(sf, f, base, n_own, item - base, 1, smax);
       if (b.masks && !b.job_count) b.masks[p] = mask;
@@ -727,7 +774,7 @@
       jl.hist = reinterpret_cast<int *>(raw + v2_counter_offset(kCap));
       jl.start = jl.hist + 20;
       double *P = reinterpret_cast<double *>(raw + v2_counter_offset(kCap) + kJobCtlBytes);
-      const int n_jobs = make_jobs(jl, active, item, active ? b.pair_i[s0 + item] - c0 : 0, mask);
+      const int n_jobs = make_jobs(jl, active, item, ci_own, mask);
       TA_STAMP(b, 0, 3);
       const size_t jbase = (size_t)blockIdx.x * b.job_stride;
       if (threadIdx.x == 0) b.job_count[blockIdx.x] = n_jobs;
@@ -760,7 +807,7 @@
       }
       if (active) {
         const int64_t p = (int64_t)s0 + threadIdx.x;
-        const int ci = b.pair_i[p] - c0, sg = NSPEC == 1 ? 0 : (int)f.sp1[threadIdx.x];
+        const int ci = ci_own, sg = NSPEC == 1 ? 0 : (int)f.sp1[threadIdx.x];
         const int *segl = jl.hist + 60, *sslot = segl + kMaxCentersPerBlock * kSegW;
         const int rel = (int)threadIdx.x - segl[ci * kSegW + sg];
         const int pidx = sslot[ci * kSegW + sg] + (rel >> 2);
@@ -843,15 +890,15 @@
   double *gacc = lds + kNF * kCap + kCap / 8;
   const int slot = b.blk_groups > 0 ? 16 * ((int)blockIdx.x % b.blk_groups) + (int)blockIdx.x / b.blk_groups
                                     : (int)blockIdx.x;
-  const int c0 = b.blk_center[slot], c1 = b.blk_center[slot + 1];
-  if (c0 >= c1) return;
-  const int s0 = b.pair_start[c0];
-  const int M = pair_stop_of(b, c1 - 1) - s0;
+  const BlockHeader *hp = b.blk_hdr + slot;
+  const HeaderRegs hd = load_header(hp, false);
+  if (hd.ncent == 0) return;
+  const int c0 = hd.c0, c1 = hd.c0 + hd.ncent;
+  const int s0 = hd.s0, M = hd.M;
   const double beta = ch.beta[0];
   for (int k = threadIdx.x; k < 3 * kCap; k += blockDim.x) gacc[k] = 0.0;
   int *cstart = reinterpret_cast<int *>(gacc) - 20;
-  if ((int)threadIdx.x <= c1 - c0 && threadIdx.x < 17)
-    cstart[threadIdx.x] = ((int)threadIdx.x < c1 - c0 ? b.pair_start[c0 + threadIdx.x] : s0 + M) - s0;
+  if (threadIdx.x < 17) cstart[threadIdx.x] = hp->rel[threadIdx.x];
   double *pctab = gacc + 3 * kCap;
   if constexpr (DEFZ && NSPEC == 1) {
     const int k = (int)blockDim.x - 1 - (int)threadIdx.x;
@@ -898,8 +945,17 @@
       pn4[item] = pc[4];
     }
   }
+  const int32_t *jcount = TRI ? b.job_count_own : b.job_count;
+  const uint32_t *jword = TRI ? b.job_word_own : b.job_word;
+  const size_t jbase = (size_t)blockIdx.x * b.job_stride;
+  uint32_t jw0 = 0u;
+  int n_listed = -1;
+  if (jcount) {
+    n_listed = jcount[blockIdx.x];
+    if ((int)threadIdx.x < b.job_stride) jw0 = jword[jbase + threadIdx.x];
+  }
   TA_STAMP(b, 1, 0);
-  stage<HD>(sf, ch, beta, b, f, s0, M);
+  stage<HD>(sf, ch, beta, b, f, hd, NSPEC == 1);
   TA_STAMP(b, 1, 1);
   const int nel = sf.n_elements;
 
@@ -913,9 +969,9 @@
       base = cstart[ci];
       n = cstart[ci + 1] - base;
     } else {
-      i = b.pair_i[p];
-      base = b.pair_start[i] - s0;
-      n = pair_stop_of(b, i) - b.pair_start[i];
+      int ci;
+      centre_of_lds(cstart, c1 - c0, item, ci, base, n);
+      i = c0 + ci;
     }
     const int a = item - base;
     const double2 axy = f.xy[item], azr = f.zr[item], aih = f.ih[item], ags = f.gs[item];
@@ -1017,9 +1073,9 @@
       base = cstart[ci];
       n = cstart[ci + 1] - base;
     } else {
-      i = b.pair_i[p];
-      base = b.pair_start[i] - s0;
-      n = pair_stop_of(b, i) - b.pair_start[i];
+      int ci;
+      centre_of_lds(cstart, c1 - c0, item, ci, base, n);
+      i = c0 + ci;
     }
     const int a = item - base;
     const double2 axy = f.xy[item], azr = f.zr[item], aih = f.ih[item], ags = f.gs[item];
@@ -1170,22 +1226,15 @@
   {
     int item = threadIdx.x;
     const bool active = item < M;
-    int n_own = 0;
-    if (active) {
-      const int i = b.pair_i[s0 + item];
-      n_own = pair_stop_of(b, i) - b.pair_start[i];
-    }
-    const bool one_pass = M <= (int)blockDim.x && !__syncthreads_or(active && (n_own >> 1) > 64);
-    const int32_t *jcount = TRI ? b.job_count_own : b.job_count;
-    const uint32_t *jword = TRI ? b.job_word_own : b.job_word;
-    const int n_jobs = (one_pass && jcount) ? jcount[blockIdx.x] : -1;
+    const bool one_pass = hd.one_pass;
+    const int n_jobs = one_pass ? n_listed : -1;
     if (n_jobs >= 0) {
-      const size_t jbase = (size_t)blockIdx.x * b.job_stride;
       uint32_t jws[4];
-#pragma unroll
-      for (int r = 0; r < 4; ++r) {
-        const int slot = job_slot(r, threadIdx.x, blockDim.x);
-        jws[r] = slot < n_jobs ? jword[jbase + slot] : 0u;
+      jws[0] = jw0;
+#pragma unroll
+      for (int r = 1; r < 4; ++r) {
+        const int js = job_slot(r, threadIdx.x, blockDim.x);
+        jws[r] = js < n_jobs ? jword[jbase + js] : 0u;
       }
       TA_STAMP(b, 1, 2);
 #pragma unroll
@@ -1202,6 +1251,8 @@
       unsigned long long mask = 0ull;
       if (active) {
         const int64_t p = (int64_t)s0 + item;
+        int ci, base, n_own;
+        centre_of_lds(cstart, c1 - c0, item, ci, base, n_own);
         const int smax = (f.ih[item].y != 0.0) ? n_own / 2 : 0;
         if (smax > 0) mask = b.masks[p];
       }
@@ -1223,12 +1274,12 @@
     double gx = gacc[item], gy = gacc[kCap + item], gz = gacc[2 * kCap + item];
     if (first) {
       const double *wr;
+      int ci = 0;
+      for (int k = 1; k < c1 - c0; ++k) ci += (item >= cstart[k]) ? 1 : 0;
       if (use_rtab) {
-        int ci = 0;
-        for (int k = 1; k < c1 - c0; ++k) ci += (item >= cstart[k]) ? 1 : 0;
         wr = rtab + ci * kRTab + (NSPEC == 1 ? 0 : (int)f.gs[item].y * sf.n_rad);
       } else {
-        const int i = b.pair_i[p];
+        const int i = c0 + ci;
         wr = b.dEdG + (size_t)i * sf.ndim + radial_term2(b.species[i], (int)f.gs[item].y) * sf.n_rad;
       }
       const double r2 = f.zr[item].y, inv_r = f.ih[item].x;
diff --git a/tensoralloy_amd/csrc/ta_nlist.hip b/tensoralloy_amd/csrc/ta_nlist.hip
--- a/tensoralloy_amd/csrc/ta_nlist.hip
+++ b/tensoralloy_amd/csrc/ta_nlist.hip
@@ -624,8 +624,10 @@
     int n_atoms, int nel, double rmax, const double *pos, const double *cells,
     const int32_t *frame_of_atom, const int32_t *start_super, const int32_t *seg_super, const int32_t *pj_super,
     const int32_t *ps_super, int32_t *seg_exact, int32_t *pair_start, int32_t *pair_stop, int32_t *pi_out,
-    int32_t *pj_out, int32_t *ps_out, int32_t *map, int32_t *slot_q, int cap, int32_t *blk_center) {
+    int32_t *pj_out, int32_t *ps_out, int32_t *map, int32_t *slot_q, int cap, int32_t *blk_center,
+    BlockHeader *blk_hdr) {
   __shared__ int cnt[kFilterGroup][kFilterMaxEl + 1];
+  __shared__ BlockHeader hdr[kFilterGroup];
   const int w = threadIdx.x >> 6, lane = threadIdx.x & 63;
   const int i0 = blockIdx.x * kFilterGroup;
   const int i = i0 + w;
@@ -664,22 +666,52 @@
   }
   if (!act && lane < nel) cnt[w][lane] = 0;
   __syncthreads();
+  __shared__ int run_k0[kFilterGroup], run_nc[kFilterGroup], run_first[kFilterGroup];
+  const int iend = min(i0 + kFilterGroup, n_atoms);
+  auto pairs_of = [&](int k) {
+    int n = 0;
+    for (int s = 0; s < nel; ++s) n += cnt[k][s];
+    return n;
+  };
   if (blk_center && threadIdx.x == 0) {
     int slot = i0, load = 0, nc = 0;
-    const int iend = min(i0 + kFilterGroup, n_atoms);
+    int total = start_super[i0];
     for (int k = 0; k < kFilterGroup && i0 + k < n_atoms; ++k) {
-      int n = 0;
-      for (int s = 0; s < nel; ++s) n += cnt[k][s];
+      const int n = pairs_of(k);
       if (k == 0 || load + n > cap || nc >= kMaxCentersPerBlock) {
+        if (k > 0) run_nc[slot - 1 - i0] = nc;
+        run_k0[slot - i0] = k;
+        run_first[slot - i0] = total;
         blk_center[slot++] = i0 + k;
         load = 0;
         nc = 0;
       }
       load += n;
+      total += n;
       ++nc;
     }
-    for (; slot < i0 + kFilterGroup; ++slot) blk_center[slot] = iend;
+    run_nc[slot - 1 - i0] = nc;
+    for (; slot < i0 + kFilterGroup; ++slot) {
+      blk_center[slot] = iend;
+      run_k0[slot - i0] = iend - i0;
+      run_nc[slot - i0] = 0;
+      run_first[slot - i0] = 0;
+    }
     if (iend == n_atoms) blk_center[i0 + kFilterGroup] = n_atoms;
+  }
+  if (blk_center && threadIdx.x < 64) {
+    __builtin_amdgcn_fence(__ATOMIC_RELEASE, "wavefront");
+    __builtin_amdgcn_wave_barrier();
+    __builtin_amdgcn_fence(__ATOMIC_ACQUIRE, "wavefront");
+    if (threadIdx.x < kFilterGroup) {
+      const int k0 = run_k0[threadIdx.x];
+      make_block_header(hdr[threadIdx.x], i0 + k0, run_nc[threadIdx.x], run_first[threadIdx.x], cap < 256 ? cap : 256,
+                        [&](int c) { return pairs_of(k0 + c); });
+    }
+    __builtin_amdgcn_fence(__ATOMIC_RELEASE, "wavefront");
+    __builtin_amdgcn_wave_barrier();
+    __builtin_amdgcn_fence(__ATOMIC_ACQUIRE, "wavefront");
+    reinterpret_cast<uint4 *>(blk_hdr + i0)[threadIdx.x] = reinterpret_cast<const uint4 *>(hdr)[threadIdx.x];
   }
   if (!act) return;
   int off = start_super[i0];
@@ -901,12 +933,13 @@
                const int32_t *frame_of_atom, const int32_t *start_super, const int32_t *seg_super,
                const int32_t *pj_super, const int32_t *ps_super, const int32_t *rev_super, int32_t *map,
                int32_t *seg_exact, int32_t *pair_start, int32_t *pair_stop, int32_t *pi_out, int32_t *pj_out,
-               int32_t *ps_out, int32_t *rev_out, int32_t *slot_q, int cap, int32_t *blk_center, hipStream_t s) {
+               int32_t *ps_out, int32_t *rev_out, int32_t *slot_q, int cap, int32_t *blk_center, BlockHeader *blk_hdr,
+               hipStream_t s) {
   if (n_atoms == 0) return;
   if (nel > kFilterMaxEl) throw std::domain_error("the MD-step list filter handles at most 8 elements");
   hipLaunchKernelGGL(filter_group_kernel, dim3(nblk(n_atoms, kFilterGroup)), dim3(64 * kFilterGroup), 0, s, n_atoms,
                      nel, rmax, pos, cells, frame_of_atom, start_super, seg_super, pj_super, ps_super, seg_exact,
-                     pair_start, pair_stop, pi_out, pj_out, ps_out, map, slot_q, cap, blk_center);
+                     pair_start, pair_stop, pi_out, pj_out, ps_out, map, slot_q, cap, blk_center, blk_hdr);
   if (n_super > 0 && !slot_q)
     hipLaunchKernelGGL(filter_rev_kernel, dim3(nblk(n_super, kBlock)), dim3(kBlock), 0, s, n_super, rev_super, map,
                        rev_out);
```

Measured after the change: 38.01 million, median of 6. 2.7% higher.
